# amin-abouee/apex-solver

Measured on AMD Instinct MI355X. Metric: ms per LM iter (Jacobian+Schur+solve), lower is better.
Workload: dtype f64; 1 GPU; final-13682 synthetic (13682 cameras / 4456117 landmarks / 28966251 observations); optimization_type=selfcal, camera_dof=9, schur_variant=sparse, s_tile_rows=856, s_tiles=8071, s_tiles_touched=4284, etree_levels=41, border_cameras=0, schur_form=4, variant_asked=Sparse, reason=, variant_choice=direct, parallelism=landmark-shard x1

## Files before the change

### apex-solver_amd/capi.py

```python
from __future__ import annotations

import ctypes as C
import os

import numpy as np

_HERE = os.path.dirname(os.path.abspath(__file__))
LIB_PATH = os.path.join(_HERE, "libapexgpu.so")
LIB_PATH = os.environ.get("APEXGPU_LIB", LIB_PATH)

NUM_STAGES = 10
STAGE_NAMES = ("cam_reduce", "landmark_reduce", "schur_scatter", "all_reduce", "factor", "tri_solve",
               "back_substitute", "step_stats", "retract", "cost")

SYMBOLS = (
    "apexgpu_create", "apexgpu_destroy", "apexgpu_last_error", "apexgpu_version", "apexgpu_set_structure",
    "apexgpu_set_cg_params", "apexgpu_set_params", "apexgpu_get_params", "apexgpu_cost", "apexgpu_assemble", "apexgpu_solve_augmented",
    "apexgpu_step_stats", "apexgpu_eval_step", "apexgpu_commit_step", "apexgpu_discard_step",
    "apexgpu_parameter_norm", "apexgpu_column_norms", "apexgpu_set_column_scaling", "apexgpu_lm_optimize", "apexgpu_get_residual", "apexgpu_get_jacobian_blocks",
    "apexgpu_get_schur", "apexgpu_camera_covariance", "apexgpu_covariance_stats", "apexgpu_landmark_covariance", "apexgpu_landmark_covariance_stats", "apexgpu_get_landmark_blocks", "apexgpu_get_hessian_csc", "apexgpu_debug_invert_blocks", "apexgpu_debug_pair_lists", "apexgpu_debug_pair_lists_queued", "apexgpu_debug_pair_lists_queued_dc", "apexgpu_debug_host_structure", "apexgpu_setup_times", "apexgpu_schur_matvec", "apexgpu_set_option", "apexgpu_enable_stage_timing", "apexgpu_reset_stage_times",
    "apexgpu_stage_times", "apexgpu_info", "apexgpu_variant_info", "apexgpu_variant_costs", "apexgpu_trim_host_cache", "apexgpu_host_cache_bytes", "apexgpu_counters", "apexgpu_debug_get_pair_records", "apexgpu_get_unique_id", "apexgpu_comm_init", "apexgpu_comm_init_shm", "apexgpu_set_shard", "apexgpu_shard_range",
    "apexgpu_debug_lockstep_solve", "apexgpu_export_step", "apexgpu_owned_landmarks", "apexgpu_debug_partition", "apexgpu_debug_check_schedule",
    "apexgpu_debug_schedule_ops", "apexgpu_debug_plan_lists", "apexgpu_debug_sinv_lists", "apexgpu_debug_sinv_lists_direct",
    "apexgpu_debug_tiles_create", "apexgpu_debug_tiles_pattern", "apexgpu_debug_tiles_set", "apexgpu_debug_tiles_factor",
    "apexgpu_debug_tiles_solve", "apexgpu_debug_tiles_matvec", "apexgpu_debug_tiles_pcg", "apexgpu_debug_tiles_get", "apexgpu_debug_tiles_destroy",
    "apexgpu_bal_open", "apexgpu_bal_close", "apexgpu_bal_last_error", "apexgpu_bal_sizes", "apexgpu_bal_raw",
    "apexgpu_bal_variables", "apexgpu_reference_columns",
    "apexgpu_pg_create", "apexgpu_pg_destroy", "apexgpu_pg_last_error", "apexgpu_pg_set_structure", "apexgpu_pg_set_params",
    "apexgpu_pg_get_params", "apexgpu_pg_cost", "apexgpu_pg_solve_augmented", "apexgpu_pg_step_stats", "apexgpu_pg_eval_step",
    "apexgpu_pg_commit_step", "apexgpu_pg_discard_step", "apexgpu_pg_parameter_norm", "apexgpu_pg_column_norms",
    "apexgpu_pg_set_column_scaling", "apexgpu_pg_lm_optimize",
    "apexgpu_pg_get_residual", "apexgpu_pg_get_jacobian_blocks", "apexgpu_pg_get_hessian", "apexgpu_pg_covariance", "apexgpu_pg_covariance_stats", "apexgpu_pg_set_option",
    "apexgpu_pg_enable_stage_timing", "apexgpu_pg_reset_stage_times", "apexgpu_pg_stage_times", "apexgpu_pg_info", "apexgpu_pg_counters",
    "apexgpu_pg_set_priors", "apexgpu_pg_get_prior_residual",
    "apexgpu_g2o_open", "apexgpu_g2o_close", "apexgpu_g2o_last_error", "apexgpu_g2o_sizes", "apexgpu_g2o_raw",
    "apexgpu_g2o_problem", "apexgpu_pose_graph_columns",
    "apexgpu_pg_create_se2", "apexgpu_pg_manifold", "apexgpu_g2o_raw_se2", "apexgpu_g2o_problem_se2",
    "apexgpu_pose_graph_columns_se2",
    "apexgpu_pg_create_so3",
    "apexgpu_pg_jv_gram", "apexgpu_pg_dogleg_step", "apexgpu_pg_gn_optimize", "apexgpu_pg_dogleg_optimize",
    "apexgpu_jv_gram", "apexgpu_dogleg_step", "apexgpu_dogleg_optimize",
    "apexgpu_pg_set_loss", "apexgpu_pg_get_loss", "apexgpu_loss_evaluate", "apexgpu_set_loss", "apexgpu_get_loss",
    "apexgpu_pg_set_information", "apexgpu_pg_get_information", "apexgpu_g2o_problem_information",
    "apexgpu_set_pose_priors", "apexgpu_set_intrinsic_priors", "apexgpu_get_prior_residual",
)
MANIFOLD_SE3, MANIFOLD_SE2, MANIFOLD_SO3 = 0, 1, 2
MANIFOLD_SIZES = {MANIFOLD_SE3: (7, 6), MANIFOLD_SE2: (3, 3), MANIFOLD_SO3: (4, 3)}
LOSS_KINDS = ("NONE", "L2", "L1", "HUBER", "CAUCHY", "FAIR", "GEMAN_MCCLURE", "WELSCH", "TUKEY", "ANDREWS", "RAMSAY",
              "TRIMMED_MEAN", "LP_NORM", "BARRON", "T_DISTRIBUTION")
(LOSS_NONE, LOSS_L2, LOSS_L1, LOSS_HUBER, LOSS_CAUCHY, LOSS_FAIR, LOSS_GEMAN_MCCLURE, LOSS_WELSCH, LOSS_TUKEY, LOSS_ANDREWS,
 LOSS_RAMSAY, LOSS_TRIMMED_MEAN, LOSS_LP_NORM, LOSS_BARRON, LOSS_T_DISTRIBUTION) = range(15)
PG_NUM_STAGES = 6
PG_STAGE_NAMES = ("assemble", "factor", "tri_solve", "step_stats", "retract", "cost")
_NON_INT = ("apexgpu_destroy", "apexgpu_debug_tiles_destroy", "apexgpu_last_error", "apexgpu_version", "apexgpu_host_cache_bytes", "apexgpu_bal_close", "apexgpu_bal_last_error",
            "apexgpu_pg_destroy", "apexgpu_pg_last_error", "apexgpu_g2o_close", "apexgpu_g2o_last_error")

ERROR_NAMES = {
    -1: "FactorizationFailed", -2: "SingularMatrix", -3: "SparseMatrixCreation", -4: "MatrixConversion",
    -5: "InvalidInput", -6: "InvalidState", -10: "DeviceError",
}


class LinAlgError(RuntimeError):

    def __init__(self, code: int, message: str):
        self.code = code
        self.kind = ERROR_NAMES.get(code, f"Error({code})")
        super().__init__(f"{self.kind}: {message}")


class LmConfigC(C.Structure):
    _fields_ = [
        ("max_iterations", C.c_int), ("cost_tolerance", C.c_double), ("parameter_tolerance", C.c_double),
        ("gradient_tolerance", C.c_double), ("damping", C.c_double), ("damping_min", C.c_double),
# ... 71 lines not shown
    L.apexgpu_eval_step.argtypes = [vp, C.POINTER(dbl)]
    L.apexgpu_commit_step.argtypes = [vp]
    L.apexgpu_discard_step.argtypes = [vp]
    L.apexgpu_parameter_norm.argtypes = [vp, C.POINTER(dbl)]
    L.apexgpu_column_norms.argtypes = [vp, vp]
    L.apexgpu_debug_lockstep_solve.argtypes = [vp, C.c_int, C.c_double]
    L.apexgpu_export_step.argtypes = [vp, vp, vp]
    L.apexgpu_owned_landmarks.argtypes = [vp, vp]
    L.apexgpu_debug_partition.argtypes = [C.c_int, vp, C.c_int, vp]
    L.apexgpu_debug_check_schedule.argtypes = [C.c_int, vp, C.c_int, C.c_int, vp, vp, C.c_char_p, C.c_int]
    L.apexgpu_debug_schedule_ops.argtypes = [C.c_int, vp, C.c_int, C.c_int, vp, C.c_int, vp, C.c_int]
    L.apexgpu_debug_plan_lists.argtypes = [C.c_int, vp, C.c_int, C.c_int, vp, C.c_int, vp, C.c_int]
    L.apexgpu_debug_sinv_lists.argtypes = [C.c_int, vp, vp, C.c_int, vp, vp]
    L.apexgpu_debug_sinv_lists_direct.argtypes = [C.c_int, vp, C.c_int, vp, vp, vp, C.c_int, vp, C.c_char_p, C.c_int]
    L.apexgpu_debug_tiles_create.argtypes = [C.c_int, C.c_int, vp, vp, C.POINTER(vp)]
    L.apexgpu_debug_tiles_pattern.argtypes = [vp, vp, vp]
    L.apexgpu_debug_tiles_set.argtypes = [vp, vp, C.c_int, dbl, C.c_int]
    L.apexgpu_debug_tiles_factor.argtypes = [vp, C.POINTER(C.c_int)]
    L.apexgpu_debug_tiles_solve.argtypes = [vp, C.c_int, vp, vp]
    L.apexgpu_debug_tiles_matvec.argtypes = [vp, vp, vp]
    L.apexgpu_debug_tiles_pcg.argtypes = [vp, vp, C.c_int, dbl, vp, C.POINTER(C.c_int), vp]
    L.apexgpu_debug_tiles_get.argtypes = [vp, C.c_int, vp, C.POINTER(C.c_int)]
    L.apexgpu_debug_tiles_destroy.argtypes = [vp]
    L.apexgpu_debug_tiles_destroy.restype = None
    L.apexgpu_set_column_scaling.argtypes = [vp, vp]
    L.apexgpu_lm_optimize.argtypes = [vp, C.POINTER(LmConfigC), C.POINTER(LmResultC), vp, C.c_int]
    L.apexgpu_get_residual.argtypes = [vp, vp]
    L.apexgpu_get_jacobian_blocks.argtypes = [vp, vp, vp]
    L.apexgpu_get_schur.argtypes = [vp, vp, vp]
    L.apexgpu_camera_covariance.argtypes = [vp, vp]
    L.apexgpu_covariance_stats.argtypes = [vp, C.POINTER(dbl * 6), vp, C.c_int]
    L.apexgpu_landmark_covariance.argtypes = [vp, vp]
    L.apexgpu_landmark_covariance_stats.argtypes = [vp, C.POINTER(dbl * 4)]
    L.apexgpu_get_landmark_blocks.argtypes = [vp, vp, vp]
    L.apexgpu_schur_matvec.argtypes = [vp, dbl, vp, vp, vp]
    L.apexgpu_set_option.argtypes = [vp, C.c_char_p, C.c_int]
    L.apexgpu_get_hessian_csc.argtypes = [vp, vp, vp, vp, vp]
    L.apexgpu_debug_invert_blocks.argtypes = [C.c_int, C.c_int64, vp, vp, vp]
    L.apexgpu_debug_host_structure.argtypes = [C.c_int64, C.c_int64, C.c_int64, C.c_int, vp, vp, C.c_int, C.c_int, vp, vp, vp, vp, vp]
    L.apexgpu_setup_times.argtypes = [vp, vp, vp]
    L.apexgpu_debug_pair_lists.argtypes = [C.c_int64, C.c_int64, C.c_int64, C.c_int, vp, vp, vp, vp, vp, vp, vp, vp]
    L.apexgpu_debug_pair_lists_queued.argtypes = [C.c_int64, C.c_int64, C.c_int64, vp, vp, vp, vp, vp, vp, vp, vp, vp]
    L.apexgpu_enable_stage_timing.argtypes = [vp, C.c_int]
    L.apexgpu_reset_stage_times.argtypes = [vp]
    L.apexgpu_stage_times.argtypes = [vp, C.POINTER(dbl * NUM_STAGES), C.POINTER(i64 * NUM_STAGES)]
    L.apexgpu_info.argtypes = [vp, C.POINTER(dbl * 16)]
    L.apexgpu_trim_host_cache.argtypes = [C.POINTER(C.c_int64)]
    L.apexgpu_host_cache_bytes.argtypes = []
    L.apexgpu_host_cache_bytes.restype = C.c_int64
    L.apexgpu_debug_get_pair_records.argtypes = [vp, vp, i64]
    L.apexgpu_variant_info.argtypes = [vp, C.c_int, C.POINTER(C.c_int), C.c_char_p, C.c_int]
    L.apexgpu_variant_costs.argtypes = [vp, C.POINTER(dbl * 4)]
    L.apexgpu_counters.argtypes = [vp, C.POINTER(i64 * 4)]
    L.apexgpu_get_unique_id.argtypes = [vp]
    L.apexgpu_comm_init.argtypes = [vp, C.c_int, C.c_int, vp]
    L.apexgpu_comm_init_shm.argtypes = [vp, C.c_int, C.c_int, C.c_char_p]
    L.apexgpu_set_shard.argtypes = [vp, C.c_int, C.c_int]
    L.apexgpu_shard_range.argtypes = [i64, i64, vp, C.c_int, C.c_int, C.POINTER(i64), C.POINTER(i64)]
    L.apexgpu_bal_open.argtypes = [C.c_char_p, C.POINTER(vp)]
    L.apexgpu_bal_close.argtypes = [vp]
    L.apexgpu_bal_close.restype = None
    L.apexgpu_bal_last_error.restype = C.c_char_p
    L.apexgpu_bal_sizes.argtypes = [vp, C.POINTER(i64), C.POINTER(i64), C.POINTER(i64)]
    L.apexgpu_bal_raw.argtypes = [vp, vp, vp, vp, vp, vp]
    L.apexgpu_bal_variables.argtypes = [vp, vp, vp]
    L.apexgpu_reference_columns.argtypes = [i64, i64, vp, vp, vp]
    L.apexgpu_pg_create.argtypes = [i64, i64, C.c_int, C.POINTER(vp)]
    L.apexgpu_pg_destroy.argtypes = [vp]
    L.apexgpu_pg_destroy.restype = None
    L.apexgpu_pg_last_error.argtypes = [vp]
    L.apexgpu_pg_last_error.restype = C.c_char_p
    L.apexgpu_pg_set_structure.argtypes = [vp, vp, vp, vp, vp, vp, dbl]
    L.apexgpu_pg_set_params.argtypes = [vp, vp]
    L.apexgpu_pg_set_priors.argtypes = [vp, C.c_int64, vp, vp, vp]
    L.apexgpu_pg_get_prior_residual.argtypes = [vp, vp]
    L.apexgpu_pg_set_loss.argtypes = [vp, C.c_int, dbl, dbl]
    L.apexgpu_set_loss.argtypes = [vp, C.c_int, dbl, dbl]
    L.apexgpu_set_pose_priors.argtypes = [vp, C.c_int64, vp, vp, vp, vp]
    L.apexgpu_set_intrinsic_priors.argtypes = [vp, C.c_int64, vp, vp, vp, vp]
    L.apexgpu_get_prior_residual.argtypes = [vp, vp, vp]
    L.apexgpu_get_loss.argtypes = [vp, C.POINTER(C.c_int), C.POINTER(dbl * 2)]
    L.apexgpu_pg_get_loss.argtypes = [vp, C.POINTER(C.c_int), C.POINTER(dbl * 2)]
    L.apexgpu_loss_evaluate.argtypes = [C.c_int, dbl, dbl, dbl, C.POINTER(dbl * 6)]
    L.apexgpu_pg_get_params.argtypes = [vp, vp]
    L.apexgpu_pg_cost.argtypes = [vp, C.POINTER(dbl)]
    L.apexgpu_pg_solve_augmented.argtypes = [vp, dbl, vp, vp]
    L.apexgpu_pg_step_stats.argtypes = [vp, C.POINTER(dbl * 3)]
    L.apexgpu_pg_eval_step.argtypes = [vp, C.POINTER(dbl)]
    L.apexgpu_pg_commit_step.argtypes = [vp]
    L.apexgpu_pg_discard_step.argtypes = [vp]
    L.apexgpu_pg_parameter_norm.argtypes = [vp, C.POINTER(dbl)]
    L.apexgpu_pg_column_norms.argtypes = [vp, vp]
    L.apexgpu_pg_set_column_scaling.argtypes = [vp, vp]
    L.apexgpu_pg_lm_optimize.argtypes = [vp, C.POINTER(LmConfigC), C.POINTER(LmResultC), vp, C.c_int]
    L.apexgpu_jv_gram.argtypes = [vp, vp, vp, C.POINTER(dbl * 3)]
    L.apexgpu_dogleg_step.argtypes = [vp, dbl, dbl, C.c_int, C.POINTER(dbl * 8)]
    L.apexgpu_dogleg_optimize.argtypes = [vp, C.POINTER(DlConfigC), C.POINTER(LmResultC), vp, C.c_int]
    L.apexgpu_pg_jv_gram.argtypes = [vp, vp, vp, C.POINTER(dbl * 3)]
    L.apexgpu_pg_dogleg_step.argtypes = [vp, dbl, dbl, C.c_int, C.POINTER(dbl * 8)]
    L.apexgpu_pg_gn_optimize.argtypes = [vp, C.POINTER(GnConfigC), C.POINTER(LmResultC), vp, C.c_int]
    L.apexgpu_pg_dogleg_optimize.argtypes = [vp, C.POINTER(DlConfigC), C.POINTER(LmResultC), vp, C.c_int]
    L.apexgpu_pg_get_residual.argtypes = [vp, vp]
    L.apexgpu_pg_get_jacobian_blocks.argtypes = [vp, vp]
    L.apexgpu_pg_get_hessian.argtypes = [vp, dbl, vp, vp]
    L.apexgpu_pg_covariance.argtypes = [vp, vp]
    L.apexgpu_pg_covariance_stats.argtypes = [vp, C.POINTER(dbl * 6), vp, C.c_int]
# ... 25 lines not shown
        if name not in _NON_INT:
            f.restype = C.c_int
    _lib = L
    return L


def tile_partition(present: np.ndarray, world: int):
    L = load()
    pr = np.ascontiguousarray(present, dtype=np.uint8)
    nt = pr.shape[0]
    owner = np.zeros(nt, dtype=np.int32)
    n_top = L.apexgpu_debug_partition(nt, pr.ctypes.data_as(C.c_void_p), int(world), owner.ctypes.data_as(C.c_void_p))
    if n_top < 0:
        raise LinAlgError(n_top, "apexgpu_debug_partition")
    return owner, n_top


def check_schedule(present: np.ndarray, world: int = 1, rank: int = 0, two_side: int = 1, overlap: int = 1, split_u1: int = 4,
                   flood_gate: int = 256, factor_flow: int = -1, factor_flow_rows: int = 24, old_idle_level_bug: bool = False,
                   drop_wait: int = -1) -> dict:
    L = load()
    pr = np.ascontiguousarray(present, dtype=np.uint8)
    nt = pr.shape[0]
    opts = np.array([two_side, overlap, split_u1, flood_gate, factor_flow, factor_flow_rows, int(old_idle_level_bug), drop_wait], dtype=np.int32)
    out = np.zeros(8, dtype=np.int64)
    msg = C.create_string_buffer(512)
    rc = L.apexgpu_debug_check_schedule(nt, pr.ctypes.data_as(C.c_void_p), int(world), int(rank), opts.ctypes.data_as(C.c_void_p),
                                        out.ctypes.data_as(C.c_void_p), msg, 512)
    if rc < 0:
        raise LinAlgError(rc, "apexgpu_debug_check_schedule: " + msg.value.decode())
    return dict(levels=rc, calls=int(out[0]), launches=int(out[1]), violations=int(out[2]) + int(out[3]), violations_top=int(out[3]),
                flow_units=int(out[4]), flow_groups=int(out[5]), waits=int(out[6]), dropped=bool(out[7]), first=msg.value.decode())


def schedule_ops(present: np.ndarray, phase: int = 0, world: int = 1, rank: int = 0, two_side: int = 1, overlap: int = 1, split_u1: int = 4,
                 flood_gate: int = 256, factor_flow: int = -1, factor_flow_rows: int = 24) -> np.ndarray:
    L = load()
    pr = np.ascontiguousarray(present, dtype=np.uint8)
    nt = pr.shape[0]
    opts = np.array([two_side, overlap, split_u1, flood_gate, factor_flow, factor_flow_rows, 0, -1], dtype=np.int32)
    args = (nt, pr.ctypes.data_as(C.c_void_p), int(world), int(rank), opts.ctypes.data_as(C.c_void_p), int(phase))
    n = L.apexgpu_debug_schedule_ops(*args, None, 0)
    if n < 0:
        raise LinAlgError(n, "apexgpu_debug_schedule_ops")
    rows = np.zeros((n, 6), dtype=np.int64)
    if n and L.apexgpu_debug_schedule_ops(*args, rows.ctypes.data_as(C.c_void_p), n) != n:
        raise LinAlgError(-6, "apexgpu_debug_schedule_ops")
    return rows


PLAN_TABLES = (("scalars", 23), ("slots", 3), ("columns", 4), ("owner_ranges", 5), ("levels", 9), ("fwd_cut", 2), ("upd_rounds", 2),
               ("bwd_step", 1), ("potrf", 5), ("panel", 7), ("upd", 7), ("fwd", 6), ("bwd", 6), ("flow_fwd", 10), ("flow_bwd", 10),
               ("units", 16), ("sym_row_ptr", 1), ("sym_entries", 3), ("sym_tiles", 3), ("group_cols", 2))


def plan_lists(present: np.ndarray, which: str, world: int = 1, rank: int = 0, two_side: int = 1, overlap: int = 1, split_u1: int = 4,
               flood_gate: int = 256, factor_flow: int = -1, factor_flow_rows: int = 24) -> np.ndarray:
    L = load()
    pr = np.ascontiguousarray(present, dtype=np.uint8)
    w = [n for n, _ in PLAN_TABLES].index(which)
    opts = np.array([two_side, overlap, split_u1, flood_gate, factor_flow, factor_flow_rows, 0, -1], dtype=np.int32)
    args = (pr.shape[0], pr.ctypes.data_as(C.c_void_p), int(world), int(rank), opts.ctypes.data_as(C.c_void_p), w)
    n = L.apexgpu_debug_plan_lists(*args, None, 0)
    if n < 0:
        raise LinAlgError(n, "apexgpu_debug_plan_lists")
    rows = np.zeros((n, PLAN_TABLES[w][1]), dtype=np.int64)
    if n and L.apexgpu_debug_plan_lists(*args, rows.ctypes.data_as(C.c_void_p), n) != n:
        raise LinAlgError(-6, "apexgpu_debug_plan_lists")
    return rows


def _sinv_rows(call, what, msg=None):
    counts = np.zeros(4, dtype=np.int64)
    n = call(None, 0, ptr(counts))
    if n < 0:
        raise LinAlgError(n, what + (": " + msg.value.decode() if msg is not None else ""))
    rows = np.zeros((n, 6), dtype=np.int64)
    if n and call(ptr(rows), n, ptr(counts)) != n:
        raise LinAlgError(-6, what)
    return rows, counts


def sinv_lists(present: np.ndarray, with_slots: bool = False):
    L = load()
    pr = np.ascontiguousarray(present, dtype=np.uint8)
    slot = np.zeros(pr.shape, dtype=np.int32)
    out = _sinv_rows(lambda rows, n, counts: L.apexgpu_debug_sinv_lists(pr.shape[0], ptr(pr), rows, n, counts, ptr(slot)), "apexgpu_debug_sinv_lists")
    return out + (slot,) if with_slots else out


def sinv_lists_direct(slot: np.ndarray, groups):
    L = load()
    sl = np.ascontiguousarray(slot, dtype=np.int32)
    gp = np.cumsum([0] + [len(g) for g in groups]).astype(np.int32)
    gc = np.array([c for g in groups for c in g] + [0], dtype=np.int32)
    msg = C.create_string_buffer(512)
    return _sinv_rows(lambda rows, n, counts: L.apexgpu_debug_sinv_lists_direct(sl.shape[0], ptr(sl), len(groups), ptr(gp), ptr(gc), rows, n, counts, msg, 512),
                      "apexgpu_debug_sinv_lists_direct", msg)


HOST_STRUCTURE_STATS = ("tile_rows", "hub_cameras", "border_tiles", "touched_tiles", "tiles", "etree_levels", "top_columns",
                        "tree_sharded", "s_order", "s_lists", "s_plan", "s_schur_lists", "s_uploads", "s_total", "pair_contributions",
                        "pair_blocks")


def host_structure(n_cam: int, n_pt: int, cam_idx: np.ndarray, pt_idx: np.ndarray, mode: int = 1, rank: int = 0, world: int = 1,
                   nested_dissection: int = 1, hubs_last: int = 1, dist_factor: int = 1, tree_sharding: int = 1, schur_form: int = 3):
    ci = np.ascontiguousarray(cam_idx, dtype=np.uint32); pi = np.ascontiguousarray(pt_idx, dtype=np.uint32)
    opts = np.array([nested_dissection, hubs_last, dist_factor, tree_sharding, schur_form], dtype=np.int32)
    stats = np.zeros(16); dc = 9 if mode in (1, 4, 5, 6) else 6
    nt = (n_cam * dc + 143) // 144
    cmap = np.zeros(n_cam, dtype=np.int32); owned = np.zeros(n_pt, dtype=np.uint8); towner = np.zeros(nt, dtype=np.int32)
    rc = load().apexgpu_debug_host_structure(n_cam, n_pt, len(ci), mode, ptr(ci), ptr(pi), rank, world, ptr(opts), ptr(stats),
                                             ptr(cmap), ptr(owned), ptr(towner))
    if rc != 0:
        raise LinAlgError(rc, "apexgpu_debug_host_structure failed")
    out = dict(zip(HOST_STRUCTURE_STATS, stats.tolist()))
    out.update(cmap=cmap, owned=owned.astype(bool), tile_owner=towner)
    return out
# ... 211 lines not shown
```

### apex-solver_amd/csrc/capi.cpp

```cpp
#include "../../include/apexgpu.h"

#include <string.h>

#include <algorithm>
#include <exception>
#include <new>
#include <string>
#include <vector>

#include "ba_structure.h"
#include "pg_solver.h"
#include "sinv_lists.h"
#include "solver.h"
#ifdef APEX_WITH_RCCL
#include <rccl/rccl.h>
#include <string.h>
#endif

struct apexgpu_solver {
    apex::Solver* s;
    std::string create_error;
};

static_assert(sizeof(apexgpu_lm_config) == sizeof(apex::LmConfig), "LmConfig layout");
static_assert(sizeof(apexgpu_lm_iter) == sizeof(apex::LmIterRecord), "LmIterRecord layout");
static_assert(sizeof(apexgpu_lm_result) == sizeof(apex::LmResult), "LmResult layout");
static_assert(sizeof(apexgpu_gn_config) == sizeof(apex::GnConfig), "GnConfig layout");
static_assert(sizeof(apexgpu_dl_config) == sizeof(apex::DlConfig), "DlConfig layout");
static_assert(sizeof(apexgpu_dl_iter) == sizeof(apex::DlIterRecord), "DlIterRecord layout");
static_assert(sizeof(apex::DoglegStepInfo) == 8 * sizeof(double), "DoglegStepInfo layout");
static_assert(APEXGPU_NUM_STAGES == apex::kNumStages, "stage count");
static_assert(APEXGPU_PG_NUM_STAGES == apex::kPgNumStages, "pose-graph stage count");

struct apexgpu_pg_solver {
    apex::PoseGraphSolver* s;
};

#define H_OR_FAIL            \
    if (!h || !h->s) return APEXGPU_ERR_INVALID_STATE

template <typename F>
static int guarded(F&& f) noexcept {
    try {
        return f();
    } catch (const std::bad_alloc&) {
        return APEXGPU_ERR_INVALID_INPUT;
    } catch (const std::exception&) {
        return APEXGPU_ERR_INVALID_INPUT;
    } catch (...) {
        return APEXGPU_ERR_INVALID_STATE;
    }
}

template <typename S>
static int covariance_stats(S* s, double out[6], double* group_ms, int group_cap) {
    if (!out) return APEXGPU_ERR_INVALID_INPUT;
    const apex::TilePlan& tp = s->plan();
    const apex::SelectedInverse& inv = tp.inverse();
    int64_t y = 0, zo = 0, zd = 0;
    inv.op_counts(&y, &zo, &zd);
    const std::vector<double>& ms = inv.group_ms();
    out[0] = (double)inv.bytes(); out[1] = (double)y; out[2] = (double)zo; out[3] = (double)zd; out[4] = tp.n_levels();
    int n = 0;
    if (group_ms)
        for (; n < group_cap && n < (int)ms.size(); ++n) group_ms[n] = ms[n];
    out[5] = n;
    return APEXGPU_OK;
}

template <typename S>
static bool shared_option(S* s, const std::string& n, int value) {
    if (n == "graphs") s->enable_graphs(value != 0);
    else if (n == "update_overlap") { s->enable_overlap(value != 0); if (value > 1) s->set_overlap_min(value); }
    else if (n == "tri_dataflow") s->enable_tri_flow(value != 0);
    else if (n == "split_u1") s->set_split_u1(value);
    else if (n == "flood_gate") s->set_gate_min(value);
    else if (n == "two_side") s->set_two_side(value);
    else if (n == "eager_step_eval") s->set_eager_step_eval(value != 0);
    else if (n == "one_wait") s->set_one_wait(value != 0);
    else if (n == "factor_flow") s->set_factor_flow(value, 0);
    else if (n == "factor_flow_rows") s->set_factor_flow(s->plan().factor_flow_cols(), value);
    else if (n == "debug_poison_sweep") s->debug_poison_next_solve(value);
    else if (n == "debug_poison_factor") s->debug_poison_next_factor();
    else if (n == "nested_dissection") s->set_nd(value != 0, value > 1 ? value : 0);
    else if (n == "covariance_timing") s->enable_covariance_timing(value != 0);
    else return false;
    return true;
}
template <typename S>
static int counters(S* s, int64_t out[4]) {
    if (!out) return APEXGPU_ERR_INVALID_INPUT;
    out[0] = s->sweep_timeouts(); out[1] = s->plan().tri_flow() ? 1 : 0; out[2] = s->factor_flow_timeouts(); out[3] = s->plan().factor_flow_groups();
    return APEXGPU_OK;
}
template <typename S>
static int stage_timing(S* s, int on) {
    if (on > 1) s->enable_stage_timing_only((uint32_t)on >> 1);
    else s->enable_stage_timing(on != 0);
    return APEXGPU_OK;
}

#include <execinfo.h>
#include <signal.h>
namespace {
void segv_backtrace(int sig) {
    void* frames[64];
    const int n = backtrace(frames, 64);
    backtrace_symbols_fd(frames, n, 2);
    raise(sig);
}
void segv_hook() {
    static const bool on = [] { const char* e = getenv("APEX_SEGV_BACKTRACE"); return e && e[0] == '1'; }();
    if (!on) return;
    static thread_local char alt[1 << 16];
    stack_t ss; ss.ss_sp = alt; ss.ss_size = sizeof(alt); ss.ss_flags = 0;
    (void)sigaltstack(&ss, nullptr);
    struct sigaction sa;
    memset(&sa, 0, sizeof(sa));
    sa.sa_handler = segv_backtrace; sa.sa_flags = SA_ONSTACK | SA_RESETHAND;
    (void)sigaction(SIGSEGV, &sa, nullptr);
}
}

extern "C" {

const char* apexgpu_version(void) { return "apexgpu 0.1 (gfx950)"; }

int apexgpu_create(int64_t n_cam, int64_t n_pt, int64_t n_obs, int mode, int device, apexgpu_solver** out) {
    if (!out) return APEXGPU_ERR_INVALID_INPUT;
// ... 240 lines not shown
    });
}

static int plan_table(const apex::PlanStructure& s, const apex::PlanLists& l, const double* tiles, const double* linv, int which, std::vector<int64_t>* out, int* width) {
    constexpr ptrdiff_t kTile = (ptrdiff_t)apex::kNB * apex::kNB;
    auto clean = [](const double* p) { return reinterpret_cast<const double*>(reinterpret_cast<uintptr_t>(p) & ~uintptr_t(7)); };
    auto in_linv = [&](const double* p) { return p >= linv && p < linv + s.nt * kTile; };
    auto arr = [&](const double* p) -> int64_t { p = clean(p); return !p ? -1 : in_linv(p) ? 1 : 0; };
    auto idx = [&](const double* p) -> int64_t { p = clean(p); return !p ? -1 : in_linv(p) ? (p - linv) / kTile : (p - tiles) / kTile; };
    auto bits = [](double v) { int64_t b; memcpy(&b, &v, sizeof b); return b; };
    auto row = [&](std::initializer_list<int64_t> v) { *width = (int)v.size(); out->insert(out->end(), v); };
    auto gemm = [&](const std::vector<apex::GemmTask>& v) {
        *width = 7;
        for (const apex::GemmTask& t : v) row({arr(t.C), idx(t.C), (int64_t)(reinterpret_cast<uintptr_t>(t.C) & 1), arr(t.A), idx(t.A), arr(t.B), idx(t.B)});
    };
    auto tri = [&](const std::vector<apex::TriTask>& v) {
        *width = 6;
        for (const apex::TriTask& t : v) row({arr(t.Mdiag), idx(t.Mdiag), arr(t.Moff), idx(t.Moff), t.k, t.other});
    };
    auto flow = [&](const std::vector<apex::FlowTask>& v) {
        *width = 10;
        for (const apex::FlowTask& t : v) row({arr(t.mat), idx(t.mat), t.src, t.dst, t.part, t.count, arr(t.mat2), idx(t.mat2), t.src2, t.slot2});
    };
    const int nt = s.nt;
    switch (which) {
        case 0: {
            const apex::PlanLists::Flow* f = l.flow;
            row({s.n_levels(), s.n_local_groups, s.n_top_cols, s.n_slots, s.n_touched, (int64_t)l.potrf.size(), (int64_t)l.panel.size(), (int64_t)l.upd.size(),
                 l.two_side_plan, l.first_ok, f[0].g0, f[0].g1, f[0].first, f[0].n, f[1].g0, f[1].g1, f[1].first, f[1].n, l.n_flow_local, l.n_flow_parts,
                 bits(s.predicted_ms), bits(f[0].sim_us), bits(f[1].sim_us)});
            break;
        }
        case 1: *width = 3; for (int I = 0; I < nt; ++I) for (int J = 0; J < nt; ++J) if (s.slot_of(I, J) >= 0) row({I, J, s.slot_of(I, J)}); break;
        case 2: *width = 4; for (int K = 0; K < nt; ++K) row({K, s.cls[K], s.owner[K], s.diag_slot[K]}); break;
        case 3:
            for (size_t o = 0; o < s.own_range.size(); ++o) row({(int64_t)o, s.own_range[o].first, s.own_range[o].second, s.own_fill[o].first, s.own_fill[o].second});
            row({-1, s.n_t_nt, s.n_touched - s.n_t_nt, s.n_f_nt, s.n_slots - s.n_f_nt});
            break;
        case 4: *width = 9; for (const apex::Level& v : l.lv) row({v.potrf, v.panel, v.fwd, v.upd, v.u1o, v.u2a, v.u2b1, v.u2b2, (int64_t)v.fwd_cut.size()}); break;
        case 5: *width = 2; for (size_t g = 0; g < l.lv.size(); ++g) for (int c : l.lv[g].fwd_cut) row({(int64_t)g, c}); break;
        case 6: *width = 2; for (const auto& r : l.upd_rounds) row({r.first, r.second}); break;
        case 7: *width = 1; for (int b : l.bwd_step) row({b}); break;
        case 8: *width = 5; for (const apex::PotrfTask& t : l.potrf) row({arr(t.A), idx(t.A), arr(t.Linv), idx(t.Linv), t.K}); break;
        case 9: gemm(l.panel); break;
        case 10: gemm(l.upd); break;
        case 11: tri(l.fwd); break;
        case 12: tri(l.bwd); break;
        case 13: flow(l.flow_fwd); break;
        case 14: flow(l.flow_bwd); break;
        case 15:
            *width = 16;
            for (const apex::FactorUnit& u : l.units)
                row({arr(u.C), idx(u.C), arr(u.A), idx(u.A), arr(u.B), idx(u.B), u.wait_flag[0], u.wait_flag[1], u.wait_flag[2], u.wait_val[0], u.wait_val[1], u.wait_val[2],
                     u.pub, u.kind, u.strip, u.pad});
            break;
        case 16: *width = 1; for (int v : l.sym_row_ptr) row({v}); break;
        case 17: *width = 3; for (const apex::SymEntry& e : l.sym_entries) row({e.slot, e.other, e.kind}); break;
        case 18: *width = 3; for (const apex::SymTile& t : l.sym_tiles) row({t.slot, t.I, t.J}); break;
        case 19: *width = 2; for (size_t g = 0; g < s.group_cols.size(); ++g) for (int K : s.group_cols[g]) row({(int64_t)g, K}); break;
        default: return APEXGPU_ERR_INVALID_INPUT;
    }
    return APEXGPU_OK;
}

int apexgpu_debug_plan_lists(int nt, const uint8_t* present, int world, int rank, const int opts[8], int which, int64_t* rows, int max_rows) {
    if (nt <= 0 || !present || !opts || world < 1 || rank < 0 || rank >= world || max_rows < 0 || (max_rows > 0 && !rows)) return APEXGPU_ERR_INVALID_INPUT;
    return guarded([&]() -> int {
    const HostPlan hp = host_plan(nt, present, world, rank, opts);
    if (!hp.err.empty()) return APEXGPU_ERR_INVALID_STATE;
    std::vector<int64_t> out;
    int width = 1;
    const int rc = plan_table(hp.s, hp.l, reinterpret_cast<const double*>(apex::kStandInTiles), reinterpret_cast<const double*>(apex::kStandInLinv), which, &out, &width);
    if (rc != APEXGPU_OK) return rc;
    const size_t n = out.size() / (size_t)width;
    if (max_rows > 0) memcpy(rows, out.data(), std::min(n, (size_t)max_rows) * (size_t)width * sizeof(int64_t));
    return (int)n;
    });
}

static int sinv_rows(const apex::SinvLists& l, int64_t* rows, int max_rows, int64_t counts[4]) {
    const size_t n = l.tasks.size() + l.prods.size();
    size_t i = 0;
    for (size_t g = 0; g < l.groups.size(); ++g)
        for (int k = 0; k < 3; ++k)
            for (int t = l.groups[g][k]; t < l.groups[g][k + 1] && i < (size_t)max_rows; ++t, ++i) {
                const apex::SinvTaskH& tk = l.tasks[t];
                int64_t* r = rows + 6 * i;
                r[0] = k; r[1] = (int64_t)g; r[2] = tk.C.array; r[3] = tk.C.tile; r[4] = tk.first; r[5] = tk.count;
            }
    for (size_t p = 0; p < l.prods.size() && l.tasks.size() + p < (size_t)max_rows; ++p) {
        const apex::SinvProdH& pr = l.prods[p];
        int64_t* r = rows + 6 * (l.tasks.size() + p);
        r[0] = 3; r[1] = pr.A.array; r[2] = pr.A.tile; r[3] = pr.B.array; r[4] = pr.B.tile; r[5] = pr.op;
    }
    if (counts) { counts[0] = l.n[0]; counts[1] = l.n[1]; counts[2] = l.n[2]; counts[3] = l.y_max; }
    return (int)n;
}

int apexgpu_debug_sinv_lists(int nt, const uint8_t* present, int64_t* rows, int max_rows, int64_t counts[4], int32_t* slot_out) {
    if (nt <= 0 || !present || max_rows < 0 || (max_rows > 0 && !rows)) return APEXGPU_ERR_INVALID_INPUT;
    return guarded([&]() -> int {
    const apex::PlanStructure s = apex::plan_structure(nt, std::vector<uint8_t>(present, present + (size_t)nt * nt), apex::PlanOptions());
    if (s.refused) return APEXGPU_ERR_INVALID_STATE;
    if (slot_out) memcpy(slot_out, s.slot.data(), (size_t)nt * nt * sizeof(int32_t));
    apex::SinvLists lists;
    if (!apex::build_sinv_lists(nt, s.slot.data(), s.group_cols, &lists).empty()) return APEXGPU_ERR_INVALID_STATE;
    return sinv_rows(lists, rows, max_rows, counts);
    });
}

int apexgpu_debug_sinv_lists_direct(int nt, const int32_t* slot, int n_groups, const int32_t* group_ptr, const int32_t* group_cols,
                                    int64_t* rows, int max_rows, int64_t counts[4], char* msg, int msg_len) {
    if (nt <= 0 || !slot || n_groups < 0 || !group_ptr || !group_cols || max_rows < 0 || (max_rows > 0 && !rows)) return APEXGPU_ERR_INVALID_INPUT;
    return guarded([&]() -> int {
    std::vector<std::vector<int>> groups(n_groups);
    for (int g = 0; g < n_groups; ++g) {
        if (group_ptr[g] < 0 || group_ptr[g + 1] < group_ptr[g]) return APEXGPU_ERR_INVALID_INPUT;
        for (int i = group_ptr[g]; i < group_ptr[g + 1]; ++i) {
            if (group_cols[i] < 0 || group_cols[i] >= nt || slot[(size_t)group_cols[i] * nt + group_cols[i]] < 0) return APEXGPU_ERR_INVALID_INPUT;
            groups[g].push_back(group_cols[i]);
        }
    }
    apex::SinvLists lists;
    const std::string e = apex::build_sinv_lists(nt, slot, groups, &lists);
    if (msg && msg_len > 0) snprintf(msg, (size_t)msg_len, "%s", e.c_str());
    if (!e.empty()) return APEXGPU_ERR_INVALID_STATE;
    return sinv_rows(lists, rows, max_rows, counts);
    });
}

int apexgpu_owned_landmarks(apexgpu_solver* h, uint8_t* mask) {
    H_OR_FAIL;
    if (!mask) return APEXGPU_ERR_INVALID_INPUT;
    return h->s->owned_landmarks(mask);
}
int apexgpu_export_step(apexgpu_solver* h, double* step_out, double* grad_out) { H_OR_FAIL; return guarded([&] { return h->s->export_step(step_out, grad_out); }); }

int apexgpu_set_option(apexgpu_solver* h, const char* name, int value) {
    H_OR_FAIL;
    const std::string n = name ? name : "";
    static const char* const structural[] = {"schur_form", "hubs_last", "dist_factor", "tree_sharding", "dist_selftest", "nested_dissection", "update_overlap",
                                             "split_u1", "flood_gate", "two_side", "factor_flow", "factor_flow_rows", "device_pair_list", "matrix_free_only",
                                             "auto_variant", "variant_cost_permille", "max_tile_updates"};
    if (h->s->has_structure())
        for (const char* k : structural)
            if (n == k) return APEXGPU_ERR_INVALID_STATE;
    if (n == "schur_form") {
        if (value != 3 && value != 4) return APEXGPU_ERR_INVALID_INPUT;
        h->s->set_schur_form(value);
    }
    else if (shared_option(h->s, n, value)) return APEXGPU_OK;
    else if (n == "matrix_free_only") h->s->set_matrix_free_only(value != 0);
    else if (n == "auto_variant") h->s->set_auto_variant(value != 0);
    else if (n == "variant_cost_permille") h->s->set_variant_cost_permille(value);
    else if (n == "device_pair_list") h->s->set_device_pair_recs(value != 0);
    else if (n == "max_tile_updates") h->s->set_max_tile_updates(value);
    else if (n == "debug_occupy_cus") return h->s->debug_occupy_cus(value, 40000);
    else if (n == "hubs_last") h->s->set_hubs_last(value != 0);
    else if (n == "dist_factor") h->s->set_dist_factor(value != 0);
    else if (n == "tree_sharding") h->s->set_tree_sharding(value != 0);
    else if (n == "dist_selftest") h->s->set_dist_selftest(value);
    else return APEXGPU_ERR_INVALID_INPUT;
    return APEXGPU_OK;
}
int apexgpu_enable_stage_timing(apexgpu_solver* h, int on) {
    H_OR_FAIL;
    return stage_timing(h->s, on);
}
int apexgpu_reset_stage_times(apexgpu_solver* h) { H_OR_FAIL; h->s->reset_stage_times(); return APEXGPU_OK; }
int apexgpu_stage_times(apexgpu_solver* h, double ms[APEXGPU_NUM_STAGES], int64_t calls[APEXGPU_NUM_STAGES]) {
    H_OR_FAIL;
    h->s->stage_times(ms, calls);
    return APEXGPU_OK;
}
int apexgpu_setup_times(apexgpu_solver* h, double seconds[6], double counts[4]) {
    H_OR_FAIL;
    if (!seconds) return APEXGPU_ERR_INVALID_INPUT;
    for (int k = 0; k < 6; ++k) seconds[k] = h->s->setup_seconds()[k];
    if (counts) { counts[0] = h->s->n_hubs(); counts[1] = h->s->pair_blocks(); counts[2] = h->s->pair_slots(); counts[3] = h->s->schur_form(); }
    return APEXGPU_OK;
}
int apexgpu_info(apexgpu_solver* h, double info[16]) {
    H_OR_FAIL;
    info[0] = h->s->n_tile_rows(); info[1] = (double)h->s->tile_count(); info[2] = h->s->schur_scatter_pairs();
    info[3] = (double)h->s->cam_dof_internal(); info[4] = h->s->last_reg(); info[5] = h->s->last_pcg_iters();
    info[6] = h->s->touched_tiles(); info[7] = h->s->local_obs();
    info[8] = h->s->n_levels();
    int64_t a = 0, b = 0, c = 0;
    h->s->plan().op_counts(&a, &b, &c);
    info[9] = (double)a; info[10] = (double)b; info[11] = (double)c;
    info[12] = h->s->dist_top_columns(); info[13] = h->s->dist_local_fraction();
    info[14] = h->s->tree_sharded() ? 1.0 : 0.0;
    info[15] = h->s->schur_form();
    return APEXGPU_OK;
}

int apexgpu_debug_get_pair_records(apexgpu_solver* h, uint32_t* recs4_out, int64_t cap_slots) {
    H_OR_FAIL;
    if (!recs4_out) return APEXGPU_ERR_INVALID_INPUT;
    return guarded([&] { return h->s->get_pair_records(recs4_out, cap_slots); });
}
int apexgpu_trim_host_cache(int64_t* released_bytes) {
    const size_t n = apex::HostBlockCache::get().trim();
    if (released_bytes) *released_bytes = (int64_t)n;
    return APEXGPU_OK;
}
int apexgpu_variant_costs(apexgpu_solver* h, double out[4]) {
    H_OR_FAIL;
    if (!out) return APEXGPU_ERR_INVALID_INPUT;
    h->s->variant_costs(out);
    return APEXGPU_OK;
}
int64_t apexgpu_host_cache_bytes(void) { return (int64_t)apex::HostBlockCache::get().kept_bytes(); }
int apexgpu_variant_info(apexgpu_solver* h, int asked_variant, int* used_variant, char* reason, int reason_len) {
    H_OR_FAIL;
    if (asked_variant != APEXGPU_VARIANT_SPARSE && asked_variant != APEXGPU_VARIANT_ITERATIVE && asked_variant != APEXGPU_VARIANT_IMPLICIT)
        return APEXGPU_ERR_INVALID_INPUT;
    if (used_variant) *used_variant = h->s->variant_used(asked_variant);
    if (reason && reason_len > 0) {
        const std::string& r = h->s->variant_reason();
        const size_t n = std::min<size_t>(r.size(), (size_t)reason_len - 1);
        memcpy(reason, r.data(), n);
        reason[n] = 0;
    }
    return APEXGPU_OK;
}

int apexgpu_counters(apexgpu_solver* h, int64_t out[4]) {
    H_OR_FAIL;
    return counters(h->s, out);
}

int apexgpu_get_unique_id(void* out128) {
#ifdef APEX_WITH_RCCL
    if (!out128) return APEXGPU_ERR_INVALID_INPUT;
    ncclUniqueId id;
    if (ncclGetUniqueId(&id) != ncclSuccess) return APEXGPU_ERR_DEVICE;
    memcpy(out128, &id, 128);
    return APEXGPU_OK;
#else
    (void)out128;
    return APEXGPU_ERR_INVALID_STATE;
#endif
}
int apexgpu_comm_init(apexgpu_solver* h, int world, int rank, const void* unique_id128) {
    H_OR_FAIL;
    if (!unique_id128) return APEXGPU_ERR_INVALID_INPUT;
    return guarded([&] { return h->s->comm_init(world, rank, unique_id128); });
}
int apexgpu_comm_init_shm(apexgpu_solver* h, int world, int rank, const char* name) {
    H_OR_FAIL;
    if (!name) return APEXGPU_ERR_INVALID_INPUT;
    return guarded([&] { return h->s->comm_init_shm(world, rank, name); });
}
int apexgpu_shard_range(int64_t n_pt, int64_t n_obs, const uint32_t* pt_idx, int rank, int world, int64_t* lo, int64_t* hi) {
    if (!pt_idx || !lo || !hi || world < 1 || rank < 0 || rank >= world || n_pt <= 0) return APEXGPU_ERR_INVALID_INPUT;
    return guarded([&]() -> int {
        std::vector<int64_t> ptr(n_pt + 1, 0);
        for (int64_t i = 0; i < n_obs; ++i) {
            if (pt_idx[i] >= (uint64_t)n_pt) return APEXGPU_ERR_INVALID_INPUT;
            ptr[pt_idx[i] + 1]++;
        }
        for (int64_t l = 0; l < n_pt; ++l) ptr[l + 1] += ptr[l];
        apex::shard_range(n_pt, ptr.data(), rank, world, lo, hi);
        return APEXGPU_OK;
    });
}
int apexgpu_set_shard(apexgpu_solver* h, int rank, int world) { H_OR_FAIL; return h->s->set_shard(rank, world); }

static int debug_pair_lists_impl(int64_t n_cam, int64_t n_pt, int64_t n_obs, int dc, const uint32_t* cam_idx, const uint32_t* pt_idx,
                                 int64_t counts[4], uint32_t* recs4_out, int32_t* chunks2_out, int64_t* blocks4_out,
                                 int32_t* tasks2_out, int32_t* o_index_out, bool queued, int64_t* qdesc3_out) {
    if (n_cam <= 0 || n_pt <= 0 || n_obs < 0 || (dc != 6 && dc != 9) || !cam_idx || !pt_idx || !counts) return APEXGPU_ERR_INVALID_INPUT;
    return guarded([&]() -> int {
        for (int64_t i = 0; i < n_obs; ++i)
            if (cam_idx[i] >= (uint64_t)n_cam || pt_idx[i] >= (uint64_t)n_pt) return APEXGPU_ERR_INVALID_INPUT;
        std::vector<int> pt_ptr(n_pt + 1, 0), order(n_obs);
        for (int64_t i = 0; i < n_obs; ++i) pt_ptr[pt_idx[i] + 1]++;
        for (int64_t l = 0; l < n_pt; ++l) pt_ptr[l + 1] += pt_ptr[l];
        { std::vector<int> fill(pt_ptr.begin(), pt_ptr.end() - 1); for (int64_t i = 0; i < n_obs; ++i) order[fill[pt_idx[i]]++] = (int)i; }
        for (int64_t l = 0; l < n_pt; ++l)
            std::stable_sort(order.begin() + pt_ptr[l], order.begin() + pt_ptr[l + 1], [&](int a, int b) { return cam_idx[a] < cam_idx[b]; });
        std::vector<uint32_t> o_cam(n_obs), o_pt(n_obs);
// ... 229 lines not shown
    return APEXGPU_OK;
}
int apexgpu_pg_set_information(apexgpu_pg_solver* h, const double* info) {
    PG_OR_FAIL;
    return guarded([&] { return h->s->set_information(info); });
}
int apexgpu_pg_get_information(apexgpu_pg_solver* h, int* present, double* info_out) {
    PG_OR_FAIL;
    if (!present) return APEXGPU_ERR_INVALID_INPUT;
    return h->s->get_information(present, info_out);
}
int apexgpu_loss_evaluate(int kind, double p0, double p1, double s, double out6[6]) {
    apex::PgLoss l;
    if (!out6 || !apex::pg_loss_make(kind, p0, p1, &l)) return APEXGPU_ERR_INVALID_INPUT;
    apex::pg_loss_evaluate(l, s, out6);
    const apex::PgCorrector c = apex::pg_corrector(out6, s);
    out6[3] = c.sqrt_rho1; out6[4] = c.residual_scaling; out6[5] = c.alpha_sq_norm;
    return APEXGPU_OK;
}
int apexgpu_pg_get_prior_residual(apexgpu_pg_solver* h, double* r7_out) {
    PG_OR_FAIL;
    return h->s->get_prior_residual(r7_out);
}
int apexgpu_pg_get_hessian(apexgpu_pg_solver* h, double lambda, double* H_out, double* g_out) {
    PG_OR_FAIL;
    return h->s->get_hessian(lambda, H_out, g_out);
}
int apexgpu_pg_covariance(apexgpu_pg_solver* h, double* cov_out) {
    PG_OR_FAIL;
    return guarded([&] { return h->s->covariance(cov_out); });
}
int apexgpu_pg_covariance_stats(apexgpu_pg_solver* h, double out[6], double* group_ms, int group_cap) { PG_OR_FAIL; return covariance_stats(h->s, out, group_ms, group_cap); }
int apexgpu_pg_set_option(apexgpu_pg_solver* h, const char* name, int value) {
    PG_OR_FAIL;
    const std::string n = name ? name : "";
    if (n == "row_owned_assembly")
        return (value == 0 || value == 1) && h->s->set_row_owned_option(value == 1) ? APEXGPU_OK : APEXGPU_ERR_INVALID_INPUT;
    return shared_option(h->s, n, value) ? APEXGPU_OK : APEXGPU_ERR_INVALID_INPUT;
}
int apexgpu_pg_enable_stage_timing(apexgpu_pg_solver* h, int on) {
    PG_OR_FAIL;
    return stage_timing(h->s, on);
}
int apexgpu_pg_reset_stage_times(apexgpu_pg_solver* h) { PG_OR_FAIL; h->s->reset_stage_times(); return APEXGPU_OK; }
int apexgpu_pg_stage_times(apexgpu_pg_solver* h, double ms[APEXGPU_PG_NUM_STAGES], int64_t calls[APEXGPU_PG_NUM_STAGES]) {
    PG_OR_FAIL;
    h->s->stage_times(ms, calls);
    return APEXGPU_OK;
}
int apexgpu_pg_counters(apexgpu_pg_solver* h, int64_t out[4]) {
    PG_OR_FAIL;
    return counters(h->s, out);
}
int apexgpu_pg_info(apexgpu_pg_solver* h, double info[8]) {
    PG_OR_FAIL;
    info[0] = h->s->n_tile_rows(); info[1] = (double)h->s->tile_count(); info[2] = (double)h->s->touched_tiles();
    info[3] = h->s->n_levels(); info[4] = (double)h->s->dof() * (double)h->s->n_vertices();
    int64_t a = 0, b = 0, c = 0;
    h->s->plan().op_counts(&a, &b, &c);
    info[5] = (double)a; info[6] = (double)b; info[7] = (double)c;
    return APEXGPU_OK;
}

}
```

### apex-solver_amd/csrc/chol_kernels.h

```cpp
#pragma once
#include <hip/hip_runtime.h>
#include <stdint.h>

#include "ba_kernels.h"
#include "tile_tasks.h"

namespace apex {

void launch_potrf_inv(const PotrfTask* tasks, int n, int* fail, hipStream_t s, int* arrived = nullptr);
void launch_gate(const int* arrived, int expected, int max_micros, hipStream_t s);
void launch_factor_flow(const FactorUnit* units, int n_units, int* ver, int* fail, int* err, hipStream_t s,
                        unsigned long long* trace = nullptr);
void launch_tile_gemm_nt(const GemmTask* tasks, int n, double alpha, double beta, hipStream_t s, bool tri_b = false);
void launch_clear_i32(int* p, int64_t n, hipStream_t s);
void launch_post_word(int* word, int* host_word_dev, hipStream_t s);
void launch_tri_flow(bool backward, const FlowTask* tasks, int n_tasks, const double* in, double* out, double* part, int* flags,
                     int nt, hipStream_t s, const double* fold_b, double* fold_out, int poison_block = -1, bool keep_flags = false);
void launch_occupy_cus(int n, int micros, int* started, hipStream_t s);
void launch_tri_step(bool trans, const TriTask* tasks, int n, double* vwork, double* vout, hipStream_t s);
void launch_tile_diag(const double* tiles, const int* diag_slot, int nt, double* diag, hipStream_t s);
void launch_tile_add_diag(double* tiles, const int* diag_slot, int n_valid, int n_total, double add_valid,
                          double set_pad, hipStream_t s);
void launch_vec_select(int n, const double* in, const int* cls, int mask, double* out, hipStream_t s);
void launch_vec_merge(int n, const double* src, const int* cls, int mask, double* dst, hipStream_t s);
void launch_tile_scale_sym(const SymTile* list, int n, double* tiles, const double* scale , hipStream_t s);

}
```

### apex-solver_amd/csrc/chol_kernels.hip

```cpp
#include <hip/hip_runtime.h>
#include <stdint.h>

#include "chol_kernels.h"
#include "device_reduce.hpp"
#include "tile_kernel_defs.h"
#include <algorithm>

namespace apex {

constexpr int BS = 16;
constexpr int NBK = NB / BS;
constexpr int BP = 18;
constexpr int BSZ = BS * BP;
constexpr int NLB = NBK * (NBK + 1) / 2;

__device__ __forceinline__ int bidx(int bi, int bj) { return bi * (bi + 1) / 2 + bj; }

__device__ __forceinline__ double readlane_f64(double v, int src) {
    const int lo = __builtin_amdgcn_readlane(__double2loint(v), src);
    const int hi = __builtin_amdgcn_readlane(__double2hiint(v), src);
    return __hiloint2double(hi, lo);
}

__device__ __forceinline__ double4_t blk_mma_nt(const double* X, const double* Y, double4_t acc, int lr, int lk, double sgn) {
// ... 38 lines not shown
__device__ __forceinline__ __amdgpu_buffer_rsrc_t coh_rsrc(const void* tile) {
    return __builtin_amdgcn_make_buffer_rsrc(const_cast<void*>(tile), 0, NB * NB * (int)sizeof(double), 0x00020000);
}
template <bool COH>
__device__ __forceinline__ double2 tile_ld2(const double* tile, __amdgpu_buffer_rsrc_t r, int off) {
    if constexpr (COH) {
        const i32x4_t q = __builtin_amdgcn_raw_buffer_load_b128(r, off * 8, 0, kCohAux);
        double2 v; v.x = __hiloint2double(q[1], q[0]); v.y = __hiloint2double(q[3], q[2]);
        return v;
    } else {
        return *reinterpret_cast<const double2*>(tile + off);
    }
}
template <bool COH>
__device__ __forceinline__ void tile_st2(double* tile, __amdgpu_buffer_rsrc_t r, int off, double2 v) {
    if constexpr (COH) {
        i32x4_t q;
        q[0] = __double2loint(v.x); q[1] = __double2hiint(v.x); q[2] = __double2loint(v.y); q[3] = __double2hiint(v.y);
        __builtin_amdgcn_raw_buffer_store_b128(q, r, off * 8, 0, kCohAux);
    } else {
        *reinterpret_cast<double2*>(tile + off) = v;
    }
}
__device__ __forceinline__ double coh_ld1(__amdgpu_buffer_rsrc_t r, int off) {
    const i32x2_t q = __builtin_amdgcn_raw_buffer_load_b64(r, off * 8, 0, kCohAux);
    return __hiloint2double(q[1], q[0]);
}
__device__ __forceinline__ void coh_st1(__amdgpu_buffer_rsrc_t r, int off, double v) {
    i32x2_t q; q[0] = __double2loint(v); q[1] = __double2hiint(v);
    __builtin_amdgcn_raw_buffer_store_b64(q, r, off * 8, 0, kCohAux);
}
template <bool COH>
__device__ __forceinline__ void blk_to_tile(const double* __restrict__ src, double* __restrict__ dst_tile, __amdgpu_buffer_rsrc_t r,
                                            int bi, int bj, int t, int nthreads) {
    for (int idx = t; idx < 128; idx += nthreads) {
        const int rr = idx >> 3, c2 = idx & 7;
        double2 v; v.x = src[rr * BP + 2 * c2]; v.y = src[rr * BP + 2 * c2 + 1];
        tile_st2<COH>(dst_tile, r, (16 * bi + rr) * NB + 16 * bj + 2 * c2, v);
    }
}

__device__ __forceinline__ double4_t blk_load_cd_sym(const double* C, int lr, int lk) {
    double4_t v;
#pragma unroll
    for (int r = 0; r < 4; ++r) {
        const int row = lk + 4 * r;
        v[r] = row >= lr ? C[row * BP + lr] : C[lr * BP + row];
    }
    return v;
}

template <int NW, bool COH>
__device__ __forceinline__ void potrf_tile_mf(double* __restrict__ A, double* __restrict__ Linv, int K, int* __restrict__ fail,
                                              double* sA, double* sD, int* bad, int* sync_cnt) {
    constexpr int NT = 64 * NW;
    const int tid = threadIdx.x, lane = tid & 63, w = tid >> 6;
    const int lr = lane & 15, lk = lane >> 4;
    constexpr int NH = NW - (NW + 3) / 4;
    const bool helper = (w & 3) != 0;
    const int hid = w - 1 - (w >> 2);
    const __amdgpu_buffer_rsrc_t rA = coh_rsrc(A), rL = coh_rsrc(Linv);
    if (tid == 0) { *bad = 0; *sync_cnt = 0; }
    {
        constexpr int NREG = (128 * 45 + NT - 1) / NT + NBK;
        double2 reg[NREG];
        int n = 0;
#pragma unroll
        for (int bi = 0; bi < NBK; ++bi) {
            const int per_row = 8 * (bi + 1), cnt = 16 * per_row;
#pragma unroll
            for (int it = 0; it < (16 * 8 * (bi + 1) + NT - 1) / NT; ++it, ++n) {
                const int idx = tid + NT * it;
                if (idx < cnt) {
                    const int rr = idx / per_row, c2 = idx - rr * per_row;
                    reg[n] = tile_ld2<COH>(A, rA, (16 * bi + rr) * NB + 2 * c2);
                }
            }
        }
        n = 0;
#pragma unroll
        for (int bi = 0; bi < NBK; ++bi) {
            const int per_row = 8 * (bi + 1), cnt = 16 * per_row;
#pragma unroll
            for (int it = 0; it < (16 * 8 * (bi + 1) + NT - 1) / NT; ++it, ++n) {
                const int idx = tid + NT * it;
                if (idx < cnt) {
                    const int rr = idx / per_row, c2 = idx - rr * per_row;
                    double* dst = sA + bidx(bi, c2 >> 3) * BSZ + rr * BP + 2 * (c2 & 7);
                    dst[0] = reg[n].x; dst[1] = reg[n].y;
                }
            }
        }
    }
    __syncthreads();
    POTRF_STAMP();

    double4_t Dm = (double4_t){0.0, 0.0, 0.0, 0.0};
    if (w == 0) Dm = blk_load_cd_sym(sA, lr, lk);
    for (int kb = 0; kb < NBK; ++kb) {
        double4_t T[(NBK - 1 + NH - 1) / NH];
        if (w == 0) {
            double4_t Xm, Ls = (double4_t){0.0, 0.0, 0.0, 0.0}, Xs = (double4_t){0.0, 0.0, 0.0, 0.0};
#pragma unroll
            for (int r = 0; r < 4; ++r) Xm[r] = (lk + 4 * r == lr) ? 1.0 : 0.0;
            double rmask[4];
#pragma unroll
            for (int q = 0; q < 4; ++q) rmask[q] = lk == q ? 1.0 : 0.0;
            auto rsq_newton = [](double d) {
                double r = __builtin_amdgcn_rsq(d);
                r = r * fma(-0.5 * d * r, r, 1.5);
// ... 70 lines not shown
                    double4_t acc = (double4_t){0.0, 0.0, 0.0, 0.0};
                    for (int k = j; k < r; ++k) {
                        const double* Y = (k == j) ? (sD + j * BSZ) : (sA + bidx(k, j) * BSZ);
                        acc = blk_mma_nn(sA + bidx(r, k) * BSZ, Y, acc, lr, lk);
                    }
                    T[nt] = acc;
                }
            }
        }
        __syncthreads();
        POTRF_STAMP();
        if (helper && kb >= 1) {
            const int r = kb - 1;
            int nt = 0;
            for (int j = hid; j < r; j += NH, ++nt) blk_store_cd(sA + bidx(r, j) * BSZ, T[nt], lr, lk, -1.0);
        }
        {
            const int m = NBK - 1 - kb;
            if (w == 0) {
                if (m > 0) {
                    double* N = sA + bidx(kb + 1, kb) * BSZ;
                    double4_t Lt = (double4_t){0.0, 0.0, 0.0, 0.0};
                    Lt = blk_mma_nt(sD + kb * BSZ, N, Lt, lr, lk, 1.0);
                    Dm = blk_load_cd_sym(sA + bidx(kb + 1, kb + 1) * BSZ, lr, lk);
#pragma unroll
                    for (int r = 0; r < 4; ++r) N[lr * BP + lk + 4 * r] = Lt[r];
#pragma unroll
                    for (int r = 0; r < 4; ++r) Dm = __builtin_amdgcn_mfma_f64_16x16x4f64(-Lt[r], Lt[r], Dm, 0, 0, 0);
                }
            } else if (helper) {
                const int t0 = m > 0 ? 1 : 0;
                for (int t = t0 + hid; t < m + kb; t += NH) {
                    if (t < m) {
                        double* P = sA + bidx(kb + 1 + t, kb) * BSZ;
                        double4_t acc = (double4_t){0.0, 0.0, 0.0, 0.0};
                        acc = blk_mma_nt(P, sD + kb * BSZ, acc, lr, lk, 1.0);
                        blk_store_cd(P, acc, lr, lk, 1.0);
                    } else {
                        const int k = t - m;
                        double* Bk = sA + bidx(kb, k) * BSZ;
                        blk_to_tile<COH>(Bk, A, rA, kb, k, lane, 64);
                        double4_t acc = (double4_t){0.0, 0.0, 0.0, 0.0};
                        acc = blk_mma_nn(sD + kb * BSZ, Bk, acc, lr, lk);
                        blk_store_cd(Bk, acc, lr, lk, 1.0);
                    }
                }
                if (hid == NH - 1) blk_to_tile<COH>(sA + bidx(kb, kb) * BSZ, A, rA, kb, kb, lane, 64);
            }
        }
        if (w == 0 || helper) {
            __builtin_amdgcn_fence(__ATOMIC_RELEASE, "workgroup");
            if (lane == 0) __hip_atomic_fetch_add(sync_cnt, 1, __ATOMIC_RELAXED, __HIP_MEMORY_SCOPE_WORKGROUP);
        }
        if (helper) {
            const int target = (kb + 1) * (NH + 1);
            while (__hip_atomic_load(sync_cnt, __ATOMIC_RELAXED, __HIP_MEMORY_SCOPE_WORKGROUP) < target) __builtin_amdgcn_s_sleep(0);
            __builtin_amdgcn_fence(__ATOMIC_ACQUIRE, "workgroup");
        }
        POTRF_STAMP();
    }
    __syncthreads();
    {
        const int r = NBK - 1;
        double4_t T[(NBK - 1 + NW - 1) / NW];
        int nt = 0;
        for (int j = w; j < r; j += NW, ++nt) {
            double4_t acc = (double4_t){0.0, 0.0, 0.0, 0.0};
            for (int k = j; k < r; ++k) {
                const double* Y = (k == j) ? (sD + j * BSZ) : (sA + bidx(k, j) * BSZ);
                acc = blk_mma_nn(sA + bidx(r, k) * BSZ, Y, acc, lr, lk);
            }
            T[nt] = acc;
        }
        __syncthreads();
        nt = 0;
        for (int j = w; j < r; j += NW, ++nt) blk_store_cd(sA + bidx(r, j) * BSZ, T[nt], lr, lk, -1.0);
        __syncthreads();
    }
#pragma unroll
    for (int bi = 0; bi < NBK; ++bi) {
        const int per_row = 8 * (bi + 1), cnt = 16 * per_row;
        for (int idx = tid; idx < cnt; idx += NT) {
            const int rr = idx / per_row, c2 = idx - rr * per_row;
            const int bj = c2 >> 3;
            const double* src = ((bj == bi) ? (sD + bi * BSZ) : (sA + bidx(bi, bj) * BSZ)) + rr * BP + 2 * (c2 & 7);
            double2 v; v.x = src[0]; v.y = src[1];
            tile_st2<COH>(Linv, rL, (16 * bi + rr) * NB + 2 * c2, v);
        }
    }
    if (tid == 0 && *bad) atomicCAS(fail, 0, K + 1);
    POTRF_STAMP();
}

template <int NW>
__global__ __launch_bounds__(64 * NW) void k_potrf_inv_mf(const PotrfTask* __restrict__ tasks, int* __restrict__ fail,
                                                          int* __restrict__ arrived) {
    if (arrived != nullptr && threadIdx.x == 0) __hip_atomic_fetch_add(arrived, 1, __ATOMIC_RELAXED, __HIP_MEMORY_SCOPE_AGENT);
    POTRF_STAMP();
    __shared__ double sA[NLB * BSZ];
    __shared__ double sD[NBK * BSZ];
    __shared__ int bad, sync_cnt;
    const PotrfTask pt = tasks[blockIdx.x];
    potrf_tile_mf<NW, false>(pt.A, pt.Linv, pt.K, fail, sA, sD, &bad, &sync_cnt);
}
#undef POTRF_STAMP

constexpr int KC = 16;
constexpr int STRIP = 48;
constexpr int NSTRIP = NB / STRIP;
constexpr int kGemmSmallMax = 56;

template <bool TRI>
__global__ __launch_bounds__(256, 3) void k_tile_gemm_nt(const GemmTask* __restrict__ tasks, int n_units, double alpha, double beta) {
    constexpr int P4 = KC + 2;
    constexpr int IMG = (NB + STRIP) * P4;
    __shared__ double sm[IMG];
    const int per_xcd = (n_units + 7) >> 3;
    const int unit = (blockIdx.x & 7) * per_xcd + (blockIdx.x >> 3);
    if ((int)(blockIdx.x >> 3) >= per_xcd || unit >= n_units) return;
    GemmTask tg = tasks[unit / NSTRIP];
    const bool first = (reinterpret_cast<uintptr_t>(tg.C) & 1) != 0;
    tg.C = reinterpret_cast<double*>(reinterpret_cast<uintptr_t>(tg.C) & ~uintptr_t(7));
    const int strip = unit % NSTRIP;
    const int tid = threadIdx.x, lane = tid & 63, w = __builtin_amdgcn_readfirstlane(tid >> 6);
    const int lr = lane & 15, lk = lane >> 4;
    GlobalCF64 Ag = (GlobalCF64)tg.A + (size_t)strip * STRIP * NB;
    GlobalCF64 Bg = (GlobalCF64)tg.B;
    constexpr int NACC = TRI ? 9 : 7;
    int cb[3];
    if (TRI) { cb[0] = 16 * (8 - w); cb[1] = 16 * (1 + w); cb[2] = w == 3 ? 0 : -16; }
    else { cb[0] = 32 * w; cb[1] = 32 * w + 16; cb[2] = 128; }
    const bool extra = TRI ? (w == 3) : (w < 3);
    double4_t acc[NACC];
#pragma unroll
    for (int j = 0; j < NACC; ++j) acc[j] = (double4_t){0.0, 0.0, 0.0, 0.0};
    constexpr int C2 = KC / 2, NR = (NB + STRIP) * C2 / 256, RPR = 256 / C2;
    static_assert((NB + STRIP) * C2 % 256 == 0 && 256 % C2 == 0 && NR == 6 && RPR == 32, "staging loop assumes whole rounds");
    const int r0 = tid / C2, c2 = tid % C2;
    const unsigned offB = r0 * NB + 2 * c2, offA = (r0 + 16) * NB + 2 * c2;
    GlobalCF64 p4 = r0 < 16 ? Bg + (size_t)(r0 + 128) * NB + 2 * c2 : Ag + (size_t)(r0 - 16) * NB + 2 * c2;
    const int dst0 = r0 * P4 + 2 * c2;
    f64x2_t rg[NR];
    auto gload = [&](int k0) {
#pragma unroll
        for (int i = 0; i < 4; ++i) rg[i] = *reinterpret_cast<GlobalCF64x2>(Bg + (offB + (unsigned)(RPR * i * NB + k0)));
        rg[4] = *reinterpret_cast<GlobalCF64x2>(p4 + k0);
        rg[5] = *reinterpret_cast<GlobalCF64x2>(Ag + (offA + (unsigned)k0));
    };
    auto stage = [&](double* img) {
#pragma unroll
        for (int i = 0; i < NR; ++i) { img[dst0 + RPR * i * P4] = rg[i].x; img[dst0 + RPR * i * P4 + 1] = rg[i].y; }
    };
    auto compute = [&](const double* img, int k0) {
        const double* sB = img;
        const double* sA = img + NB * P4;
#pragma unroll
        for (int kk = 0; kk < KC; kk += 4) {
            if (TRI) {
                if (k0 > cb[0]) continue;
                double av[3], bv[3];
#pragma unroll
                for (int i = 0; i < 3; ++i) av[i] = sA[(16 * i + lr) * P4 + kk + lk];
#pragma unroll
                for (int j = 0; j < 3; ++j) bv[j] = sB[((cb[j] < 0 ? 0 : cb[j]) + lr) * P4 + kk + lk];
#pragma unroll
                for (int j = 0; j < 3; ++j) {
                    if (k0 > cb[j]) continue;
#pragma unroll
                    for (int i = 0; i < 3; ++i)
                        acc[3 * i + j] = __builtin_amdgcn_mfma_f64_16x16x4f64(av[i], bv[j], acc[3 * i + j], 0, 0, 0);
                }
            } else {
                double av[3], bv[2];
#pragma unroll
                for (int i = 0; i < 3; ++i) av[i] = sA[(16 * i + lr) * P4 + kk + lk];
#pragma unroll
                for (int j = 0; j < 2; ++j) bv[j] = sB[(cb[j] + lr) * P4 + kk + lk];
#pragma unroll
                for (int i = 0; i < 3; ++i)
#pragma unroll
                    for (int j = 0; j < 2; ++j)
                        acc[2 * i + j] = __builtin_amdgcn_mfma_f64_16x16x4f64(av[i], bv[j], acc[2 * i + j], 0, 0, 0);
                if (extra) {
                    const double ax = sA[(16 * w + lr) * P4 + kk + lk], bx = sB[(128 + lr) * P4 + kk + lk];
                    acc[6] = __builtin_amdgcn_mfma_f64_16x16x4f64(ax, bx, acc[6], 0, 0, 0);
                }
            }
        }
    };
    gload(0);
    for (int k0 = 0; k0 < NB; k0 += KC) {
        __syncthreads();
        stage(sm);
        __syncthreads();
        if (k0 + KC < NB) gload(k0 + KC);
        compute(sm, k0);
    }
    GlobalF64 C = (GlobalF64)tg.C + (size_t)strip * STRIP * NB;
    auto brow = [&](int n) { return TRI ? 16 * (n / 3) : (n < 6 ? 16 * (n / 2) : 16 * w); };
    auto bcol = [&](int n) { return TRI ? cb[n % 3] : (n < 6 ? cb[n % 2] : 128); };
    if (beta == 0.0 || first) {
        const double zero = first ? 0.0 : -0.0;
#pragma unroll
        for (int n = 0; n < NACC; ++n) {
            if (TRI ? (n % 3 == 2 && !extra) : (n == 6 && !extra)) continue;
#pragma unroll
            for (int r = 0; r < 4; ++r) C[(size_t)(brow(n) + lk + 4 * r) * NB + bcol(n) + lr] = alpha * acc[n][r] + zero;
        }
        return;
    }
    if (TRI) {
#pragma unroll
        for (int n = 0; n < NACC; ++n) {
            if (n % 3 == 2 && !extra) continue;
#pragma unroll
            for (int r = 0; r < 4; ++r) {
                GlobalF64 p = C + (size_t)(brow(n) + lk + 4 * r) * NB + bcol(n) + lr;
                *p = alpha * acc[n][r] + beta * *p;
            }
        }
        return;
    }
    double cv[3][4];
#pragma unroll
    for (int n = 0; n < 2; ++n)
#pragma unroll
        for (int r = 0; r < 4; ++r) cv[n][r] = C[(size_t)(brow(n) + lk + 4 * r) * NB + bcol(n) + lr];
#pragma unroll
    for (int n = 0; n < NACC; ++n) {
        if (n + 2 < NACC && (n + 2 < 6 || extra)) {
#pragma unroll
            for (int r = 0; r < 4; ++r) cv[(n + 2) % 3][r] = C[(size_t)(brow(n + 2) + lk + 4 * r) * NB + bcol(n + 2) + lr];
        }
        if (n == 6 && !extra) continue;
#pragma unroll
        for (int r = 0; r < 4; ++r)
            C[(size_t)(brow(n) + lk + 4 * r) * NB + bcol(n) + lr] = alpha * acc[n][r] + beta * cv[n % 3][r];
    }
}

__global__ __launch_bounds__(192) void k_tile_gemm_nt_small(const GemmTask* __restrict__ tasks, int n_units, double alpha,
                                                              double beta) {
    __shared__ double sA[48 * PS];
    __shared__ double sB[48 * PS];
    const int unit = blockIdx.x;
    if (unit >= n_units) return;
    GemmTask tg = tasks[unit / 9];
    const bool first = (reinterpret_cast<uintptr_t>(tg.C) & 1) != 0;
    tg.C = reinterpret_cast<double*>(reinterpret_cast<uintptr_t>(tg.C) & ~uintptr_t(7));
    if (first) beta = 0.0;
    const int blk = unit % 9, bi = blk / 3, bj = blk % 3;
    GlobalCF64 Ag = (GlobalCF64)tg.A + (size_t)bi * 48 * NB;
    GlobalCF64 Bg = (GlobalCF64)tg.B + (size_t)bj * 48 * NB;
    GlobalF64 C = (GlobalF64)tg.C + (size_t)bi * 48 * NB + bj * 48;
    const int tid = threadIdx.x, lane = tid & 63, w = tid >> 6;
    const int lr = lane & 15, lk = lane >> 4;
    double4_t acc[3];
#pragma unroll
    for (int j = 0; j < 3; ++j) acc[j] = (double4_t){0.0, 0.0, 0.0, 0.0};
    constexpr int C2 = KS / 2, NR = 48 * C2 / 192;
    static_assert(48 * C2 % 192 == 0 && NB % KS == 0, "staging loops assume whole rounds");
    f64x2_t ra[NR], rb[NR];
    auto gload = [&](int k0) {
#pragma unroll
        for (int i = 0; i < NR; ++i) {
            const int idx = tid + 192 * i, row = idx / C2, c2 = idx % C2;
            ra[i] = *reinterpret_cast<GlobalCF64x2>(Ag + (size_t)row * NB + k0 + 2 * c2);
            rb[i] = *reinterpret_cast<GlobalCF64x2>(Bg + (size_t)row * NB + k0 + 2 * c2);
        }
    };
    double cv[3][4];
    if (beta != 0.0) {
#pragma unroll
        for (int j = 0; j < 3; ++j)
#pragma unroll
            for (int r = 0; r < 4; ++r) cv[j][r] = C[(size_t)(16 * w + lk + 4 * r) * NB + 16 * j + lr];
    }
    gload(0);
    for (int k0 = 0; k0 < NB; k0 += KS) {
        __syncthreads();
#pragma unroll
        for (int i = 0; i < NR; ++i) {
            const int idx = tid + 192 * i, row = idx / C2, c2 = idx % C2;
            sA[row * PS + 2 * c2] = ra[i].x; sA[row * PS + 2 * c2 + 1] = ra[i].y;
            sB[row * PS + 2 * c2] = rb[i].x; sB[row * PS + 2 * c2 + 1] = rb[i].y;
        }
        __syncthreads();
        if (k0 + KS < NB) gload(k0 + KS);
#pragma unroll
        for (int kk = 0; kk < KS; kk += 4) {
            const double a = sA[(16 * w + lr) * PS + kk + lk];
#pragma unroll
            for (int j = 0; j < 3; ++j) {
                const double b = sB[(16 * j + lr) * PS + kk + lk];
                acc[j] = __builtin_amdgcn_mfma_f64_16x16x4f64(a, b, acc[j], 0, 0, 0);
            }
        }
    }
#pragma unroll
    for (int j = 0; j < 3; ++j)
#pragma unroll
        for (int r = 0; r < 4; ++r) {
            const double v = alpha * acc[j][r];
            C[(size_t)(16 * w + lk + 4 * r) * NB + 16 * j + lr] = (beta != 0.0) ? v + beta * cv[j][r] : (first ? v + 0.0 : v);
        }
}

__global__ __launch_bounds__(576) void k_tile_gemm_nt_small_strip(const GemmTask* __restrict__ tasks, int n_units, double alpha,
                                                                    double beta) {
    __shared__ double sA[48 * PS];
    __shared__ double sB[NB * PS];
    const int unit = blockIdx.x;
    if (unit >= n_units) return;
    const GemmTask tg = tasks[unit / 3];
    const int bi = unit % 3;
    GlobalCF64 Ag = (GlobalCF64)tg.A + (size_t)bi * 48 * NB;
    GlobalCF64 Bg = (GlobalCF64)tg.B;
    GlobalF64 C = (GlobalF64)tg.C + (size_t)bi * 48 * NB;
    const int tid = threadIdx.x, lane = tid & 63, w = tid >> 6;
    const int lr = lane & 15, lk = lane >> 4;
    const int wr = w / 3, wc = w % 3;
    double4_t acc[3];
#pragma unroll
    for (int j = 0; j < 3; ++j) acc[j] = (double4_t){0.0, 0.0, 0.0, 0.0};
    constexpr int C2 = KS / 2, NRA = 48 * C2 / 576, NRB = NB * C2 / 576;
    static_assert(48 * C2 % 576 == 0 && NB * C2 % 576 == 0, "staging loops assume whole rounds");
    f64x2_t ra[NRA], rb[NRB];
    auto gload = [&](int k0) {
#pragma unroll
        for (int i = 0; i < NRA; ++i) {
            const int idx = tid + 576 * i, row = idx / C2, c2 = idx % C2;
            ra[i] = *reinterpret_cast<GlobalCF64x2>(Ag + (size_t)row * NB + k0 + 2 * c2);
        }
#pragma unroll
        for (int i = 0; i < NRB; ++i) {
            const int idx = tid + 576 * i, row = idx / C2, c2 = idx % C2;
            rb[i] = *reinterpret_cast<GlobalCF64x2>(Bg + (size_t)row * NB + k0 + 2 * c2);
        }
    };
    gload(0);
    for (int k0 = 0; k0 < NB; k0 += KS) {
        __syncthreads();
#pragma unroll
        for (int i = 0; i < NRA; ++i) {
            const int idx = tid + 576 * i, row = idx / C2, c2 = idx % C2;
            sA[row * PS + 2 * c2] = ra[i].x; sA[row * PS + 2 * c2 + 1] = ra[i].y;
        }
#pragma unroll
        for (int i = 0; i < NRB; ++i) {
            const int idx = tid + 576 * i, row = idx / C2, c2 = idx % C2;
            sB[row * PS + 2 * c2] = rb[i].x; sB[row * PS + 2 * c2 + 1] = rb[i].y;
        }
        __syncthreads();
        if (k0 + KS < NB) gload(k0 + KS);
#pragma unroll
        for (int kk = 0; kk < KS; kk += 4) {
            const double a = sA[(16 * wr + lr) * PS + kk + lk];
#pragma unroll
            for (int j = 0; j < 3; ++j) {
                const double b = sB[(48 * wc + 16 * j + lr) * PS + kk + lk];
                acc[j] = __builtin_amdgcn_mfma_f64_16x16x4f64(a, b, acc[j], 0, 0, 0);
            }
        }
    }
#pragma unroll
    for (int j = 0; j < 3; ++j)
#pragma unroll
        for (int r = 0; r < 4; ++r) {
            GlobalF64 dst = C + (size_t)(16 * wr + lk + 4 * r) * NB + 48 * wc + 16 * j + lr;
            const double v = alpha * acc[j][r];
            *dst = (beta != 0.0) ? v + beta * *dst : v;
        }
}

constexpr int HROWS = NB / 2;
constexpr int TP = NB + 1;

template <bool TRANS>
__device__ __forceinline__ void tile_gemv_lds(const double* __restrict__ M, const double* sv, double* sout, double* sT,
                                              double* spart, int tid) {
    double accT = 0.0;
    for (int h = 0; h < 2; ++h) {
        double2 reg[21];
#pragma unroll
        for (int i = 0; i < 21; ++i) {
            const int idx = tid + 256 * i;
            if (idx < HROWS * (NB / 2)) {
                const int row = idx / (NB / 2), c2 = idx - row * (NB / 2);
                reg[i] = *reinterpret_cast<const double2*>(M + (size_t)(HROWS * h + row) * NB + 2 * c2);
            }
        }
        __syncthreads();
// ... 264 lines not shown
        }
        spart[g][c] = v;
        __syncthreads();
        if (tid < NB) {
            const double* __restrict__ bsrc = t.src == -2 ? fold_b : b;
            const double rhs = bsrc ? bsrc[(size_t)t.dst * NB + tid] : 0.0;
            const double val = rhs - ((spart[0][tid] + spart[1][tid]) + (spart[2][tid] + spart[3][tid]));
            if (t.src == -2) fold_out[(size_t)t.dst * NB + tid] = val;
            else sx[tid] = val;
        }
        if (t.src == -2) return;
    }
    __syncthreads();
    double acc[kFwdRows];
    matvec(m, acc);
    if (cl == 15) {
        double* __restrict__ o = (t.src >= 0 ? part + (size_t)t.part * NB : y + (size_t)t.dst * NB) + row0;
#pragma unroll
        for (int rr = 0; rr < kFwdRows; ++rr) flow_st(o + rr, acc[rr]);
    }
    flow_publish(t.src >= 0 ? cnt + t.dst : done + t.dst, tid);
}

__device__ __forceinline__ void flow_wait_ge(const int* ver, int flag, int want, int tid, int* err) {
    if (flag >= 0) flow_wait(ver + flag, want, tid, err);
}
__device__ __forceinline__ void flow_wait_unit(const int* ver, const FactorUnit& u, int tid, int* err) {
    const int f0 = u.wait_flag[0], f1 = u.wait_flag[1], f2 = u.wait_flag[2], w0 = u.wait_val[0], w1 = u.wait_val[1], w2 = u.wait_val[2];
    if (tid < 64) {
        const int f = tid == 0 ? f0 : (tid == 1 ? f1 : (tid == 2 ? f2 : -1));
        const int want = tid == 0 ? w0 : (tid == 1 ? w1 : w2);
        int spins = 0;
        for (;;) {
            const bool ok = f < 0 || __hip_atomic_load(ver + f, __ATOMIC_RELAXED, __HIP_MEMORY_SCOPE_AGENT) >= want;
            if (__all(ok)) break;
            const bool dead = tid == 3 && __hip_atomic_load(err, __ATOMIC_RELAXED, __HIP_MEMORY_SCOPE_AGENT) != 0;
            if (__any(dead)) break;
            __builtin_amdgcn_s_sleep(1);
            if (++spins > kFlowSpinLimit) { if (tid == 0) atomicOr(err, 1); break; }
        }
    }
    __syncthreads();
}

constexpr int kFlowFactorThreadsC = 768;
constexpr int kFlowPK = NB + 2;
__device__ __forceinline__ void flow_update_unit(const FactorUnit& u, double* __restrict__ sA, double* __restrict__ sB,
                                                 int* __restrict__ ver, int* __restrict__ err, unsigned long long* __restrict__ trace) {
    const int tid = threadIdx.x, lane = tid & 63, w = tid >> 6;
    const int lr = lane & 15, lk = lane >> 4;
    const int wr = w / 3, wc = w % 3;
    const int bi = u.strip / 3, bj = u.strip % 3;
    const __amdgpu_buffer_rsrc_t rC = coh_rsrc(u.C), rA = coh_rsrc(u.A), rB = coh_rsrc(u.B);
    flow_wait_unit(ver, u, tid, err);
    if (trace && tid == 0) trace[1] = wall_clock64();
    const bool act = tid < 576;
    double cv[4] = {0.0, 0.0, 0.0, 0.0};
    if (act && !(u.kind & kFlowFirstWriter)) {
#pragma unroll
        for (int r = 0; r < 4; ++r) cv[r] = coh_ld1(rC, (48 * bi + 16 * wr + lk + 4 * r) * NB + 48 * bj + 16 * wc + lr);
    }
    constexpr int C2 = NB / 2, NR = 48 * C2 / 576;
    static_assert(48 * C2 % 576 == 0, "staging loops assume whole rounds");
    if (act) {
        double2 ra[NR], rb[NR];
#pragma unroll
        for (int i = 0; i < NR; ++i) {
            const int idx = tid + 576 * i, row = idx / C2, c2 = idx % C2;
            ra[i] = tile_ld2<true>(u.A, rA, (48 * bi + row) * NB + 2 * c2);
            rb[i] = tile_ld2<true>(u.B, rB, (48 * bj + row) * NB + 2 * c2);
        }
#pragma unroll
        for (int i = 0; i < NR; ++i) {
            const int idx = tid + 576 * i, row = idx / C2, c2 = idx % C2;
            sA[row * kFlowPK + 2 * c2] = ra[i].x; sA[row * kFlowPK + 2 * c2 + 1] = ra[i].y;
            sB[row * kFlowPK + 2 * c2] = rb[i].x; sB[row * kFlowPK + 2 * c2 + 1] = rb[i].y;
        }
    }
    __syncthreads();
    if (act) {
        double4_t acc = (double4_t){0.0, 0.0, 0.0, 0.0};
        const double* pa = sA + (16 * wr + lr) * kFlowPK + lk;
        const double* pb = sB + (16 * wc + lr) * kFlowPK + lk;
#pragma unroll
        for (int kk = 0; kk < NB; kk += 4) acc = __builtin_amdgcn_mfma_f64_16x16x4f64(pa[kk], pb[kk], acc, 0, 0, 0);
#pragma unroll
        for (int r = 0; r < 4; ++r)
            coh_st1(rC, (48 * bi + 16 * wr + lk + 4 * r) * NB + 48 * bj + 16 * wc + lr, -1.0 * acc[r] + 1.0 * cv[r]);
    }
    flow_publish(ver + u.pub, tid);
}

__device__ __forceinline__ void flow_solve_unit(const FactorUnit& u, double* __restrict__ sA, double* __restrict__ sB,
                                                int* __restrict__ ver, int* __restrict__ err, unsigned long long* __restrict__ trace) {
    const int tid = threadIdx.x, lane = tid & 63, w = tid >> 6;
    const int lr = lane & 15, lk = lane >> 4;
    const int row0 = 16 * u.strip;
    const __amdgpu_buffer_rsrc_t rC = coh_rsrc(u.C), rB = coh_rsrc(u.B);
    constexpr int C2 = KS / 2, NCH = NB / KS, NRB = NB * C2 / 576;
    static_assert(NB * C2 % 576 == 0 && 16 * C2 <= 576, "staging loops assume whole rounds");
    flow_wait_unit(ver, u, tid, err);
    if (trace && tid == 0) trace[1] = wall_clock64();
    const bool act = tid < 576;
    double2 ra[NCH], rb[NCH][NRB];
#pragma unroll
    for (int c = 0; c < NCH; ++c)
        if (tid < 16 * C2) ra[c] = tile_ld2<true>(u.C, rC, (row0 + tid / C2) * NB + KS * c + 2 * (tid % C2));
    if (act) {
#pragma unroll
        for (int c = 0; c < NCH; ++c)
#pragma unroll
            for (int i = 0; i < NRB; ++i) {
                const int idx = tid + 576 * i, row = idx / C2, c2 = idx % C2;
                rb[c][i] = tile_ld2<true>(u.B, rB, row * NB + KS * c + 2 * c2);
            }
    }
    double4_t acc = (double4_t){0.0, 0.0, 0.0, 0.0};
#pragma unroll
    for (int c = 0; c < NCH; ++c) {
        __syncthreads();
        if (tid < 16 * C2) { const int row = tid / C2, c2 = tid % C2; sA[row * PS + 2 * c2] = ra[c].x; sA[row * PS + 2 * c2 + 1] = ra[c].y; }
        if (act) {
#pragma unroll
            for (int i = 0; i < NRB; ++i) {
                const int idx = tid + 576 * i, row = idx / C2, c2 = idx % C2;
                sB[row * PS + 2 * c2] = rb[c][i].x; sB[row * PS + 2 * c2 + 1] = rb[c][i].y;
            }
        }
        __syncthreads();
        if (act) {
#pragma unroll
            for (int kk = 0; kk < KS; kk += 4)
                acc = __builtin_amdgcn_mfma_f64_16x16x4f64(sA[lr * PS + kk + lk], sB[(16 * w + lr) * PS + kk + lk], acc, 0, 0, 0);
        }
    }
    if (act) {
#pragma unroll
        for (int r = 0; r < 4; ++r) coh_st1(rC, (row0 + lk + 4 * r) * NB + 16 * w + lr, acc[r]);
    }
    flow_publish(ver + u.pub, tid);
}


__device__ __forceinline__ void flow_update_tile_unit(const FactorUnit& u, double* __restrict__ sA, double* __restrict__ sB,
                                                      int* __restrict__ ver, int* __restrict__ err, unsigned long long* __restrict__ trace) {
    const int tid = threadIdx.x, lane = tid & 63, w = tid >> 6;
    const int lr = lane & 15, lk = lane >> 4;
    const __amdgpu_buffer_rsrc_t rC = coh_rsrc(u.C), rA = coh_rsrc(u.A), rB = coh_rsrc(u.B);
    flow_wait_unit(ver, u, tid, err);
    if (trace && tid == 0) trace[1] = wall_clock64();
    constexpr int NBW = 7;
    const int nb = w < 9 ? 7 : 6, b0 = w < 9 ? 7 * w : 63 + 6 * (w - 9);
    constexpr int C2 = KS / 2, NCH = NB / KS;
    constexpr int NLD = (NB * C2 + kFlowFactorThreadsC - 1) / kFlowFactorThreadsC;
    double2 ra[NLD], rb[NLD];
    auto load_chunk = [&](int c) {
#pragma unroll
        for (int i = 0; i < NLD; ++i) {
            const int idx = tid + kFlowFactorThreadsC * i, row = min(idx / C2, NB - 1), c2 = idx % C2;
            ra[i] = tile_ld2<true>(u.A, rA, row * NB + KS * c + 2 * c2);
            rb[i] = tile_ld2<true>(u.B, rB, row * NB + KS * c + 2 * c2);
        }
    };
    load_chunk(0);
    double4_t acc[NBW];
#pragma unroll
    for (int q = 0; q < NBW; ++q) acc[q] = (double4_t){0.0, 0.0, 0.0, 0.0};
    double cv[NBW][4];
#pragma unroll
    for (int c = 0; c < NCH; ++c) {
        __syncthreads();
#pragma unroll
        for (int i = 0; i < NLD; ++i) {
            const int idx = tid + kFlowFactorThreadsC * i, row = idx / C2, c2 = idx % C2;
            if (idx < NB * C2) {
                sA[row * PS + 2 * c2] = ra[i].x; sA[row * PS + 2 * c2 + 1] = ra[i].y;
                sB[row * PS + 2 * c2] = rb[i].x; sB[row * PS + 2 * c2 + 1] = rb[i].y;
            }
        }
        if (c + 1 < NCH) {
            load_chunk(c + 1);
        } else {
            const bool first = (u.kind & kFlowFirstWriter) != 0;
#pragma unroll
            for (int q = 0; q < NBW; ++q) {
                const int b = min(b0 + q, 80), br = b / 9, bc = b - 9 * br;
#pragma unroll
                for (int r = 0; r < 4; ++r) cv[q][r] = first ? 0.0 : coh_ld1(rC, (16 * br + lk + 4 * r) * NB + 16 * bc + lr);
            }
        }
        __syncthreads();
#pragma unroll
        for (int q = 0; q < NBW; ++q) {
            if (q < nb) {
                const int b = b0 + q, br = b / 9, bc = b - 9 * br;
                const double* pa = sA + (16 * br + lr) * PS + lk;
                const double* pb = sB + (16 * bc + lr) * PS + lk;
#pragma unroll
                for (int kk = 0; kk < KS; kk += 4) acc[q] = __builtin_amdgcn_mfma_f64_16x16x4f64(pa[kk], pb[kk], acc[q], 0, 0, 0);
            }
        }
    }
#pragma unroll
    for (int q = 0; q < NBW; ++q) {
        if (q < nb) {
            const int b = b0 + q, br = b / 9, bc = b - 9 * br;
#pragma unroll
            for (int r = 0; r < 4; ++r) coh_st1(rC, (16 * br + lk + 4 * r) * NB + 16 * bc + lr, -1.0 * acc[q][r] + 1.0 * cv[q][r]);
        }
    }
    __builtin_amdgcn_s_waitcnt(0);
    __syncthreads();
    if (tid == 0) __hip_atomic_fetch_add(ver + u.pub, kFlowUnitsPerTile, __ATOMIC_RELAXED, __HIP_MEMORY_SCOPE_AGENT);
}

constexpr int kFlowFactorThreads = 768;
__global__ __launch_bounds__(kFlowFactorThreads) void k_factor_flow(const FactorUnit* __restrict__ units, int* __restrict__ ver,
                                                                     int* __restrict__ fail, int* __restrict__ err,
                                                                     unsigned long long* __restrict__ trace) {
    __shared__ double smem[(NLB + NBK) * BSZ];
    __shared__ int bad, sync_cnt;
    static_assert((16 + NB) * PS <= (NLB + NBK) * BSZ && 2 * 48 * kFlowPK <= (NLB + NBK) * BSZ && 2 * NB * PS <= (NLB + NBK) * BSZ, "the products' staging areas fit in the potrf's");
    static_assert(kFlowFactorThreadsC == kFlowFactorThreads, "one constant");
    const FactorUnit u = units[blockIdx.x];
    const int tid = threadIdx.x;
    if (trace) {
        trace += 3 * (size_t)blockIdx.x;
        if (tid == 0) trace[0] = wall_clock64();
    }
    const int kind = u.kind & 15;
    if (kind == 0) {
        flow_wait_unit(ver, u, tid, err);
        if (trace && tid == 0) trace[1] = wall_clock64();
        potrf_tile_mf<kFlowFactorThreads / 64, true>(u.C, const_cast<double*>(u.A), u.strip, fail, smem, smem + NLB * BSZ, &bad, &sync_cnt);
        __builtin_amdgcn_s_waitcnt(0);
        __syncthreads();
        if (tid == 0) __hip_atomic_fetch_add(ver + u.pub, kFlowUnitsPerTile, __ATOMIC_RELAXED, __HIP_MEMORY_SCOPE_AGENT);
    } else if (kind == 1) {
        flow_solve_unit(u, smem, smem + 16 * PS, ver, err, trace);
    } else if (kind == 3) {
        flow_update_tile_unit(u, smem, smem + NB * PS, ver, err, trace);
    } else {
        flow_update_unit(u, smem, smem + 48 * kFlowPK, ver, err, trace);
    }
    if (trace && tid == 0) trace[2] = wall_clock64();
}

__global__ __launch_bounds__(256) void k_tile_diag(const double* __restrict__ tiles, const int* __restrict__ diag_slot,
                                                     int nt, double* __restrict__ diag) {
    const int i = blockIdx.x * 256 + threadIdx.x;
    if (i >= nt * NB) return;
    const int I = i / NB, r = i - I * NB;
    diag[i] = tiles[(size_t)diag_slot[I] * (NB * NB) + (size_t)r * NB + r];
}

__global__ __launch_bounds__(256) void k_tile_add_diag(double* __restrict__ tiles, const int* __restrict__ diag_slot,
                                                         int n_valid, int n_total, double add_valid, double set_pad) {
    const int i = blockIdx.x * 256 + threadIdx.x;
    if (i >= n_total) return;
    const int I = i / NB, r = i - I * NB;
    double* d = tiles + (size_t)diag_slot[I] * (NB * NB) + (size_t)r * NB + r;
    if (i < n_valid) { if (add_valid != 0.0) *d += add_valid; }
    else *d = set_pad;
}

__global__ __launch_bounds__(256) void k_tile_scale_sym(const SymTile* __restrict__ list, double* __restrict__ tiles,
                                                          const double* __restrict__ scale) {
    const SymTile t = list[blockIdx.x];
    double* T = tiles + (size_t)t.slot * (NB * NB);
    const double* sr = scale + (size_t)t.I * NB;
    const double* sc = scale + (size_t)t.J * NB;
    for (int e = threadIdx.x; e < NB * NB; e += 256) {
        const int r = e / NB, c = e - r * NB;
        T[e] *= sr[r] * sc[c];
    }
}

__global__ __launch_bounds__(256) void k_vec_select(int n, const double* __restrict__ in, const int* __restrict__ cls, int mask,
                                                      double* __restrict__ out) {
    const int i = blockIdx.x * 256 + threadIdx.x;
    if (i < n) out[i] = ((mask >> cls[i / NB]) & 1) ? in[i] : 0.0;
}
__global__ __launch_bounds__(256) void k_vec_merge(int n, const double* __restrict__ src, const int* __restrict__ cls, int mask,
                                                     double* __restrict__ dst) {
    const int i = blockIdx.x * 256 + threadIdx.x;
    if (i < n && ((mask >> cls[i / NB]) & 1)) dst[i] = src[i];
}

__global__ __launch_bounds__(64) void k_gate(const int* __restrict__ arrived, int expected, long long max_ticks) {
    if (threadIdx.x != 0) return;
    const long long t0 = wall_clock64();
    while (__hip_atomic_load(arrived, __ATOMIC_RELAXED, __HIP_MEMORY_SCOPE_AGENT) < expected && wall_clock64() - t0 < max_ticks)
        __builtin_amdgcn_s_sleep(16);
}
void launch_gate(const int* arrived, int expected, int max_micros, hipStream_t s) {
    hipLaunchKernelGGL(k_gate, dim3(1), dim3(64), 0, s, arrived, expected, (long long)max_micros * 100);
}
void launch_factor_flow(const FactorUnit* units, int n_units, int* ver, int* fail, int* err, hipStream_t s, unsigned long long* trace) {
    if (n_units <= 0) return;
    hipLaunchKernelGGL(k_factor_flow, dim3(n_units), dim3(kFlowFactorThreads), 0, s, units, ver, fail, err, trace);
}
void launch_potrf_inv(const PotrfTask* tasks, int n, int* fail, hipStream_t s, int* arrived) {
    if (n <= 0) return;
    hipLaunchKernelGGL(k_potrf_inv_mf<12>, dim3(n), dim3(768), 0, s, tasks, fail, arrived);
}
void launch_tile_gemm_nt(const GemmTask* tasks, int n, double alpha, double beta, hipStream_t s, bool tri_b) {
    if (n <= 0) return;
    if (n <= kGemmSmallMax) {
        if (beta != 0.0) hipLaunchKernelGGL(k_tile_gemm_nt_small, dim3(9 * n), dim3(192), 0, s, tasks, 9 * n, alpha, beta);
        else hipLaunchKernelGGL(k_tile_gemm_nt_small_strip, dim3(3 * n), dim3(576), 0, s, tasks, 3 * n, alpha, beta);
        return;
    }
    const int units = n * NSTRIP, per_xcd = (units + 7) / 8;
    if (tri_b) hipLaunchKernelGGL(k_tile_gemm_nt<true>, dim3(8 * per_xcd), dim3(256), 0, s, tasks, units, alpha, beta);
    else hipLaunchKernelGGL(k_tile_gemm_nt<false>, dim3(8 * per_xcd), dim3(256), 0, s, tasks, units, alpha, beta);
}
void launch_tri_step(bool trans, const TriTask* tasks, int n, double* vwork, double* vout, hipStream_t s) {
    if (n <= 0) return;
    const int grid = 8 * ((n + 7) / 8);
    if (trans) hipLaunchKernelGGL(k_tri_step<true>, dim3(grid), dim3(256), 0, s, tasks, n, vwork, vout);
    else hipLaunchKernelGGL(k_tri_step<false>, dim3(grid), dim3(256), 0, s, tasks, n, vwork, vout);
}
__global__ __launch_bounds__(256) void k_occupy_cu(long long ticks_100mhz, int* started) {
    __shared__ char hog[156 * 1024];
    if (threadIdx.x == 0) {
        hog[blockIdx.x & 1023] = 1;
        __hip_atomic_fetch_add(started, 1, __ATOMIC_RELAXED, __HIP_MEMORY_SCOPE_SYSTEM);
        const long long t0 = (long long)__builtin_amdgcn_s_memrealtime();
        while ((long long)__builtin_amdgcn_s_memrealtime() - t0 < ticks_100mhz) __builtin_amdgcn_s_sleep(32);
        if (hog[(blockIdx.x + 7) & 1023] == 77) started[1] = 1;
    }
    __syncthreads();
}
void launch_occupy_cus(int n, int micros, int* started, hipStream_t s) {
    if (n > 0) hipLaunchKernelGGL(k_occupy_cu, dim3(n), dim3(256), 0, s, (long long)micros * 100, started);
}

__global__ __launch_bounds__(256) void k_clear_i32(int* __restrict__ p, int64_t n) {
    for (int64_t i = (int64_t)blockIdx.x * 256 + threadIdx.x; i < n; i += (int64_t)gridDim.x * 256) p[i] = 0;
}
void launch_clear_i32(int* p, int64_t n, hipStream_t s) {
    if (n <= 0) return;
    hipLaunchKernelGGL(k_clear_i32, dim3((unsigned)std::min<int64_t>(64, (n + 255) / 256)), dim3(256), 0, s, p, n);
}
__global__ void k_post_word(int* __restrict__ word, int* __restrict__ host_word) {
    const int v = word[0];
    if (v != 0) { host_word[0] = v; word[0] = 0; }
}
void launch_post_word(int* word, int* host_word_dev, hipStream_t s) { hipLaunchKernelGGL(k_post_word, dim3(1), dim3(1), 0, s, word, host_word_dev); }

void launch_tri_flow(bool backward, const FlowTask* tasks, int n_tasks, const double* in, double* out, double* part, int* flags,
                     int nt, hipStream_t s, const double* fold_b, double* fold_out, int poison_block, bool keep_flags) {
    if (n_tasks <= 0) return;
    if (!keep_flags) launch_clear_i32(flags, (int64_t)2 * nt, s);
    if (poison_block >= 0 && poison_block < nt)
        (void)hipMemsetD32Async(reinterpret_cast<hipDeviceptr_t>(flags + poison_block), (int)0x80000000, 1, s);
    int* err = flags + 2 * nt;
    if (backward) hipLaunchKernelGGL(k_tri_bwd_flow, dim3(n_tasks), dim3(kBwdThreads), 0, s, tasks, in, out, part, flags, flags + nt, err);
    else hipLaunchKernelGGL(k_tri_fwd_flow, dim3(n_tasks), dim3(kFwdThreads), 0, s, tasks, in, out, part, flags, flags + nt, err, fold_b, fold_out);
}
void launch_tile_diag(const double* tiles, const int* diag_slot, int nt, double* diag, hipStream_t s) {
    hipLaunchKernelGGL(k_tile_diag, dim3((nt * NB + 255) / 256), dim3(256), 0, s, tiles, diag_slot, nt, diag);
}
void launch_tile_add_diag(double* tiles, const int* diag_slot, int n_valid, int n_total, double add_valid,
                          double set_pad, hipStream_t s) {
    hipLaunchKernelGGL(k_tile_add_diag, dim3((n_total + 255) / 256), dim3(256), 0, s, tiles, diag_slot, n_valid, n_total, add_valid, set_pad);
}
void launch_vec_select(int n, const double* in, const int* cls, int mask, double* out, hipStream_t s) {
// ... 14 lines not shown
```

### apex-solver_amd/csrc/factor_schedule.cpp

```cpp
#include "factor_schedule.h"

#include <algorithm>

namespace apex {

std::vector<SchedOp> factor_schedule(const ScheduleInput& in, int g0, int g1) {
    const std::vector<Level>& lv_ = in.lv;
    std::vector<SchedOp> ops;
    auto launch = [&](StreamId s, int list, int64_t first, int64_t n, int arrive = -1) {
        if (n > 0) ops.push_back({kOpLaunch, (uintptr_t)s, 0, list, first, (int)n, arrive});
    };
    auto wait = [&](StreamId s, int lv, LevelEvent k) { ops.push_back({kOpWait, (uintptr_t)s, (uintptr_t)lv * kLevelEvents + k, -1, 0, 0, -1}); };
    auto record = [&](int lv, LevelEvent k, StreamId s) { ops.push_back({kOpRecord, (uintptr_t)s, (uintptr_t)lv * kLevelEvents + k, -1, 0, 0, -1}); };
    auto potrf = [&](int lv) { launch(kMain, 0, lv_[lv].potrf, lv_[lv + 1].potrf - lv_[lv].potrf, in.gate_min > 0 ? lv : -1); };
    auto panel = [&](int lv) { launch(kMain, 1, lv_[lv].panel, lv_[lv + 1].panel - lv_[lv].panel); };
    auto updates = [&](int r0, int r1, StreamId s) {
        for (int r = r0; r < r1; ++r) launch(s, 2, in.upd_rounds[r].first, in.upd_rounds[r].second);
    };
    auto gate = [&](int lv, StreamId s) { ops.push_back({kOpGate, (uintptr_t)s, 0, -1, lv + 1, lv_[lv + 2].potrf - lv_[lv + 1].potrf, -1}); };
    const bool two = in.overlap && in.n_levels > 2;
    const int ph = (g0 == in.n_local_groups && g1 == in.n_levels && in.n_local_groups < in.n_levels) ? 1 : 0;
    const ScheduleInput::Flow& flow = in.flow[ph];
    const int g_end = g1;
    if (in.flow_on && flow.n > 0 && flow.g0 >= g0 && flow.g1 == g1) g1 = flow.g0;
    if (in.gate_min > 0) ops.push_back({kOpClearGates, kMain, 0, -1, 0, in.n_levels + 1, -1});
    int last_a = -1, last_b = -1;
    std::vector<int> lastb((size_t)std::max(g1 - g0, 1), -1);
    bool u2_pending = false, o_pending = false;
    int b2_pending = -1, a_waited = -1;
    auto a_wait_upto = [&](int lvb) {
        if (lvb > a_waited) { wait(kSide, lvb, kEvB2); a_waited = lvb; }
    };
    for (int lv = g0; lv < g1; ++lv) {
        potrf(lv);
        if (lv > g0 && o_pending) wait(kMain, lv - 1, kEvO);
        const int r0 = lv_[lv].upd, rd = lv_[lv].u1o, rs = lv_[lv].u2a, r1 = lv_[lv + 1].upd;
        int64_t n_u2 = 0, n_o = 0;
        for (int r = rs; r < r1; ++r) n_u2 += in.upd_rounds[r].second;
        for (int r = rd; r < rs; ++r) n_o += in.upd_rounds[r].second;
        const bool has_u2 = two && n_u2 >= in.overlap_min;
        const bool has_o = two && in.split_u1 && n_o >= in.split_u1_min;
        panel(lv);
        if (has_u2 || has_o) record(lv, kEvT, kMain);
        if (has_u2) wait(kSide, lv, kEvT);
        if (has_o) wait(kSo, lv, kEvT);
        if (two && lv > g0 && u2_pending) {
            wait(kMain, lv - 1, kEvU2);
            if (has_o) wait(kSo, lv - 1, kEvU2);
        } else if (two && lv > g0 && !in.skip_idle_wait) {
            if (last_a >= 0) {
                wait(kMain, last_a, kEvB);
                if (has_o) wait(kSo, last_a, kEvB);
                last_a = -1;
            }
            if (last_b >= 0) {
                wait(kMain, last_b, kEvB2);
                if (has_o) wait(kSo, last_b, kEvB2);
                last_b = -1;
            }
        }
        updates(r0, rd, kMain);
        updates(rd, rs, has_o ? kSo : kMain);
        o_pending = has_o;
        if (has_o) record(lv, kEvO, kSo);
        const bool b2_side = has_u2 && in.two_side_plan && r1 > lv_[lv].u2b2;
        const bool gated = has_u2 && in.gate_min > 0 && n_u2 >= in.gate_min && lv + 1 < g1;
        if (gated) gate(lv, kSide);
        if (!has_u2 && r1 > rs) {
            if (last_a >= 0) { wait(kMain, last_a, kEvB); last_a = -1; }
            if (last_b >= 0) { wait(kMain, last_b, kEvB2); last_b = -1; }
        }
        const int ra = lv_[lv].u2b1, rb = lv_[lv].u2b2;
        const StreamId sa = has_u2 ? kSide : kMain, sb = b2_side ? kSide2 : sa;
        if (has_u2 && lv - 2 >= g0) a_wait_upto(lastb[lv - 2 - g0]);
        updates(rs, ra, sa);
        u2_pending = has_u2;
        if (has_u2) record(lv, kEvU2, kSide);
        if (b2_side) {
            wait(kSide2, lv, kEvT);
            if (gated) gate(lv, kSide2);
        }
        if (has_u2 && lv - 1 >= g0) a_wait_upto(lastb[lv - 1 - g0]);
        updates(ra, rb, sa);
        updates(rb, r1, sb);
        if (has_u2) { record(lv, kEvB, kSide); last_a = lv; }
        if (b2_side) { record(lv, kEvB2, kSide2); last_b = lv; }
        lastb[lv - g0] = b2_pending = b2_side ? lv : b2_pending;
    }
    if (g1 > g0 && o_pending) wait(kMain, g1 - 1, kEvO);
    if (last_a >= 0) wait(kMain, last_a, kEvB);
    if (last_b >= 0) wait(kMain, last_b, kEvB2);
    if (g1 < g_end) {
        ops.push_back({kOpClearVersions, kMain, 0, -1, flow.first, flow.n, -1});
        launch(kMain, 3, flow.first, flow.n);
    }
    return ops;
}

int check_schedule(const std::vector<SchedOp>& ops, const std::vector<PotrfTask>& potrf, const std::vector<GemmTask>& panel,
                   const std::vector<GemmTask>& upd, const std::vector<FactorUnit>& units, std::string* first_violation) {
    std::vector<uintptr_t> streams;
    auto sid = [&](uintptr_t s) { for (size_t i = 0; i < streams.size(); ++i) if (streams[i] == s) return (int)i; streams.push_back(s); return (int)streams.size() - 1; };
    auto orders = [](const SchedOp& o) { return o.op == kOpLaunch || o.op == kOpRecord || o.op == kOpWait; };
    for (const SchedOp& o : ops) if (orders(o)) (void)sid(o.stream);
    const int S = (int)streams.size();
    typedef std::vector<int> Clock;
    std::vector<Clock> now((size_t)S, Clock((size_t)S, 0));
    std::vector<std::pair<uintptr_t, Clock>> events;
    struct Access { int launch; bool write; };
    struct Launch { int stream, pos; Clock before; const SchedOp* op; };
    std::vector<Launch> launches;
    std::vector<std::pair<const double*, Access>> acc;
    int bad = 0;
    auto complain = [&](const std::string& m) { if (bad++ == 0 && first_violation) *first_violation = m; };
// ... 63 lines not shown
```

### apex-solver_amd/csrc/factor_schedule.h

```cpp
#pragma once
#include <stdint.h>

#include <string>
#include <utility>
#include <vector>

#include "tile_tasks.h"

namespace apex {

enum StreamId { kMain, kSide, kSide2, kSo };
enum LevelEvent { kEvT, kEvU2, kEvO, kEvB, kEvB2, kLevelEvents };

enum SchedKind {
    kOpLaunch = 0,
    kOpRecord = 1,
    kOpWait = 2,
    kOpGate = 3,
    kOpClearGates = 4,
    kOpClearVersions = 5,
};

struct SchedOp {
    int op;
    uintptr_t stream;
    uintptr_t event;
    int list;
    int64_t first;
    int count;
    int arrive;
};

struct Level { int potrf = 0, panel = 0, fwd = 0, upd = 0, u1o = 0, u2a = 0, u2b1 = 0, u2b2 = 0; std::vector<int> fwd_cut; };

struct ScheduleInput {
    const std::vector<Level>& lv;
    const std::vector<std::pair<int64_t, int64_t>>& upd_rounds;
    int n_levels, n_local_groups;
    bool overlap; int overlap_min;
    bool split_u1; int split_u1_min;
    bool two_side_plan;
    int gate_min;
    bool skip_idle_wait;
    bool flow_on;
    struct Flow { int g0, g1, first, n; } flow[2];
};

std::vector<SchedOp> factor_schedule(const ScheduleInput& in, int g0, int g1);

int check_schedule(const std::vector<SchedOp>& ops, const std::vector<PotrfTask>& potrf, const std::vector<GemmTask>& panel,
                   const std::vector<GemmTask>& upd, const std::vector<FactorUnit>& units, std::string* first_violation);

}
```

### apex-solver_amd/csrc/plan_lists.cpp

```cpp
#include "plan_lists.h"

#include <math.h>
#include <stdio.h>
#include <stdlib.h>

#include <algorithm>
#include <iterator>
#include <numeric>

#include "host_parallel.h"

namespace apex {

namespace {
constexpr int kTriInline = 8;

double* tile_at(double* base, int64_t i) { return base + (size_t)i * kNB * kNB; }

void nested_dissection(const std::vector<std::vector<int>>& adj, std::vector<int> nodes, std::vector<int>& out,
                              int leaf) {
    std::sort(nodes.begin(), nodes.end());
    if ((int)nodes.size() <= leaf) { out.insert(out.end(), nodes.begin(), nodes.end()); return; }
    const int n = (int)adj.size();
    std::vector<int> mark(n, -1), dist(n, -1);
// ... 610 lines not shown
                }, 1);
                for (size_t i = 0; i < c1 - c0 && !past; ++i) {
                    if (!errs[i].empty()) return errs[i];
                    const double gain = cands[c0 + i].second - (sims[i] + 15.0);
                    if (gain > best_total) { best_total = gain; best_gf = cands[c0 + i].first; }
                    else if (gain < best_total - 300.0) past = true;
                }
            }
        }
        if (g1 - best_gf < 2) continue;
        std::vector<FactorUnit> best_units;
        double sim = 0.0;
        const std::string e = flow_units(s, best_gf, g1, tiles, linv, &best_units, &sim);
        if (!e.empty()) return e;
        fl.g0 = best_gf; fl.n = (int)best_units.size(); fl.sim_us = sim;
        out->units.insert(out->units.end(), best_units.begin(), best_units.end());
    }
    return "";
}

void flag_first_writers(const PlanStructure& s, const double* tiles, PlanLists* out) {
    const PlanLists::Flow* flow = out->flow;
    out->first_ok = false;
    if (s.distributed() || s.n_slots <= s.n_touched || flow[1].n != 0) return;
    auto slot_of_ptr = [&](const double* c) { return (int64_t)((c - tiles) / (ptrdiff_t)(kNB * kNB)); };
    std::vector<char> seen_a((size_t)s.n_slots, 0);
    for (int64_t sl = 0; sl < s.n_touched; ++sl) seen_a[(size_t)sl] = 1;
    std::vector<char> seen_b(seen_a);
    int64_t upd_before_flow = (int64_t)out->upd.size();
    if (flow[0].n > 0) {
        const int r = out->lv[(size_t)flow[0].g0].upd;
        if (r < (int)out->upd_rounds.size()) upd_before_flow = out->upd_rounds[(size_t)r].first;
    }
    for (size_t q = 0; q < out->upd.size(); ++q) {
        const int64_t sl = slot_of_ptr(out->upd[q].C);
        if ((int64_t)q < upd_before_flow) seen_b[(size_t)sl] = 1;
        if (!seen_a[(size_t)sl]) { seen_a[(size_t)sl] = 1; out->upd[q].C = reinterpret_cast<double*>(reinterpret_cast<uintptr_t>(out->upd[q].C) | 1); }
    }
    std::vector<const double*> first_a((size_t)s.n_slots, nullptr), first_b((size_t)s.n_slots, nullptr);
    for (FactorUnit& u : out->units) {
        if (u.kind != 2 && u.kind != 3) continue;
        const int64_t sl = slot_of_ptr(u.C);
        if (!seen_b[(size_t)sl]) { seen_b[(size_t)sl] = 1; first_a[(size_t)sl] = u.A; first_b[(size_t)sl] = u.B; }
        if (first_a[(size_t)sl] == u.A && first_b[(size_t)sl] == u.B && first_a[(size_t)sl] != nullptr) u.kind |= kFlowFirstWriter;
    }
    bool all = true;
    for (int64_t sl = s.n_touched; sl < s.n_slots; ++sl) all = all && seen_a[(size_t)sl] && (flow[0].n == 0 || seen_b[(size_t)sl]);
    if (all) out->first_ok = true;
    else {
        for (GemmTask& t : out->upd) t.C = reinterpret_cast<double*>(reinterpret_cast<uintptr_t>(t.C) & ~uintptr_t(7));
        for (FactorUnit& u : out->units) u.kind &= 15;
    }
}
}

std::string build_plan_lists(const PlanStructure& s, const std::vector<uint8_t>& present, const PlanOptions& o, double* tiles, double* linv, PlanLists* out) {
    *out = PlanLists();
    if (s.refused) return s.message;
    level_lists(s, tiles, linv, out);
    sweep_lists(s, tiles, linv, out);
    sym_lists(s, present, out);
    out->two_side_plan = o.two_side == 2 || (o.two_side == 1 && (int64_t)out->upd.size() >= 256 * (int64_t)s.n_levels());
    const std::string e = flow_regions(s, o.flow_cols, o.flow_rows, tiles, linv, out);
    if (e.empty()) flag_first_writers(s, tiles, out);
    return e;
}

}
```

### apex-solver_amd/csrc/plan_lists.h

```cpp
#pragma once
#include <stdint.h>

#include <string>
#include <utility>
#include <vector>

#include "factor_schedule.h"
#include "tile_tasks.h"

namespace apex {

constexpr uintptr_t kStandInTiles = uintptr_t(1) << 44, kStandInLinv = uintptr_t(1) << 45;

struct PlanOptions {
    int rank = 0, world = 1;
    bool own_all = false;
    int two_side = 1;
    int flow_cols = -1, flow_rows = 24;
    int64_t max_updates = 80000000LL;
    double cost_limit_ms = 0.0;
};

using PlanCols = std::vector<std::vector<int>>;

struct PlanStructure {
    int nt = 0;
    PlanCols col_rows;
    std::vector<int> cls;
    std::vector<int> owner;
    int n_top_cols = 0;
    double local_frac = 1.0;
    std::vector<int> slot, diag_slot;
    std::vector<std::pair<int64_t, int64_t>> own_range, own_fill;
    int64_t n_t_nt = 0, n_f_nt = 0, n_slots = 0, n_touched = 0;
    int64_t n_potrf = 0, n_trsm = 0, n_upd = 0;
    int n_true_levels = 0, n_local_groups = 0;
    PlanCols group_cols, row_cols;
    std::vector<int> group_of;
    double predicted_ms = 0.0;
    int refused = 0;
    std::string message;

    int n_levels() const { return (int)group_cols.size(); }
    bool distributed() const { return n_local_groups < n_levels(); }
    int slot_of(int I, int J) const { return slot[(size_t)I * nt + J]; }
};

struct PlanLists {
    std::vector<PotrfTask> potrf;
    std::vector<GemmTask> panel, upd;
    std::vector<std::pair<int64_t, int64_t>> upd_rounds;
    std::vector<Level> lv;
    std::vector<int> bwd_step;
    std::vector<TriTask> fwd, bwd;
    std::vector<FlowTask> flow_fwd, flow_bwd;
    int n_flow_local = 0;
    int n_flow_parts = 0;
    std::vector<int> sym_row_ptr; std::vector<SymEntry> sym_entries; std::vector<SymTile> sym_tiles;
    std::vector<FactorUnit> units;
    struct Flow { int g0 = 0, g1 = 0, first = 0, n = 0; double sim_us = 0.0; } flow[2];
    bool two_side_plan = false;
    bool first_ok = false;
};

struct ScheduleSwitches {
    bool overlap = true;
    int overlap_min = 2;
    bool split_u1 = true;
    int split_u1_min = 4;
    int gate_min = 256;
    bool skip_idle_wait = false;
    bool flow_on = true;
};
inline ScheduleInput schedule_input(const PlanStructure& s, const PlanLists& l, const ScheduleSwitches& w) {
    const PlanLists::Flow* f = l.flow;
    return ScheduleInput{l.lv, l.upd_rounds, s.n_levels(), s.n_local_groups, w.overlap, w.overlap_min, w.split_u1, w.split_u1_min, l.two_side_plan,
                         w.gate_min, w.skip_idle_wait, w.flow_on, {{f[0].g0, f[0].g1, f[0].first, f[0].n}, {f[1].g0, f[1].g1, f[1].first, f[1].n}}};
}

std::vector<int> tile_order(int nt, const std::vector<uint8_t>& adj, bool nested_dissection, int leaf, int n_fixed_last = 1);

double predict_solve_ms(int64_t n_potrf, int64_t n_trsm, int64_t n_upd, int64_t n_tiles, int n_levels);

PlanStructure plan_structure(int nt, const std::vector<uint8_t>& present, const PlanOptions& opts);

std::vector<int> plan_owners(int nt, const std::vector<uint8_t>& present, int world);

std::string build_plan_lists(const PlanStructure& s, const std::vector<uint8_t>& present, const PlanOptions& opts, double* tiles,
                             double* linv, PlanLists* out);

}
```

### apex-solver_amd/csrc/tile_backend.h

```cpp
#pragma once
#include <hip/hip_runtime.h>
#include <stdint.h>

#include <initializer_list>
#include <string>

#include "column_map.h"
#include "device_buffer.h"
#include "dogleg_kernels.h"
#include "dogleg_scalars.hpp"
#include "jacobi_scaling.h"
#include "lm_loop.h"
#include "stage_timer.h"
#include "step_state.h"
#include "tile_plan.h"
#include "tr_loop.h"

namespace apex {

#define HIP_TRY(expr, ...)                                    \
    do {                                                      \
        int _rc = check_hip((expr), #expr, ##__VA_ARGS__);    \
        if (_rc != kOk) return _rc;                           \
    } while (0)

class TileBackend : public TrBackend {
   public:
    void enable_graphs(bool on) { tp_.enable_graphs(on); }
    void enable_overlap(bool on) { tp_.enable_overlap(on); }
    void enable_tri_flow(bool on) { tp_.enable_tri_flow(on); }
    int sweep_timeouts() const { return tp_.sweep_timeouts(); }
    void debug_poison_next_solve(int which) { tp_.debug_poison_next_solve(which); }
    void debug_poison_next_factor() { tp_.debug_poison_next_factor(); }
    void set_split_u1(int min_tasks) { tp_.set_split_u1(min_tasks); }
    void set_overlap_min(int n) { tp_.set_overlap_min(n); }
    void set_gate_min(int n) { tp_.set_gate_min(n); }
    void set_two_side(int mode) { tp_.set_two_side(mode); }
    void set_factor_flow(int max_cols, int max_rows) { tp_.set_factor_flow(max_cols, max_rows); }
    int factor_flow_timeouts() const { return n_factor_flow_timeouts_; }
    void set_one_wait(bool on) { one_wait_ = on; }
    void set_eager_step_eval(bool on) { eager_eval_ = on; }
    void set_nd(bool on, int leaf) { use_nd_ = on; if (leaf > 0) nd_leaf_ = leaf; }
    void enable_covariance_timing(bool on) { tp_.inverse().enable_timing(on); }
    void enable_stage_timing(bool on) { timer_.enable(on); }
    void enable_stage_timing_only(uint32_t stage_mask) { timer_.enable_only(stage_mask); }
    void reset_stage_times() { timer_.reset(); }
    int stage_times(double* ms, int64_t* launches) { return timer_.times(ms, launches); }
    int n_levels() const { return tp_.n_levels(); }
    const TilePlan& plan() const { return tp_; }
    const char* last_error() const override { return err_.c_str(); }
    int step_stats(double out3[3]) final;
    int eval_step(double* trial_cost) final;
    int commit_step() final;
    int discard_step() final;
    int dogleg_step(double mu, double radius, int reuse, DoglegStepInfo* out) final;

   protected:
    TileBackend(int device, int n_stages, int nd_leaf, int stats_stage, int n_partial)
        : device_(device), nd_leaf_(nd_leaf), timer_(n_stages), n_partial_(n_partial), stats_stage_(stats_stage) {}
    int fail(int code, const std::string& msg) { err_ = msg; return code; }
    int check_hip(hipError_t e, const char* what, std::string* err = nullptr);
    void begin_solve(double lambda) { st_.begin_solve(); last_lambda_ = lambda; }
    int enqueue_eager_eval();
    void post_eager_answers() { st_.post_answers(answers_from_sums(eager_host_)); }
    int answers_of_step(bool trial, StepAnswers* out);
    int direct_solve(bool speculative, double lambda, double* step_out, double* grad_out);
    int factor_fresh(double lambda, double reg, int* failed);
    int factor_again(double lambda, double reg, int* failed);
    enum class ExportAs { kPlain, kStep, kGradient };
    struct ExportSegment { const double* dev; const ColumnMap* map; const JacobiScaling* scale; };
    int export_columns(std::initializer_list<ExportSegment> segs, ExportAs as, double* out);
    int export_tiles_dense(const ColumnMap& map, int64_t ld, int64_t slot_bound, double* out);

    virtual int rebuild_system(double lambda, double reg) = 0;
    virtual int factor_now(int* failed, bool defer_flags) = 0;
    virtual int enqueue_sweeps() = 0;
    virtual int finish_step(double* step_out, double* grad_out) = 0;
    virtual int recover_factor(double lambda, int failed, bool gave_up) = 0;
    virtual const int* own_flag() const { return nullptr; }
    virtual int own_flag_raised() { return kOk; }
    virtual void keep_factor() { tp_.set_factor_valid(true); }
    virtual int enqueue_step_stats() = 0;
    virtual int enqueue_trial_point(double* sumsq_out) = 0;
    virtual int enqueue_retract(int from, double sign, int to) = 0;
    virtual bool keeps_current_on_discard() const { return false; }
    virtual double* step_sums(int* n) = 0;
    virtual StepAnswers answers_from_sums(const double* h) const = 0;
    virtual void params_moved() {}
    virtual int dogleg_refusal() = 0;
    virtual int dogleg_segments(DlSegment out[2]) = 0;
    virtual void enqueue_jv_gram(const double* const a[2], const double* const b[2], double* out3) = 0;
    virtual int solve_for_dogleg(double mu) = 0;
    virtual void dogleg_trial_begins() {}

    int enqueue_dogleg_tail(bool fresh);
    int jv_gram_columns(const double* a, const double* b, double out3[3]);
    void drop_dogleg_cache() { have_dl_cache_ = false; }
    void release_dogleg_buffers() { for (int k = 0; k < 2; ++k) { dl_h_[k].reset(); dl_a_[k].reset(); } dls_.reset(); }

    int device_;
    StepState st_;
    double last_lambda_ = 0.0;
    bool one_wait_ = true, eager_eval_ = true;
    bool scaled_ = false;
    int n_factor_flow_timeouts_ = 0;
    bool use_nd_ = true;
    int nd_leaf_;
    std::string err_;
    hipStream_t stream_ = nullptr;
    struct StreamLast { hipStream_t& s; ~StreamLast() { if (s) (void)hipStreamDestroy(s); } } stream_last_{stream_};
    TilePlan tp_;
    StageTimer timer_;
    PinnedBuffer<double> eager_host_;
    DeviceBuffer<double> partial_;
    const int n_partial_;
    bool dl_mode_ = false;

   private:
    const int stats_stage_;
    DeviceBuffer<double> dl_h_[2], dl_a_[2];
    DeviceBuffer<DoglegScalars> dls_;
    PinnedBuffer<DoglegScalars> dl_host_;
    DeviceBuffer<double> jv_out_;
    double dl_radius_ = 0.0;
    bool have_dl_cache_ = false;
// ... 4 lines not shown
```

### apex-solver_amd/csrc/tile_backend.hip

```cpp
#include "tile_backend.h"

#include <stddef.h>

#include <vector>

namespace apex {

int TileBackend::check_hip(hipError_t e, const char* what, std::string* err) {
    if (e == hipSuccess) return kOk;
    *(err ? err : &err_) = std::string("HIP error in ") + what + ": " + hipGetErrorString(e);
    return kDeviceError;
}

int TileBackend::factor_again(double lambda, double reg, int* failed) {
    ++n_factor_flow_timeouts_;
    int rc = rebuild_system(lambda, reg);
    if (rc == kOk) rc = factor_now(failed, false);
    if (rc == kOk && tp_.factor_flow_gave_up()) return fail(kDeviceError, "dataflow factorisation timed out twice");
    return rc;
}

int TileBackend::factor_fresh(double lambda, double reg, int* failed) {
    const int rc = factor_now(failed, false);
    return (rc != kOk || !tp_.factor_flow_gave_up()) ? rc : factor_again(lambda, reg, failed);
// ... 19 lines not shown
                rc = recover_factor(lambda, failed, gave_up);
                attempt = -1;
                continue;
            }
        }
        if (!tp_.sweep_timed_out()) { keep_factor(); return kOk; }
        st_.invalidate_step();
        if (attempt > 0 || !tp_.tri_flow()) return fail(kDeviceError, "triangular sweep timed out");
        tp_.enable_tri_flow(false);
    }
    return rc;
}

int TileBackend::export_columns(std::initializer_list<ExportSegment> segs, ExportAs as, double* out) {
    std::vector<std::vector<double>> h;
    for (const ExportSegment& sg : segs) {
        h.emplace_back((size_t)sg.map->size());
        HIP_TRY(hipMemcpyAsync(h.back().data(), sg.dev, h.back().size() * sizeof(double), hipMemcpyDeviceToHost, stream_));
    }
    HIP_TRY(hipStreamSynchronize(stream_));
    size_t k = 0;
    for (const ExportSegment& sg : segs) {
        const double* v = h[k++].data();
        const double* s = (scaled_ && as != ExportAs::kPlain) ? sg.scale->host.data() : nullptr;
        if (!s) sg.map->scatter(v, out, 0.0);
        else if (as == ExportAs::kStep) sg.map->scatter(v, out, 0.0, [s](double x, int64_t i) { return x / s[i]; });
        else sg.map->scatter(v, out, 0.0, [s](double x, int64_t i) { return x * s[i]; });
    }
    return kOk;
}

int TileBackend::export_tiles_dense(const ColumnMap& map, int64_t ld, int64_t slot_bound, double* out) {
    const size_t tile_elems = (size_t)kNB * kNB;
    const int64_t n = map.size();
    std::vector<double> t(tile_elems);
    for (int I = 0; I < tp_.nt(); ++I)
        for (int J = 0; J <= I; ++J) {
            const int s = tp_.slot(I, J);
            if (s < 0 || s >= slot_bound) continue;
            HIP_TRY(hipMemcpyAsync(t.data(), tp_.tiles() + (size_t)s * tile_elems, tile_elems * sizeof(double), hipMemcpyDeviceToHost, stream_));
            HIP_TRY(hipStreamSynchronize(stream_));
            for (int r = 0; r < kNB; ++r)
                for (int c = 0; c < kNB; ++c) {
                    const int64_t gi = (int64_t)I * kNB + r, gj = (int64_t)J * kNB + c;
                    if (gi >= n || gj >= n || gj > gi) continue;
                    const double val = t[(size_t)r * kNB + c];
                    out[map.col[gi] * ld + map.col[gj]] = val;
                    out[map.col[gj] * ld + map.col[gi]] = val;
                }
        }
    return kOk;
}

int TileBackend::enqueue_eager_eval() {
    if (!eager_host_) HIP_TRY(eager_host_.alloc(8));
    int n = 0;
    double* sums = step_sums(&n);
    int rc = enqueue_step_stats();
    if (rc == kOk) rc = enqueue_trial_point(sums + n);
    if (rc != kOk) return rc;
    HIP_TRY(hipMemcpyAsync(eager_host_, sums, (n + 1) * sizeof(double), hipMemcpyDeviceToHost, stream_));
    return kOk;
}

int TileBackend::answers_of_step(bool trial, StepAnswers* out) {
    const StepAnswers* posted = nullptr;
    if (const Status rc = trial ? st_.ask_trial(&posted) : st_.ask_stats(&posted)) return fail(rc, st_.refusal);
    if (posted) { *out = *posted; return kOk; }
    HIP_TRY(hipSetDevice(device_));
    int n = 0;
    double* sums = step_sums(&n);
    if (trial) st_.trial_written();
    const int rc = trial ? enqueue_trial_point(sums + n) : enqueue_step_stats();
    if (rc != kOk) return rc;
    HIP_TRY(hipGetLastError());
    double h[8] = {};
    HIP_TRY(hipMemcpyAsync(h + (trial ? n : 0), sums + (trial ? n : 0), (trial ? 1 : n) * sizeof(double), hipMemcpyDeviceToHost, stream_));
    HIP_TRY(hipStreamSynchronize(stream_));
    *out = answers_from_sums(h);
    return kOk;
}
int TileBackend::step_stats(double out3[3]) {
    StepAnswers a;
    const int rc = answers_of_step(false, &a);
    if (rc == kOk) { out3[0] = a.gradient_norm; out3[1] = a.step_norm; out3[2] = a.predicted_reduction; }
    return rc;
}
int TileBackend::eval_step(double* trial_cost) {
    StepAnswers a;
    const int rc = answers_of_step(true, &a);
    if (rc == kOk) *trial_cost = cost_from_sumsq(a.trial_sumsq);
    return rc;
}
int TileBackend::commit_step() {
    if (const Status rc = st_.commit()) return fail(rc, st_.refusal);
    params_moved();
    return kOk;
}
int TileBackend::discard_step() {
    if (const Status rc = st_.begin_discard()) return fail(rc, st_.refusal);
    HIP_TRY(hipSetDevice(device_));
    if (!keeps_current_on_discard()) {
        const int rc = enqueue_retract(st_.cur ^ 1, -1.0, st_.cur);
        if (rc != kOk) return rc;
    }
    HIP_TRY(hipStreamSynchronize(stream_));
// ... 93 lines not shown
```

### apex-solver_amd/csrc/tile_plan.h

```cpp
#pragma once
#include <hip/hip_runtime.h>
#include <stdint.h>

#include <array>
#include <functional>
#include <string>
#include <utility>
#include <vector>

#include "chol_kernels.h"
#include "device_buffer.h"
#include "factor_schedule.h"
#include "plan_lists.h"
#include "tile_pcg.h"
#include "tile_sinv.h"

namespace apex {

struct TilePlanMemory {
    DeviceBuffer<double> tiles_, linv_;
    DeviceBuffer<int> slot_, diag_slot_, flag_;
    DeviceBuffer<int> cls_;
    DeviceBuffer<double> exch_;
    DeviceBuffer<int> gate_cnt_;
    DeviceBuffer<PotrfTask> potrf_tasks_;
    DeviceBuffer<GemmTask> trsm_tasks_, upd_tasks_;
    DeviceBuffer<TriTask> tri_fwd_, tri_bwd_;
    DeviceBuffer<FlowTask> flow_fwd_, flow_bwd_;
    DeviceBuffer<double> flow_part_;
    DeviceBuffer<int> flow_flags_;
    PinnedBuffer<int> flow_err_host_;
    DeviceBuffer<FactorUnit> flow_units_;
    DeviceBuffer<int> flow_ver_;
    DeviceBuffer<unsigned long long> flow_trace_;
    DeviceBuffer<SymTile> sym_tiles_;
};

class TilePlan : private TilePlanMemory {
   public:
    TilePlan() = default;
    ~TilePlan();
    TilePlan(const TilePlan&) = delete;
    TilePlan& operator=(const TilePlan&) = delete;

    std::string build(int nt, const std::vector<uint8_t>& present, hipStream_t stream);

    struct Comm {
        std::function<bool(double* buf, size_t n, hipStream_t stream)> sum;
        std::function<bool(int* buf, size_t n, hipStream_t stream)> max_int;
    };
    void set_partition(int rank, int world) { opts_.rank = rank; opts_.world = world; }
    void set_own_all(bool on) { opts_.own_all = on; }
    void set_comm(Comm c) { comm_ = std::move(c); }
    bool distributed() const { return structure_.distributed(); }
    int n_top_columns() const { return structure_.n_top_cols; }
    double local_work_fraction() const { return structure_.local_frac; }
    int64_t n_reduce_slots() const { return distributed() ? structure_.n_t_nt : structure_.n_touched; }
    int part_world() const { return opts_.world; }
    std::pair<int64_t, int64_t> owner_slot_range(int o) const { return structure_.own_range[o]; }
    void top_slot_ranges(std::pair<int64_t, int64_t> out[2]) const;
    void factor_phase(int phase);
    int* flag_dev() const { return flag_; }
    void solve_phase(int phase, const double* rhs, double* x, double* work);
    double* exch_buffer() const { return exch_; }

    int nt() const { return structure_.nt; }
    int64_t n_pad() const { return (int64_t)structure_.nt * kNB; }
    int64_t n_slots() const { return structure_.n_slots; }
    int64_t n_touched_slots() const { return structure_.n_touched; }
    int n_levels() const { return structure_.n_levels(); }
    const std::vector<std::vector<int>>& group_columns() const { return structure_.group_cols; }
    void op_counts(int64_t* potrf, int64_t* trsm, int64_t* upd) const { *potrf = (int64_t)lists_.potrf.size(); *trsm = (int64_t)lists_.panel.size(); *upd = (int64_t)lists_.upd.size(); }
    double* tiles() const { return tiles_; }
    const double* linv() const { return linv_; }
    const int* slot_host() const { return structure_.slot.data(); }
    int slot(int I, int J) const { return structure_.slot_of(I, J); }
    TileMap tilemap() const { return TileMap{tiles_, slot_, structure_.nt}; }
    const int* diag_slot_dev() const { return diag_slot_; }
    void enable_graphs(bool on) { use_graphs_ = on; }
    void enable_overlap(bool on) { sw_.overlap = on; }
    void set_overlap_min(int n) { sw_.overlap_min = n; }
    void set_two_side(int mode) { opts_.two_side = mode; }
    void set_gate_min(int n) { sw_.gate_min = n; }
    void set_factor_flow(int max_cols, int max_rows) { opts_.flow_cols = max_cols; if (max_rows > 0) opts_.flow_rows = max_rows; }
    int factor_flow_groups() const { return !sw_.flow_on ? 0 : (lists_.flow[0].g1 - lists_.flow[0].g0) + (lists_.flow[1].g1 - lists_.flow[1].g0); }
    int factor_flow_cols() const { return opts_.flow_cols; }
    double factor_flow_sim_us() const { return lists_.flow[0].sim_us + lists_.flow[1].sim_us; }
    int factor_flow_units() const { return lists_.flow[0].n + lists_.flow[1].n; }
    hipError_t enable_flow_trace();
    hipError_t read_flow_trace(std::vector<FactorUnit>* units, std::vector<unsigned long long>* stamps);
    bool refused_too_large() const { return refused_ == 1; }
    bool refused_no_memory() const { return refused_ == 2; }
    bool refused_by_cost() const { return refused_ == 3; }
    double predicted_ms() const { return structure_.predicted_ms; }
    void set_cost_limit_ms(double ms) { opts_.cost_limit_ms = ms; }
    void set_max_updates(int64_t n) { opts_.max_updates = n > 0 ? n : PlanOptions().max_updates; }
    bool factor_flow_gave_up() { const bool g = flow_gave_up_; flow_gave_up_ = false; return g; }
    void set_split_u1(int min_tasks) { sw_.split_u1 = min_tasks > 0; if (min_tasks > 0) sw_.split_u1_min = min_tasks; }
    hipError_t read_flags(int* failed_at);
    void enable_tri_flow(bool on);
    bool tri_flow() const { return tri_flow_; }
    bool sweep_timed_out();
    bool sweep_timed_out_peek() const { return flow_err_host_ && flow_err_host_[0] != 0; }
    int sweep_timeouts() const { return n_sweep_timeouts_; }
    void debug_poison_next_solve(int which) { poison_ = which; }
    void debug_poison_next_factor() { poison_factor_ = true; }
    hipError_t debug_occupy_cus(int n_cus, int micros);

    hipError_t zero_tiles(bool own_touched_only = false, bool skip_fill = false);
    bool first_writers_flagged() const { return lists_.first_ok; }
    void add_diag(int n_valid, double add_valid, double pad_value);
    void diag(double* out) const;
    void scale_sym(const double* scale);
    hipError_t factor(int* failed_at, bool defer_flags = false);
    hipError_t solve(const double* rhs, double* x, double* work);
    void sym_matvec(const double* x, double* y) { pcg_.matvec(x, y); }
    hipError_t pcg(const double* rhs, double* x, double* work, int max_iter, double tol, int* iters) { tiles_written(); return pcg_.solve(rhs, x, work, max_iter, tol, iters); }
    const double* pcg_scalars() const { return pcg_.scalars(); }

    void set_factor_valid(bool on) { factor_valid_ = on; ++factor_epoch_; }
    bool factor_valid() const { return factor_valid_; }
    SelectedInverse& inverse();
    const SelectedInverse& inverse() const { return inverse_; }

   private:
    std::string refuse_by_memory();
    std::string upload();
    ScheduleInput input() const;
    void issue(const std::vector<SchedOp>& ops);
    void enqueue_factor(int g0, int g1) { issue(factor_schedule(input(), g0, g1)); }
    void enqueue_solve(const double* rhs, double* x, double* work);
    void launch_fwd_group(int lv, double* bvec, double* yvec, hipStream_t s);
    void enqueue_dist_solve(int phase, const double* rhs, double* x, double* work);
    bool run_graph(int which, const double* rhs, double* x, double* work);
    void release();
// ... 39 lines not shown
```

### apex-solver_amd/csrc/tile_plan.hip

```cpp
#include "tile_plan.h"
#include "host_parallel.h"

#include <chrono>
#include <thread>

#include <stdlib.h>

#include <algorithm>

namespace apex {

void TilePlan::release() {
    for (int i = 0; i < kGraphs; ++i) {
        if (graph_exec_[i]) { (void)hipGraphExecDestroy(graph_exec_[i]); graph_exec_[i] = nullptr; }
        graph_failed_[i] = false;
    }
    inverse_.release();
    pcg_.release();
    tiles_written();
    static_cast<TilePlanMemory&>(*this) = TilePlanMemory();
    lists_ = PlanLists(); sw_.flow_on = true; flow_gave_up_ = false;
    flow_err_host_dev_ = nullptr;
    if (occ_stream_) { (void)hipStreamSynchronize(occ_stream_); (void)hipStreamDestroy(occ_stream_); occ_stream_ = nullptr; }
    for (const auto& evs : ev_) for (hipEvent_t e : evs) if (e) (void)hipEventDestroy(e);
// ... 73 lines not shown
    TP_TRY(hipDeviceSynchronize());
    return "";
}
#undef TP_TRY

hipError_t TilePlan::zero_tiles(bool own_touched_only, bool skip_fill) {
    tiles_written();
    const size_t te = (size_t)kNB * kNB * sizeof(double);
    hipError_t e = hipSuccess;
    auto clear = [&](int64_t first, int64_t count) {
        if (e == hipSuccess && count > 0) e = hipMemsetAsync(tiles_ + (size_t)first * kNB * kNB, 0, (size_t)count * te, stream_);
    };
    if (distributed() && !opts_.own_all && opts_.rank < (int)structure_.own_range.size()) {
        if (own_touched_only) { clear(structure_.own_range[opts_.rank].first, structure_.own_range[opts_.rank].second); clear(structure_.n_t_nt, structure_.n_touched - structure_.n_t_nt); }
        else clear(0, structure_.n_touched);
        clear(structure_.own_fill[opts_.rank].first, structure_.own_fill[opts_.rank].second);
        clear(structure_.n_f_nt, structure_.n_slots - structure_.n_f_nt);
    } else {
        clear(0, (skip_fill && lists_.first_ok) ? structure_.n_touched : structure_.n_slots);
    }
    if (e != hipSuccess) return e;
    launch_clear_i32(flag_, 4, stream_);
    return hipGetLastError();
}

void TilePlan::add_diag(int n_valid, double add_valid, double pad_value) {
    tiles_written();
    launch_tile_add_diag(tiles_, diag_slot_, n_valid, (int)n_pad(), add_valid, pad_value, stream_);
}

void TilePlan::scale_sym(const double* scale) { tiles_written(); launch_tile_scale_sym(sym_tiles_, n_sym_tiles(), tiles_, scale, stream_); }

void TilePlan::diag(double* out) const { launch_tile_diag(tiles_, diag_slot_, structure_.nt, out, stream_); }

void TilePlan::launch_fwd_group(int lv, double* bvec, double* yvec, hipStream_t s) {
    const std::vector<int>& cut = lists_.lv[lv].fwd_cut;
    if (cut.size() < 2) {
        launch_tri_step(false, tri_fwd_ + lists_.lv[lv].fwd, lists_.lv[lv + 1].fwd - lists_.lv[lv].fwd, bvec, yvec, s);
        return;
    }
    for (size_t i = 0; i < cut.size(); ++i) {
        const int b = cut[i], e = i + 1 < cut.size() ? cut[i + 1] : lists_.lv[lv + 1].fwd;
        launch_tri_step(false, tri_fwd_ + b, e - b, bvec, yvec, s);
    }
}

ScheduleInput TilePlan::input() const { return schedule_input(structure_, lists_, sw_); }

void TilePlan::issue(const std::vector<SchedOp>& ops) {
    for (const SchedOp& o : ops) {
        const hipStream_t s = stream_of(o.stream);
        switch (o.op) {
            case kOpLaunch:
                if (o.list == 0) launch_potrf_inv(potrf_tasks_ + o.first, o.count, flag_, s, o.arrive >= 0 ? gate_cnt_ + o.arrive : nullptr);
                else if (o.list == 1) launch_tile_gemm_nt(trsm_tasks_ + o.first, o.count, 1.0, 0.0, s, true);
                else if (o.list == 2) launch_tile_gemm_nt(upd_tasks_ + o.first, o.count, -1.0, 1.0, s);
                else launch_factor_flow(flow_units_ + o.first, o.count, flow_ver_, flag_, flag_ + 1, s, flow_trace_ ? flow_trace_ + 3 * (size_t)o.first : nullptr);
                break;
            case kOpRecord: (void)hipEventRecord(ev_[o.event / kLevelEvents][o.event % kLevelEvents], s); break;
            case kOpWait: (void)hipStreamWaitEvent(s, ev_[o.event / kLevelEvents][o.event % kLevelEvents], 0); break;
            case kOpGate: launch_gate(gate_cnt_ + o.first, o.count, 150, s); break;
            case kOpClearGates: launch_clear_i32(gate_cnt_, o.count, s); break;
            case kOpClearVersions:
                launch_clear_i32(flow_ver_, structure_.n_slots, s);
                if (poison_factor_)
                    (void)hipMemsetAsync(flow_ver_ + lists_.units[(size_t)o.first].pub, 0x80, sizeof(int), s);
                break;
        }
    }
}

void TilePlan::enqueue_solve(const double* rhs, double* x, double* work) {
    double* bvec = work;
    double* yvec = work + n_pad();
    const bool flow = tri_flow_ && n_flow_fwd() > 0;
    if (flow) {
        launch_tri_flow(false, flow_fwd_, n_flow_fwd(), rhs, yvec, flow_part_, flow_flags_, structure_.nt, stream_, nullptr, nullptr,
                        poison_ == 1 ? structure_.nt - 1 : -1);
    } else {
        (void)hipMemcpyAsync(bvec, rhs, n_pad() * sizeof(double), hipMemcpyDeviceToDevice, stream_);
        for (int lv = 0; lv < structure_.n_levels(); ++lv)
            launch_fwd_group(lv, bvec, yvec, stream_);
    }
    if (flow) {
        launch_tri_flow(true, flow_bwd_, n_flow_bwd(), yvec, x, flow_part_, flow_flags_, structure_.nt, stream_, nullptr, nullptr,
                        poison_ == 2 ? structure_.nt - 1 : -1);
        return;
    }
    for (int s = 0; s < structure_.n_levels(); ++s)
        launch_tri_step(true, tri_bwd_ + lists_.bwd_step[s], lists_.bwd_step[s + 1] - lists_.bwd_step[s], yvec, x, stream_);
}

void TilePlan::enqueue_dist_solve(int phase, const double* rhs, double* x, double* work) {
    double* bvec = work;
    double* yvec = work + n_pad();
    const int n = (int)n_pad();
    const int L1 = structure_.n_local_groups;
    const bool flow = tri_flow_ && lists_.n_flow_local > 0;
    if (phase == 0 && flow) {
        (void)hipMemsetAsync(exch_, 0, n_pad() * sizeof(double), stream_);
        launch_tri_flow(false, flow_fwd_, lists_.n_flow_local, rhs, yvec, flow_part_, flow_flags_, structure_.nt, stream_,
                        opts_.rank == 0 ? rhs : nullptr, exch_);
    } else if (phase == 1 && flow) {
        launch_tri_flow(false, flow_fwd_ + lists_.n_flow_local, n_flow_fwd() - lists_.n_flow_local, exch_, yvec, flow_part_, flow_flags_, structure_.nt,
                        stream_, nullptr, nullptr);
        launch_tri_flow(true, flow_bwd_, n_flow_bwd(), yvec, x, flow_part_, flow_flags_, structure_.nt, stream_, nullptr, nullptr);
        launch_vec_select(n, x, cls_, opts_.rank == 0 ? 6 : 2, exch_, stream_);
    } else if (phase == 0) {
        launch_vec_select(n, rhs, cls_, opts_.rank == 0 ? 7 : 3, bvec, stream_);
// ... 179 lines not shown
```

### apex-solver_amd/csrc/tile_tasks.h

```cpp
#pragma once

namespace apex {

constexpr int kNB = 144;

struct GemmTask {
    double* C;
    const double* A;
    const double* B;
};

struct PotrfTask {
    double* A;
    double* Linv;
    int K;
};

constexpr int kFlowFirstWriter = 16;
constexpr int kFlowUnitsPerTile = 9;
struct FactorUnit {
    double* C;
    const double* A;
    const double* B;
    int wait_flag[3];
    int wait_val[3];
    int pub;
    int kind;
    int strip;
    int pad;
};

struct TriTask {
    const double* Mdiag;
    const double* Moff;
    int k;
    int other;
};

struct FlowTask {
    const double* mat;
    int src;
    int dst;
    int part;
    int count;
    const double* mat2 = nullptr;
    int src2 = -1;
    int slot2 = -1;
};

struct SymEntry {
    int slot;
    int other;
    int kind;
};

struct SymTile { int slot, I, J; };

constexpr int kSinvTransA = 1, kSinvTransB = 2, kSinvNeg = 4;
struct SinvProd {
    const double* A;
    const double* B;
    int op;
    int pad;
};
struct SinvTask {
    double* C;
    int first;
    int count;
};

}
// ... 1 lines not shown
```

### apex-solver_amd/pose_graph.py

```python
from __future__ import annotations

import ctypes as C
from dataclasses import dataclass, field

import numpy as np

from . import capi
from .loss import Loss, create_loss_function
from .synthetic import PoseGraphData

G2O_ERROR_NAMES = {-30: "Io", -31: "Parse", -32: "MissingFields", -33: "InvalidNumber", -34: "DuplicateVertex",
                   -35: "InvalidQuaternion"}


class G2oError(RuntimeError):

    def __init__(self, code: int, message: str):
        self.code = code
        self.kind = G2O_ERROR_NAMES.get(code, f"Error({code})")
        super().__init__(f"{self.kind}: {message}")


@dataclass
class G2oGraph:
# ... 419 lines not shown
    def commit_step(self): h = self._need(); h.check(h.L.apexgpu_pg_commit_step(h.h))
    def discard_step(self): h = self._need(); h.check(h.L.apexgpu_pg_discard_step(h.h))

    def parameter_norm(self) -> float:
        h = self._need()
        c = C.c_double()
        h.check(h.L.apexgpu_pg_parameter_norm(h.h, C.byref(c)))
        return c.value

    def get_residual(self) -> np.ndarray:
        h = self._need()
        r = np.zeros((h.n_edges, h.dof))
        h.check(h.L.apexgpu_pg_get_residual(h.h, capi.ptr(r)))
        return r

    def get_jacobian_blocks(self) -> np.ndarray:
        h = self._need()
        j = np.zeros((h.n_edges, h.dof, 2 * h.dof))
        h.check(h.L.apexgpu_pg_get_jacobian_blocks(h.h, capi.ptr(j)))
        return j

    def get_hessian(self, lam: float = 0.0):
        h = self._need()
        n = h.dof * h.n_vertices
        H = np.zeros((n, n)); g = np.zeros(n)
        h.check(h.L.apexgpu_pg_get_hessian(h.h, float(lam), capi.ptr(H), capi.ptr(g)))
        return H, g

    def pose_covariance_blocks(self) -> np.ndarray:
        h = self._need()
        out = np.zeros((h.n_vertices, h.dof, h.dof))
        h.check(h.L.apexgpu_pg_covariance(h.h, capi.ptr(out)))
        return out

    def compute_covariances(self) -> dict:
        blocks = self.pose_covariance_blocks()
        return {f"x{int(i)}": blocks[k].copy() for k, i in enumerate(self.problem.data.ids)}

    def covariance_stats(self, group_cap: int = 0) -> dict:
        from .solver import _covariance_stats
        h = self._need()
        return _covariance_stats(h, h.L.apexgpu_pg_covariance_stats, group_cap)

    def info(self) -> dict:
        h = self._need()
        a = (C.c_double * 8)()
        h.check(h.L.apexgpu_pg_info(h.h, C.byref(a)))
        return {"tile_rows": int(a[0]), "tiles": int(a[1]), "touched_tiles": int(a[2]), "etree_levels": int(a[3]),
                "total_dof": int(a[4]), "n_potrf": int(a[5]), "n_trsm": int(a[6]), "n_update": int(a[7])}

    def set_option(self, name: str, value: int):
        h = self._need(); h.check(h.L.apexgpu_pg_set_option(h.h, name.encode(), int(value)))

    def counters(self) -> dict:
        h = self._need(); out = (C.c_int64 * 4)()
        h.check(h.L.apexgpu_pg_counters(h.h, C.byref(out)))
        return dict(sweep_timeouts=int(out[0]), tri_dataflow=bool(out[1]), factor_flow_timeouts=int(out[2]), factor_flow_groups=int(out[3]))

    def enable_stage_timing(self, on=True): h = self._need(); h.check(h.L.apexgpu_pg_enable_stage_timing(h.h, int(on)))
    def reset_stage_times(self): h = self._need(); h.check(h.L.apexgpu_pg_reset_stage_times(h.h))

    def stage_times(self) -> dict:
        h = self._need()
        ms = (C.c_double * capi.PG_NUM_STAGES)(); n = (C.c_int64 * capi.PG_NUM_STAGES)()
        h.check(h.L.apexgpu_pg_stage_times(h.h, C.byref(ms), C.byref(n)))
        return {name: (ms[i], n[i]) for i, name in enumerate(capi.PG_STAGE_NAMES)}

    def lm_optimize(self, cfg):
        h = self._need()
        c = cfg.to_c()
        c.variant = 0
        res = capi.LmResultC()
        cap = cfg.max_iterations + 2
        hist = (capi.LmIterC * cap)()
        h.check(h.L.apexgpu_pg_lm_optimize(h.h, C.byref(c), C.byref(res), C.cast(hist, C.c_void_p), cap))
        n = res.iterations
        H = np.array([[getattr(hist[i], f) for f, _ in capi.LmIterC._fields_] for i in range(min(n, cap))])
        return res, H.reshape(-1, 8), c

    def gn_optimize(self, cfg: GaussNewtonConfig):
        h = self._need()
        c = cfg.to_c()
        res = capi.LmResultC()
        cap = cfg.max_iterations + 2
        hist = (capi.LmIterC * cap)()
        h.check(h.L.apexgpu_pg_gn_optimize(h.h, C.byref(c), C.byref(res), C.cast(hist, C.c_void_p), cap))
        H = np.array([[getattr(hist[i], f) for f, _ in capi.LmIterC._fields_] for i in range(min(res.iterations, cap))])
        return res, H.reshape(-1, 8), c

    def dogleg_optimize(self, cfg: DogLegConfig):
        h = self._need()
        c = cfg.to_c()
        res = capi.LmResultC()
        cap = cfg.max_iterations + 2
        hist = (capi.DlIterC * cap)()
        h.check(h.L.apexgpu_pg_dogleg_optimize(h.h, C.byref(c), C.byref(res), C.cast(hist, C.c_void_p), cap))
        H = np.array([[getattr(hist[i], f) for f, _ in capi.DlIterC._fields_] for i in range(min(res.iterations, cap))])
        return res, H.reshape(-1, 12), c

    def dogleg_step(self, mu: float, radius: float, reuse: bool = False) -> dict:
        h = self._need()
        o = (C.c_double * 8)()
        h.check(h.L.apexgpu_pg_dogleg_step(h.h, float(mu), float(radius), 1 if reuse else 0, C.byref(o)))
        return dict(gradient_norm=o[0], step_norm=o[1], predicted_reduction=o[2], step_type=int(o[3]), alpha=o[4], beta=o[5],
                    scaled_step_norm=o[6], reused=bool(o[7]))

# ... 15 lines not shown
```

### apex-solver_amd/solver.py

```python
from __future__ import annotations

import ctypes as C
import enum
from dataclasses import dataclass, field, replace

import numpy as np

from . import capi
from .layout import ColumnLayout, reference_column_layout
from .loss import Loss, create_loss_function
from .pose_graph import DogLegConfig
from .synthetic import BAProblemData


class LinearSolverType(enum.Enum):

    SparseCholesky = "SparseCholesky"
    SparseQR = "SparseQR"
    SparseSchurComplement = "SparseSchurComplement"
    DenseCholesky = "DenseCholesky"
    DenseQR = "DenseQR"
    GpuSchurComplement = "GpuSchurComplement"
    GpuSparseCholesky = "GpuSparseCholesky"

# ... 421 lines not shown
        return out

    def landmark_covariance_blocks(self) -> np.ndarray:
        h = self._need()
        out = np.zeros((h.n_pt, 3, 3))
        h.check(h.L.apexgpu_landmark_covariance(h.h, capi.ptr(out)))
        return out

    def compute_covariances(self, landmarks: bool = False) -> dict:
        out = camera_covariance_dict(self.camera_covariance_blocks())
        if landmarks:
            out.update(landmark_covariance_dict(self.landmark_covariance_blocks()))
        return out

    def covariance_stats(self, group_cap: int = 0) -> dict:
        h = self._need()
        return _covariance_stats(h, h.L.apexgpu_covariance_stats, group_cap)

    def landmark_covariance_stats(self) -> dict:
        h = self._need()
        out = (C.c_double * 4)()
        h.check(h.L.apexgpu_landmark_covariance_stats(h.h, C.byref(out)))
        return dict(extra_bytes=int(out[0]), pairs=int(out[1]), recomputed_z=bool(out[2]), landmark_ms=float(out[3]))

    def get_landmark_blocks(self):
        h = self._need()
        hi = np.zeros((h.n_pt, 3, 3)); gl = np.zeros((h.n_pt, 3))
        h.check(h.L.apexgpu_get_landmark_blocks(h.h, capi.ptr(hi), capi.ptr(gl)))
        return hi, gl

    def info(self) -> dict:
        h = self._need(); out = (C.c_double * 16)()
        h.check(h.L.apexgpu_info(h.h, C.byref(out)))
        return dict(tile_rows=int(out[0]), tiles=int(out[1]), pair_blocks=float(out[2]), cam_dof=int(out[3]),
                    last_reg=float(out[4]), pcg_iterations=int(out[5]), touched_tiles=int(out[6]), local_obs=int(out[7]), etree_levels=int(out[8]),
                    n_potrf=int(out[9]), n_trsm=int(out[10]), n_update=int(out[11]),
                    dist_top_columns=int(out[12]), dist_local_fraction=float(out[13]), tree_sharded=bool(out[14]), schur_form=int(out[15]))

    def variant_info(self, asked: "SchurVariant | None" = None) -> dict:
        h = self._need()
        asked = self.variant if asked is None else asked
        used = C.c_int(0); buf = C.create_string_buffer(512)
        h.check(h.L.apexgpu_variant_info(h.h, asked.value, C.byref(used), buf, 512))
        c = (C.c_double * 4)()
        h.check(h.L.apexgpu_variant_costs(h.h, C.byref(c)))
        return dict(variant_asked=asked.name, variant_used=SchurVariant(used.value).name, reason=buf.value.decode(),
                    predicted_direct_ms=float(c[0]), predicted_matrix_free_ms=float(c[1]),
                    variant_choice=("direct", "matrix-free by predicted cost", "matrix-free: plan refused", "matrix-free by option")[int(c[2])])

    def counters(self) -> dict:
        h = self._need(); out = (C.c_int64 * 4)()
        h.check(h.L.apexgpu_counters(h.h, C.byref(out)))
        return dict(sweep_timeouts=int(out[0]), tri_dataflow=bool(out[1]), factor_flow_timeouts=int(out[2]), factor_flow_groups=int(out[3]))

    def setup_times(self) -> dict:
        h = self._need(); sec = (C.c_double * 6)(); cnt = (C.c_double * 4)()
        h.check(h.L.apexgpu_setup_times(h.h, C.byref(sec), C.byref(cnt)))
        return dict(order=sec[0], lists=sec[1], tile_plan=sec[2], schur_lists=sec[3], uploads=sec[4], total=sec[5],
                    hub_cameras=int(cnt[0]), pair_blocks=int(cnt[1]), pair_slots=int(cnt[2]), schur_form=int(cnt[3]))

    def set_option(self, name: str, value: int):
        h = self._need(); h.check(h.L.apexgpu_set_option(h.h, name.encode(), int(value)))

    def pair_records(self) -> np.ndarray:
        h = self._need()
        n = self.setup_times()["pair_slots"]
        out = np.zeros((n, 4), dtype=np.uint32)
        h.check(h.L.apexgpu_debug_get_pair_records(h.h, capi.ptr(out), n))
        return out

    def owned_landmarks(self) -> np.ndarray:
        h = self._need()
        m = np.zeros(h.n_pt, dtype=np.uint8)
        h.check(h.L.apexgpu_owned_landmarks(h.h, capi.ptr(m)))
        return m.astype(bool)

    def export_step(self):
        h = self._need()
        step = np.zeros(self._problem.total_dof); grad = np.zeros(self._problem.total_dof)
        h.check(h.L.apexgpu_export_step(h.h, capi.ptr(step), capi.ptr(grad)))
        return step, grad

    @staticmethod
    def lockstep_solve(solvers, lam: float):
        hs = (C.c_void_p * len(solvers))(*[s._need().h for s in solvers])
        h0 = solvers[0]._need()
        rc = h0.L.apexgpu_debug_lockstep_solve(hs, len(solvers), float(lam))
        if rc != 0:
            for s in solvers:
                msg = s._need().L.apexgpu_last_error(s._need().h)
                if msg:
                    raise capi.LinAlgError(rc, msg.decode())
            raise capi.LinAlgError(rc, "lockstep solve")

    def enable_stage_timing(self, on=True): h = self._need(); h.check(h.L.apexgpu_enable_stage_timing(h.h, int(on)))
    def reset_stage_times(self): h = self._need(); h.check(h.L.apexgpu_reset_stage_times(h.h))

    def stage_times(self) -> dict:
        h = self._need()
        ms = (C.c_double * capi.NUM_STAGES)(); n = (C.c_int64 * capi.NUM_STAGES)()
        h.check(h.L.apexgpu_stage_times(h.h, C.byref(ms), C.byref(n)))
        return {name: (ms[i], n[i]) for i, name in enumerate(capi.STAGE_NAMES)}

    def lm_optimize(self, cfg: LevenbergMarquardtConfig):
        h = self._need()
        c = cfg.to_c()
# ... 185 lines not shown
```

### include/apexgpu.h

```cpp
#ifndef APEXGPU_H
#define APEXGPU_H

#include <stdint.h>

#ifdef __cplusplus
extern "C" {
#endif

typedef struct apexgpu_solver apexgpu_solver;

#define APEXGPU_OK 0
#define APEXGPU_ERR_FACTORIZATION_FAILED (-1)
#define APEXGPU_ERR_SINGULAR_MATRIX (-2)
#define APEXGPU_ERR_SPARSE_MATRIX_CREATION (-3)
#define APEXGPU_ERR_MATRIX_CONVERSION (-4)
#define APEXGPU_ERR_INVALID_INPUT (-5)
#define APEXGPU_ERR_INVALID_STATE (-6)
#define APEXGPU_ERR_DEVICE (-10)

#define APEXGPU_MODE_BUNDLE_ADJUSTMENT 0
#define APEXGPU_MODE_SELF_CALIBRATION 1
#define APEXGPU_MODE_ONLY_POSE 2
#define APEXGPU_MODE_ONLY_LANDMARKS 3
#define APEXGPU_MODE_ONLY_INTRINSICS 4
// ... 46 lines not shown
typedef struct {
    int max_iterations;
    double cost_tolerance;
    double parameter_tolerance;
    double gradient_tolerance;
    double damping;
    double damping_min;
    double damping_max;
    double damping_nu;
    double trust_region_radius;
    double min_trust_region_radius;
    double min_cost_threshold;
    double timeout_s;
    int variant;
    int use_jacobi_scaling;
} apexgpu_lm_config;

typedef struct {
    double cost, damping, rho, accepted, gradient_norm, step_norm, predicted_reduction, trial_cost;
} apexgpu_lm_iter;

typedef struct {
    int status;
    int iterations;
    double initial_cost, final_cost, final_gradient_norm, final_step_norm, elapsed_s;
    int cost_evaluations, jacobian_evaluations, successful_steps, unsuccessful_steps;
} apexgpu_lm_result;

int apexgpu_lm_optimize(apexgpu_solver* h, apexgpu_lm_config* cfg, apexgpu_lm_result* result,
                        apexgpu_lm_iter* history, int history_capacity);

int apexgpu_get_residual(apexgpu_solver* h, double* r_out );
int apexgpu_get_jacobian_blocks(apexgpu_solver* h, double* jc_out, double* jl_out);
int apexgpu_get_schur(apexgpu_solver* h, double* S_out, double* gred_out);
int apexgpu_camera_covariance(apexgpu_solver* h, double* cov_out );
int apexgpu_covariance_stats(apexgpu_solver* h, double out[6], double* group_ms, int group_cap);
int apexgpu_landmark_covariance(apexgpu_solver* h, double* cov_out );
int apexgpu_landmark_covariance_stats(apexgpu_solver* h, double out[4]);
int apexgpu_get_landmark_blocks(apexgpu_solver* h, double* hinv_out , double* gl_out );
int apexgpu_debug_invert_blocks(int device, int64_t n, const double* blocks9, double* inv9_out, int32_t* ok_out);
int apexgpu_get_hessian_csc(apexgpu_solver* h, int64_t* nnz_out, int64_t* colptr_out, int64_t* rowidx_out, double* values_out);
int apexgpu_schur_matvec(apexgpu_solver* h, double lambda, const double* x_in, double* y_explicit, double* y_implicit);

int apexgpu_set_option(apexgpu_solver* h, const char* name, int value);

#define APEXGPU_NUM_STAGES 10
int apexgpu_enable_stage_timing(apexgpu_solver* h, int on);
int apexgpu_reset_stage_times(apexgpu_solver* h);
int apexgpu_stage_times(apexgpu_solver* h, double ms[APEXGPU_NUM_STAGES], int64_t calls[APEXGPU_NUM_STAGES]);
int apexgpu_info(apexgpu_solver* h, double info[16]);
int apexgpu_variant_info(apexgpu_solver* h, int asked_variant, int* used_variant, char* reason, int reason_len);
int apexgpu_variant_costs(apexgpu_solver* h, double out[4]);
int apexgpu_counters(apexgpu_solver* h, int64_t out[4]);
int apexgpu_debug_get_pair_records(apexgpu_solver* h, uint32_t* recs4_out, int64_t cap_slots);
int apexgpu_setup_times(apexgpu_solver* h, double seconds[6], double counts[4]);

int apexgpu_get_unique_id(void* out128);
int apexgpu_comm_init(apexgpu_solver* h, int world, int rank, const void* unique_id128);
int apexgpu_comm_init_shm(apexgpu_solver* h, int world, int rank, const char* name);
int apexgpu_set_shard(apexgpu_solver* h, int rank, int world);
int apexgpu_debug_lockstep_solve(apexgpu_solver** hs, int n, double lambda);
int apexgpu_owned_landmarks(apexgpu_solver* h, uint8_t* mask);
int apexgpu_debug_partition(int nt, const uint8_t* present, int world, int* owner_out);
int apexgpu_debug_check_schedule(int nt, const uint8_t* present, int world, int rank, const int opts[8], int64_t out[8], char* msg, int msg_len);
int apexgpu_debug_schedule_ops(int nt, const uint8_t* present, int world, int rank, const int opts[8], int phase, int64_t* rows, int max_rows);
int apexgpu_debug_plan_lists(int nt, const uint8_t* present, int world, int rank, const int opts[8], int which, int64_t* rows, int max_rows);
int apexgpu_debug_sinv_lists(int nt, const uint8_t* present, int64_t* rows, int max_rows, int64_t counts[4], int32_t* slot_out);
int apexgpu_debug_sinv_lists_direct(int nt, const int32_t* slot, int n_groups, const int32_t* group_ptr, const int32_t* group_cols,
                                    int64_t* rows, int max_rows, int64_t counts[4], char* msg, int msg_len);
typedef struct apexgpu_tiles apexgpu_tiles;
int apexgpu_debug_tiles_create(int device, int nt, const uint8_t* present, const int opts[8], apexgpu_tiles** out);
int apexgpu_debug_tiles_pattern(apexgpu_tiles* h, int32_t* slot_out, int64_t info[8]);
int apexgpu_debug_tiles_set(apexgpu_tiles* h, const double* touched, int n_valid, double add_diag, int fill_mode);
int apexgpu_debug_tiles_factor(apexgpu_tiles* h, int* failed_at);
int apexgpu_debug_tiles_solve(apexgpu_tiles* h, int n_rhs, const double* rhs, double* x);
int apexgpu_debug_tiles_matvec(apexgpu_tiles* h, const double* x, double* y);
int apexgpu_debug_tiles_pcg(apexgpu_tiles* h, const double* rhs, int max_iter, double tol, double* x, int* iters, double scal_out[5]);
int apexgpu_debug_tiles_get(apexgpu_tiles* h, int which, double* out, int* recomputed);
void apexgpu_debug_tiles_destroy(apexgpu_tiles* h);
int apexgpu_debug_host_structure(int64_t n_cam, int64_t n_pt, int64_t n_obs, int mode, const uint32_t* cam_idx,
                                 const uint32_t* pt_idx, int rank, int world, const int opts[5], double stats_out[16],
                                 int32_t* cmap_out, uint8_t* owned_out, int32_t* tile_owner_out);
int apexgpu_debug_pair_lists(int64_t n_cam, int64_t n_pt, int64_t n_obs, int dc, const uint32_t* cam_idx, const uint32_t* pt_idx,
                             int64_t counts[4], uint32_t* recs4_out, int32_t* chunks2_out, int64_t* blocks4_out,
                             int32_t* tasks2_out, int32_t* o_index_out);
int apexgpu_debug_pair_lists_queued(int64_t n_cam, int64_t n_pt, int64_t n_obs, const uint32_t* cam_idx, const uint32_t* pt_idx,
                                    int64_t counts[4], uint32_t* recs4_out, int32_t* chunks2_out, int64_t* blocks4_out,
                                    int32_t* tasks2_out, int32_t* o_index_out, int64_t* qdesc3_out);
int apexgpu_debug_pair_lists_queued_dc(int64_t n_cam, int64_t n_pt, int64_t n_obs, int dc, const uint32_t* cam_idx, const uint32_t* pt_idx,
                                       int64_t counts[4], uint32_t* recs4_out, int32_t* chunks2_out, int64_t* blocks4_out,
                                       int32_t* tasks2_out, int32_t* o_index_out, int64_t* qdesc3_out);
int apexgpu_export_step(apexgpu_solver* h, double* step_out, double* grad_out);
int apexgpu_shard_range(int64_t n_pt, int64_t n_obs, const uint32_t* pt_idx, int rank, int world, int64_t* lo,
                        int64_t* hi);

typedef struct apexgpu_bal apexgpu_bal;
#define APEXGPU_BAL_ERR_IO (-20)
#define APEXGPU_BAL_ERR_PARSE (-21)
#define APEXGPU_BAL_ERR_MISSING_FIELDS (-22)
#define APEXGPU_BAL_ERR_INVALID_NUMBER (-23)
int apexgpu_bal_open(const char* path, apexgpu_bal** out);
void apexgpu_bal_close(apexgpu_bal* b);
const char* apexgpu_bal_last_error(void);
int apexgpu_bal_sizes(const apexgpu_bal* b, int64_t* n_cam, int64_t* n_pt, int64_t* n_obs);
int apexgpu_bal_raw(const apexgpu_bal* b, uint32_t* cam_idx, uint32_t* pt_idx, double* obs_uv, double* cameras9,
                    double* points3);
// ... 65 lines not shown
} apexgpu_gn_config;

typedef struct {
    int max_iterations;
    double cost_tolerance;
    double parameter_tolerance;
    double gradient_tolerance;
    double trust_region_radius;
    double trust_region_min;
    double trust_region_max;
    double trust_region_decrease_factor;
    double good_step_quality;
    double poor_step_quality;
    double mu;
    double min_mu;
    double max_mu;
    double mu_increase_factor;
    double min_cost_threshold;
    double timeout_s;
    int variant;
    int use_jacobi_scaling;
    int enable_step_reuse;
} apexgpu_dl_config;

typedef struct {
    double cost, radius, mu, rho, accepted, gradient_norm, step_norm, predicted_reduction, trial_cost, step_type, beta, reused;
} apexgpu_dl_iter;

int apexgpu_pg_jv_gram(apexgpu_pg_solver* h, const double* a, const double* b, double out3[3]);
int apexgpu_pg_dogleg_step(apexgpu_pg_solver* h, double mu, double radius, int reuse, double out8[8]);
int apexgpu_pg_gn_optimize(apexgpu_pg_solver* h, apexgpu_gn_config* cfg, apexgpu_lm_result* result, apexgpu_lm_iter* history,
                           int history_capacity);
int apexgpu_pg_dogleg_optimize(apexgpu_pg_solver* h, apexgpu_dl_config* cfg, apexgpu_lm_result* result, apexgpu_dl_iter* history,
                               int history_capacity);

int apexgpu_jv_gram(apexgpu_solver* h, const double* a, const double* b, double out3[3]);
int apexgpu_dogleg_step(apexgpu_solver* h, double mu, double radius, int reuse, double out8[8]);
int apexgpu_dogleg_optimize(apexgpu_solver* h, apexgpu_dl_config* cfg, apexgpu_lm_result* result, apexgpu_dl_iter* history,
                            int history_capacity);

int apexgpu_pg_get_residual(apexgpu_pg_solver* h, double* r_out);
int apexgpu_pg_get_jacobian_blocks(apexgpu_pg_solver* h, double* j_out);
int apexgpu_pg_get_hessian(apexgpu_pg_solver* h, double lambda, double* H_out, double* g_out);
int apexgpu_pg_covariance(apexgpu_pg_solver* h, double* cov_out );
int apexgpu_pg_covariance_stats(apexgpu_pg_solver* h, double out[6], double* group_ms, int group_cap);

int apexgpu_pg_set_option(apexgpu_pg_solver* h, const char* name, int value);
#define APEXGPU_PG_NUM_STAGES 6
int apexgpu_pg_enable_stage_timing(apexgpu_pg_solver* h, int on);
int apexgpu_pg_reset_stage_times(apexgpu_pg_solver* h);
int apexgpu_pg_stage_times(apexgpu_pg_solver* h, double ms[APEXGPU_PG_NUM_STAGES], int64_t calls[APEXGPU_PG_NUM_STAGES]);
int apexgpu_pg_info(apexgpu_pg_solver* h, double info[8]);
int apexgpu_pg_counters(apexgpu_pg_solver* h, int64_t out[4]);

typedef struct apexgpu_g2o apexgpu_g2o;
#define APEXGPU_G2O_ERR_IO (-30)
#define APEXGPU_G2O_ERR_PARSE (-31)
#define APEXGPU_G2O_ERR_MISSING_FIELDS (-32)
#define APEXGPU_G2O_ERR_INVALID_NUMBER (-33)
#define APEXGPU_G2O_ERR_DUPLICATE_VERTEX (-34)
#define APEXGPU_G2O_ERR_INVALID_QUATERNION (-35)
int apexgpu_g2o_open(const char* path, apexgpu_g2o** out);
void apexgpu_g2o_close(apexgpu_g2o* g);
const char* apexgpu_g2o_last_error(void);
int apexgpu_g2o_sizes(const apexgpu_g2o* g, int64_t* n_vertices_se3, int64_t* n_edges_se3, int64_t* n_vertices_se2,
                      int64_t* n_edges_se2);
int apexgpu_g2o_raw(const apexgpu_g2o* g, int64_t* ids, double* poses7, int64_t* e_from, int64_t* e_to, double* meas7,
                    double* info36);
int apexgpu_g2o_problem(const apexgpu_g2o* g, int64_t* sorted_ids, double* poses7, uint32_t* e_from, uint32_t* e_to,
                        double* meas7, int64_t* pose_col, uint8_t* fix6);
int apexgpu_pose_graph_columns(int64_t n_vertices, const int64_t* ids, int64_t* pose_col);
int apexgpu_g2o_raw_se2(const apexgpu_g2o* g, int64_t* ids, double* poses3, int64_t* e_from, int64_t* e_to, double* meas3,
                        double* info9);
int apexgpu_g2o_problem_se2(const apexgpu_g2o* g, int64_t* sorted_ids, double* poses3, uint32_t* e_from, uint32_t* e_to,
                            double* meas3, int64_t* pose_col, uint8_t* fix3);
int apexgpu_pose_graph_columns_se2(int64_t n_vertices, const int64_t* ids, int64_t* pose_col);
int apexgpu_g2o_problem_information(const apexgpu_g2o* g, int manifold, double* info_out);

#ifdef __cplusplus
}
#endif
#endif
```

Baseline: 12.19 ms.

## Raise wave priority on critical-chain factor units and kernels

Marks factorization units on the critical dependency chain (kFlowCritical) and raises hardware wave priority via s_setprio for potrf, trsm and update kernels and for flow units on that chain. Helper waves in potrf drop priority while spinning. The aim is to shorten the elimination-tree critical path when many independent updates compete for compute units. It is on by default (chain_prio=true, threshold 256). It also adds a debug factor_diag export and a plan table for chain units. The risk is starving non-critical work or adding scheduling overhead.

```diff
diff --git a/apex-solver_amd/capi.py b/apex-solver_amd/capi.py
--- a/apex-solver_amd/capi.py
+++ b/apex-solver_amd/capi.py
@@ -19,7 +19,7 @@
     "apexgpu_step_stats", "apexgpu_eval_step", "apexgpu_commit_step", "apexgpu_discard_step",
     "apexgpu_parameter_norm", "apexgpu_column_norms", "apexgpu_set_column_scaling", "apexgpu_lm_optimize", "apexgpu_get_residual", "apexgpu_get_jacobian_blocks",
     "apexgpu_get_schur", "apexgpu_camera_covariance", "apexgpu_covariance_stats", "apexgpu_landmark_covariance", "apexgpu_landmark_covariance_stats", "apexgpu_get_landmark_blocks", "apexgpu_get_hessian_csc", "apexgpu_debug_invert_blocks", "apexgpu_debug_pair_lists", "apexgpu_debug_pair_lists_queued", "apexgpu_debug_pair_lists_queued_dc", "apexgpu_debug_host_structure", "apexgpu_setup_times", "apexgpu_schur_matvec", "apexgpu_set_option", "apexgpu_enable_stage_timing", "apexgpu_reset_stage_times",
-    "apexgpu_stage_times", "apexgpu_info", "apexgpu_variant_info", "apexgpu_variant_costs", "apexgpu_trim_host_cache", "apexgpu_host_cache_bytes", "apexgpu_counters", "apexgpu_debug_get_pair_records", "apexgpu_get_unique_id", "apexgpu_comm_init", "apexgpu_comm_init_shm", "apexgpu_set_shard", "apexgpu_shard_range",
+    "apexgpu_stage_times", "apexgpu_info", "apexgpu_variant_info", "apexgpu_variant_costs", "apexgpu_trim_host_cache", "apexgpu_host_cache_bytes", "apexgpu_counters", "apexgpu_debug_factor_diag", "apexgpu_pg_debug_factor_diag", "apexgpu_debug_get_pair_records", "apexgpu_get_unique_id", "apexgpu_comm_init", "apexgpu_comm_init_shm", "apexgpu_set_shard", "apexgpu_shard_range",
     "apexgpu_debug_lockstep_solve", "apexgpu_export_step", "apexgpu_owned_landmarks", "apexgpu_debug_partition", "apexgpu_debug_check_schedule",
     "apexgpu_debug_schedule_ops", "apexgpu_debug_plan_lists", "apexgpu_debug_sinv_lists", "apexgpu_debug_sinv_lists_direct",
     "apexgpu_debug_tiles_create", "apexgpu_debug_tiles_pattern", "apexgpu_debug_tiles_set", "apexgpu_debug_tiles_factor",
@@ -197,6 +197,8 @@
     L.apexgpu_variant_info.argtypes = [vp, C.c_int, C.POINTER(C.c_int), C.c_char_p, C.c_int]
     L.apexgpu_variant_costs.argtypes = [vp, C.POINTER(dbl * 4)]
     L.apexgpu_counters.argtypes = [vp, C.POINTER(i64 * 4)]
+    L.apexgpu_debug_factor_diag.argtypes = [vp, vp, C.POINTER(i64)]
+    L.apexgpu_pg_debug_factor_diag.argtypes = [vp, vp, C.POINTER(i64)]
     L.apexgpu_get_unique_id.argtypes = [vp]
     L.apexgpu_comm_init.argtypes = [vp, C.c_int, C.c_int, vp]
     L.apexgpu_comm_init_shm.argtypes = [vp, C.c_int, C.c_int, C.c_char_p]
@@ -328,19 +330,21 @@
 PLAN_TABLES = (("scalars", 23), ("slots", 3), ("columns", 4), ("owner_ranges", 5), ("levels", 9), ("fwd_cut", 2), ("upd_rounds", 2),
                ("bwd_step", 1), ("potrf", 5), ("panel", 7), ("upd", 7), ("fwd", 6), ("bwd", 6), ("flow_fwd", 10), ("flow_bwd", 10),
                ("units", 16), ("sym_row_ptr", 1), ("sym_entries", 3), ("sym_tiles", 3), ("group_cols", 2))
+PLAN_TABLES_MORE = (("chain_units", 5),)
 
 
 def plan_lists(present: np.ndarray, which: str, world: int = 1, rank: int = 0, two_side: int = 1, overlap: int = 1, split_u1: int = 4,
                flood_gate: int = 256, factor_flow: int = -1, factor_flow_rows: int = 24) -> np.ndarray:
     L = load()
     pr = np.ascontiguousarray(present, dtype=np.uint8)
-    w = [n for n, _ in PLAN_TABLES].index(which)
+    tables = PLAN_TABLES + PLAN_TABLES_MORE
+    w = [n for n, _ in tables].index(which)
     opts = np.array([two_side, overlap, split_u1, flood_gate, factor_flow, factor_flow_rows, 0, -1], dtype=np.int32)
     args = (pr.shape[0], pr.ctypes.data_as(C.c_void_p), int(world), int(rank), opts.ctypes.data_as(C.c_void_p), w)
     n = L.apexgpu_debug_plan_lists(*args, None, 0)
     if n < 0:
         raise LinAlgError(n, "apexgpu_debug_plan_lists")
-    rows = np.zeros((n, PLAN_TABLES[w][1]), dtype=np.int64)
+    rows = np.zeros((n, tables[w][1]), dtype=np.int64)
     if n and L.apexgpu_debug_plan_lists(*args, rows.ctypes.data_as(C.c_void_p), n) != n:
         raise LinAlgError(-6, "apexgpu_debug_plan_lists")
     return rows
diff --git a/apex-solver_amd/csrc/capi.cpp b/apex-solver_amd/csrc/capi.cpp
--- a/apex-solver_amd/csrc/capi.cpp
+++ b/apex-solver_amd/csrc/capi.cpp
@@ -75,6 +75,7 @@
     else if (n == "tri_dataflow") s->enable_tri_flow(value != 0);
     else if (n == "split_u1") s->set_split_u1(value);
     else if (n == "flood_gate") s->set_gate_min(value);
+    else if (n == "chain_prio") s->set_chain_prio(value);
     else if (n == "two_side") s->set_two_side(value);
     else if (n == "eager_step_eval") s->set_eager_step_eval(value != 0);
     else if (n == "one_wait") s->set_one_wait(value != 0);
@@ -421,12 +422,13 @@
             *width = 16;
             for (const apex::FactorUnit& u : l.units)
                 row({arr(u.C), idx(u.C), arr(u.A), idx(u.A), arr(u.B), idx(u.B), u.wait_flag[0], u.wait_flag[1], u.wait_flag[2], u.wait_val[0], u.wait_val[1], u.wait_val[2],
-                     u.pub, u.kind, u.strip, u.pad});
+                     u.pub, u.kind & ~apex::kFlowCritical, u.strip, u.pad});
             break;
         case 16: *width = 1; for (int v : l.sym_row_ptr) row({v}); break;
         case 17: *width = 3; for (const apex::SymEntry& e : l.sym_entries) row({e.slot, e.other, e.kind}); break;
         case 18: *width = 3; for (const apex::SymTile& t : l.sym_tiles) row({t.slot, t.I, t.J}); break;
         case 19: *width = 2; for (size_t g = 0; g < s.group_cols.size(); ++g) for (int K : s.group_cols[g]) row({(int64_t)g, K}); break;
+        case 20: *width = 5; for (const apex::FactorUnit& u : l.units) row({u.kind & 15, arr(u.C), idx(u.C), u.strip, (u.kind & apex::kFlowCritical) != 0}); break;
         default: return APEXGPU_ERR_INVALID_INPUT;
     }
     return APEXGPU_OK;
@@ -509,7 +511,7 @@
     H_OR_FAIL;
     const std::string n = name ? name : "";
     static const char* const structural[] = {"schur_form", "hubs_last", "dist_factor", "tree_sharding", "dist_selftest", "nested_dissection", "update_overlap",
-                                             "split_u1", "flood_gate", "two_side", "factor_flow", "factor_flow_rows", "device_pair_list", "matrix_free_only",
+                                             "split_u1", "flood_gate", "chain_prio", "two_side", "factor_flow", "factor_flow_rows", "device_pair_list", "matrix_free_only",
                                              "auto_variant", "variant_cost_permille", "max_tile_updates"};
     if (h->s->has_structure())
         for (const char* k : structural)
@@ -598,6 +600,11 @@
 int apexgpu_counters(apexgpu_solver* h, int64_t out[4]) {
     H_OR_FAIL;
     return counters(h->s, out);
+}
+int apexgpu_debug_factor_diag(apexgpu_solver* h, double* out, int64_t* n) {
+    H_OR_FAIL;
+    if (!n) return APEXGPU_ERR_INVALID_INPUT;
+    return guarded([&] { return h->s->factor_diag(out, n); });
 }
 
 int apexgpu_get_unique_id(void* out128) {
@@ -933,6 +940,11 @@
     PG_OR_FAIL;
     return counters(h->s, out);
 }
+int apexgpu_pg_debug_factor_diag(apexgpu_pg_solver* h, double* out, int64_t* n) {
+    PG_OR_FAIL;
+    if (!n) return APEXGPU_ERR_INVALID_INPUT;
+    return guarded([&] { return h->s->factor_diag(out, n); });
+}
 int apexgpu_pg_info(apexgpu_pg_solver* h, double info[8]) {
     PG_OR_FAIL;
     info[0] = h->s->n_tile_rows(); info[1] = (double)h->s->tile_count(); info[2] = (double)h->s->touched_tiles();
diff --git a/apex-solver_amd/csrc/chol_kernels.h b/apex-solver_amd/csrc/chol_kernels.h
--- a/apex-solver_amd/csrc/chol_kernels.h
+++ b/apex-solver_amd/csrc/chol_kernels.h
@@ -7,11 +7,11 @@
 
 namespace apex {
 
-void launch_potrf_inv(const PotrfTask* tasks, int n, int* fail, hipStream_t s, int* arrived = nullptr);
+void launch_potrf_inv(const PotrfTask* tasks, int n, int* fail, hipStream_t s, int* arrived = nullptr, bool chain_prio = false);
 void launch_gate(const int* arrived, int expected, int max_micros, hipStream_t s);
 void launch_factor_flow(const FactorUnit* units, int n_units, int* ver, int* fail, int* err, hipStream_t s,
                         unsigned long long* trace = nullptr);
-void launch_tile_gemm_nt(const GemmTask* tasks, int n, double alpha, double beta, hipStream_t s, bool tri_b = false);
+void launch_tile_gemm_nt(const GemmTask* tasks, int n, double alpha, double beta, hipStream_t s, bool tri_b = false, bool chain_prio = false);
 void launch_clear_i32(int* p, int64_t n, hipStream_t s);
 void launch_post_word(int* word, int* host_word_dev, hipStream_t s);
 void launch_tri_flow(bool backward, const FlowTask* tasks, int n_tasks, const double* in, double* out, double* part, int* flags,
diff --git a/apex-solver_amd/csrc/chol_kernels.hip b/apex-solver_amd/csrc/chol_kernels.hip
--- a/apex-solver_amd/csrc/chol_kernels.hip
+++ b/apex-solver_amd/csrc/chol_kernels.hip
@@ -114,10 +114,13 @@
 
 template <int NW, bool COH>
 __device__ __forceinline__ void potrf_tile_mf(double* __restrict__ A, double* __restrict__ Linv, int K, int* __restrict__ fail,
-                                              double* sA, double* sD, int* bad, int* sync_cnt) {
+                                              double* sA, double* sD, int* bad, int* sync_cnt, bool prio) {
     constexpr int NT = 64 * NW;
     const int tid = threadIdx.x, lane = tid & 63, w = tid >> 6;
     const int lr = lane & 15, lk = lane >> 4;
+    const int wu = __builtin_amdgcn_readfirstlane(w);
+    const bool helper_u = (wu & 3) != 0;
+    if (prio) { if (wu == 0) __builtin_amdgcn_s_setprio(3); else __builtin_amdgcn_s_setprio(2); }
     constexpr int NH = NW - (NW + 3) / 4;
     const bool helper = (w & 3) != 0;
     const int hid = w - 1 - (w >> 2);
@@ -294,11 +297,13 @@
             __builtin_amdgcn_fence(__ATOMIC_RELEASE, "workgroup");
             if (lane == 0) __hip_atomic_fetch_add(sync_cnt, 1, __ATOMIC_RELAXED, __HIP_MEMORY_SCOPE_WORKGROUP);
         }
+        if (prio && helper_u) __builtin_amdgcn_s_setprio(0);
         if (helper) {
             const int target = (kb + 1) * (NH + 1);
             while (__hip_atomic_load(sync_cnt, __ATOMIC_RELAXED, __HIP_MEMORY_SCOPE_WORKGROUP) < target) __builtin_amdgcn_s_sleep(0);
             __builtin_amdgcn_fence(__ATOMIC_ACQUIRE, "workgroup");
         }
+        if (prio && helper_u) __builtin_amdgcn_s_setprio(2);
         POTRF_STAMP();
     }
     __syncthreads();
@@ -331,19 +336,20 @@
         }
     }
     if (tid == 0 && *bad) atomicCAS(fail, 0, K + 1);
+    if (prio) __builtin_amdgcn_s_setprio(0);
     POTRF_STAMP();
 }
 
 template <int NW>
 __global__ __launch_bounds__(64 * NW) void k_potrf_inv_mf(const PotrfTask* __restrict__ tasks, int* __restrict__ fail,
-                                                          int* __restrict__ arrived) {
+                                                          int* __restrict__ arrived, int prio) {
     if (arrived != nullptr && threadIdx.x == 0) __hip_atomic_fetch_add(arrived, 1, __ATOMIC_RELAXED, __HIP_MEMORY_SCOPE_AGENT);
     POTRF_STAMP();
     __shared__ double sA[NLB * BSZ];
     __shared__ double sD[NBK * BSZ];
     __shared__ int bad, sync_cnt;
     const PotrfTask pt = tasks[blockIdx.x];
-    potrf_tile_mf<NW, false>(pt.A, pt.Linv, pt.K, fail, sA, sD, &bad, &sync_cnt);
+    potrf_tile_mf<NW, false>(pt.A, pt.Linv, pt.K, fail, sA, sD, &bad, &sync_cnt, prio != 0);
 }
 #undef POTRF_STAMP
 
@@ -353,7 +359,7 @@
 constexpr int kGemmSmallMax = 56;
 
 template <bool TRI>
-__global__ __launch_bounds__(256, 3) void k_tile_gemm_nt(const GemmTask* __restrict__ tasks, int n_units, double alpha, double beta) {
+__global__ __launch_bounds__(256, 3) void k_tile_gemm_nt(const GemmTask* __restrict__ tasks, int n_units, double alpha, double beta, int prio) {
     constexpr int P4 = KC + 2;
     constexpr int IMG = (NB + STRIP) * P4;
     __shared__ double sm[IMG];
@@ -430,6 +436,7 @@
             }
         }
     };
+    if (prio) __builtin_amdgcn_s_setprio(1);
     gload(0);
     for (int k0 = 0; k0 < NB; k0 += KC) {
         __syncthreads();
@@ -482,7 +489,7 @@
 }
 
 __global__ __launch_bounds__(192) void k_tile_gemm_nt_small(const GemmTask* __restrict__ tasks, int n_units, double alpha,
-                                                              double beta) {
+                                                              double beta, int prio) {
     __shared__ double sA[48 * PS];
     __shared__ double sB[48 * PS];
     const int unit = blockIdx.x;
@@ -518,6 +525,7 @@
 #pragma unroll
             for (int r = 0; r < 4; ++r) cv[j][r] = C[(size_t)(16 * w + lk + 4 * r) * NB + 16 * j + lr];
     }
+    if (prio) __builtin_amdgcn_s_setprio(1);
     gload(0);
     for (int k0 = 0; k0 < NB; k0 += KS) {
         __syncthreads();
@@ -549,7 +557,7 @@
 }
 
 __global__ __launch_bounds__(576) void k_tile_gemm_nt_small_strip(const GemmTask* __restrict__ tasks, int n_units, double alpha,
-                                                                    double beta) {
+                                                                    double beta, int prio) {
     __shared__ double sA[48 * PS];
     __shared__ double sB[NB * PS];
     const int unit = blockIdx.x;
@@ -580,6 +588,7 @@
             rb[i] = *reinterpret_cast<GlobalCF64x2>(Bg + (size_t)row * NB + k0 + 2 * c2);
         }
     };
+    if (prio) __builtin_amdgcn_s_setprio(1);
     gload(0);
     for (int k0 = 0; k0 < NB; k0 += KS) {
         __syncthreads();
@@ -950,7 +959,9 @@
     const int wr = w / 3, wc = w % 3;
     const int bi = u.strip / 3, bj = u.strip % 3;
     const __amdgpu_buffer_rsrc_t rC = coh_rsrc(u.C), rA = coh_rsrc(u.A), rB = coh_rsrc(u.B);
+    const bool crit = __builtin_amdgcn_readfirstlane(u.kind & kFlowCritical) != 0;
     flow_wait_unit(ver, u, tid, err);
+    if (crit) __builtin_amdgcn_s_setprio(1);
     if (trace && tid == 0) trace[1] = wall_clock64();
     const bool act = tid < 576;
     double cv[4] = {0.0, 0.0, 0.0, 0.0};
@@ -986,6 +997,7 @@
         for (int r = 0; r < 4; ++r)
             coh_st1(rC, (48 * bi + 16 * wr + lk + 4 * r) * NB + 48 * bj + 16 * wc + lr, -1.0 * acc[r] + 1.0 * cv[r]);
     }
+    if (crit) __builtin_amdgcn_s_setprio(0);
     flow_publish(ver + u.pub, tid);
 }
 
@@ -997,7 +1009,9 @@
     const __amdgpu_buffer_rsrc_t rC = coh_rsrc(u.C), rB = coh_rsrc(u.B);
     constexpr int C2 = KS / 2, NCH = NB / KS, NRB = NB * C2 / 576;
     static_assert(NB * C2 % 576 == 0 && 16 * C2 <= 576, "staging loops assume whole rounds");
+    const bool crit = __builtin_amdgcn_readfirstlane(u.kind & kFlowCritical) != 0;
     flow_wait_unit(ver, u, tid, err);
+    if (crit) __builtin_amdgcn_s_setprio(1);
     if (trace && tid == 0) trace[1] = wall_clock64();
     const bool act = tid < 576;
     double2 ra[NCH], rb[NCH][NRB];
@@ -1036,6 +1050,7 @@
 #pragma unroll
         for (int r = 0; r < 4; ++r) coh_st1(rC, (row0 + lk + 4 * r) * NB + 16 * w + lr, acc[r]);
     }
+    if (crit) __builtin_amdgcn_s_setprio(0);
     flow_publish(ver + u.pub, tid);
 }
 
@@ -1130,7 +1145,8 @@
     if (kind == 0) {
         flow_wait_unit(ver, u, tid, err);
         if (trace && tid == 0) trace[1] = wall_clock64();
-        potrf_tile_mf<kFlowFactorThreads / 64, true>(u.C, const_cast<double*>(u.A), u.strip, fail, smem, smem + NLB * BSZ, &bad, &sync_cnt);
+        potrf_tile_mf<kFlowFactorThreads / 64, true>(u.C, const_cast<double*>(u.A), u.strip, fail, smem, smem + NLB * BSZ, &bad, &sync_cnt,
+                                                     __builtin_amdgcn_readfirstlane(u.kind & kFlowCritical) != 0);
         __builtin_amdgcn_s_waitcnt(0);
         __syncthreads();
         if (tid == 0) __hip_atomic_fetch_add(ver + u.pub, kFlowUnitsPerTile, __ATOMIC_RELAXED, __HIP_MEMORY_SCOPE_AGENT);
@@ -1198,20 +1214,21 @@
     if (n_units <= 0) return;
     hipLaunchKernelGGL(k_factor_flow, dim3(n_units), dim3(kFlowFactorThreads), 0, s, units, ver, fail, err, trace);
 }
-void launch_potrf_inv(const PotrfTask* tasks, int n, int* fail, hipStream_t s, int* arrived) {
+void launch_potrf_inv(const PotrfTask* tasks, int n, int* fail, hipStream_t s, int* arrived, bool chain_prio) {
     if (n <= 0) return;
-    hipLaunchKernelGGL(k_potrf_inv_mf<12>, dim3(n), dim3(768), 0, s, tasks, fail, arrived);
-}
-void launch_tile_gemm_nt(const GemmTask* tasks, int n, double alpha, double beta, hipStream_t s, bool tri_b) {
+    hipLaunchKernelGGL(k_potrf_inv_mf<12>, dim3(n), dim3(768), 0, s, tasks, fail, arrived, chain_prio ? 1 : 0);
+}
+void launch_tile_gemm_nt(const GemmTask* tasks, int n, double alpha, double beta, hipStream_t s, bool tri_b, bool chain_prio) {
     if (n <= 0) return;
+    const int prio = chain_prio ? 1 : 0;
     if (n <= kGemmSmallMax) {
-        if (beta != 0.0) hipLaunchKernelGGL(k_tile_gemm_nt_small, dim3(9 * n), dim3(192), 0, s, tasks, 9 * n, alpha, beta);
-        else hipLaunchKernelGGL(k_tile_gemm_nt_small_strip, dim3(3 * n), dim3(576), 0, s, tasks, 3 * n, alpha, beta);
+        if (beta != 0.0) hipLaunchKernelGGL(k_tile_gemm_nt_small, dim3(9 * n), dim3(192), 0, s, tasks, 9 * n, alpha, beta, prio);
+        else hipLaunchKernelGGL(k_tile_gemm_nt_small_strip, dim3(3 * n), dim3(576), 0, s, tasks, 3 * n, alpha, beta, prio);
         return;
     }
     const int units = n * NSTRIP, per_xcd = (units + 7) / 8;
-    if (tri_b) hipLaunchKernelGGL(k_tile_gemm_nt<true>, dim3(8 * per_xcd), dim3(256), 0, s, tasks, units, alpha, beta);
-    else hipLaunchKernelGGL(k_tile_gemm_nt<false>, dim3(8 * per_xcd), dim3(256), 0, s, tasks, units, alpha, beta);
+    if (tri_b) hipLaunchKernelGGL(k_tile_gemm_nt<true>, dim3(8 * per_xcd), dim3(256), 0, s, tasks, units, alpha, beta, prio);
+    else hipLaunchKernelGGL(k_tile_gemm_nt<false>, dim3(8 * per_xcd), dim3(256), 0, s, tasks, units, alpha, beta, prio);
 }
 void launch_tri_step(bool trans, const TriTask* tasks, int n, double* vwork, double* vout, hipStream_t s) {
     if (n <= 0) return;
diff --git a/apex-solver_amd/csrc/factor_schedule.cpp b/apex-solver_amd/csrc/factor_schedule.cpp
--- a/apex-solver_amd/csrc/factor_schedule.cpp
+++ b/apex-solver_amd/csrc/factor_schedule.cpp
@@ -7,15 +7,16 @@
 std::vector<SchedOp> factor_schedule(const ScheduleInput& in, int g0, int g1) {
     const std::vector<Level>& lv_ = in.lv;
     std::vector<SchedOp> ops;
-    auto launch = [&](StreamId s, int list, int64_t first, int64_t n, int arrive = -1) {
-        if (n > 0) ops.push_back({kOpLaunch, (uintptr_t)s, 0, list, first, (int)n, arrive});
+    auto launch = [&](StreamId s, int list, int64_t first, int64_t n, int arrive = -1, bool chain = false) {
+        if (n > 0) ops.push_back({kOpLaunch, (uintptr_t)s, 0, list, first, (int)n, arrive, chain ? 1 : 0});
     };
+    auto on_chain = [&](int64_t n) { return in.chain_prio > 0 && n <= in.chain_prio; };
     auto wait = [&](StreamId s, int lv, LevelEvent k) { ops.push_back({kOpWait, (uintptr_t)s, (uintptr_t)lv * kLevelEvents + k, -1, 0, 0, -1}); };
     auto record = [&](int lv, LevelEvent k, StreamId s) { ops.push_back({kOpRecord, (uintptr_t)s, (uintptr_t)lv * kLevelEvents + k, -1, 0, 0, -1}); };
-    auto potrf = [&](int lv) { launch(kMain, 0, lv_[lv].potrf, lv_[lv + 1].potrf - lv_[lv].potrf, in.gate_min > 0 ? lv : -1); };
-    auto panel = [&](int lv) { launch(kMain, 1, lv_[lv].panel, lv_[lv + 1].panel - lv_[lv].panel); };
-    auto updates = [&](int r0, int r1, StreamId s) {
-        for (int r = r0; r < r1; ++r) launch(s, 2, in.upd_rounds[r].first, in.upd_rounds[r].second);
+    auto potrf = [&](int lv) { launch(kMain, 0, lv_[lv].potrf, lv_[lv + 1].potrf - lv_[lv].potrf, in.gate_min > 0 ? lv : -1, in.chain_prio > 0); };
+    auto panel = [&](int lv) { const int64_t n = lv_[lv + 1].panel - lv_[lv].panel; launch(kMain, 1, lv_[lv].panel, n, -1, on_chain(n)); };
+    auto updates = [&](int r0, int r1, StreamId s, bool chain = false) {
+        for (int r = r0; r < r1; ++r) launch(s, 2, in.upd_rounds[r].first, in.upd_rounds[r].second, -1, chain && on_chain(in.upd_rounds[r].second));
     };
     auto gate = [&](int lv, StreamId s) { ops.push_back({kOpGate, (uintptr_t)s, 0, -1, lv + 1, lv_[lv + 2].potrf - lv_[lv + 1].potrf, -1}); };
     const bool two = in.overlap && in.n_levels > 2;
@@ -59,7 +60,7 @@
                 last_b = -1;
             }
         }
-        updates(r0, rd, kMain);
+        updates(r0, rd, kMain, true);
         updates(rd, rs, has_o ? kSo : kMain);
         o_pending = has_o;
         if (has_o) record(lv, kEvO, kSo);
diff --git a/apex-solver_amd/csrc/factor_schedule.h b/apex-solver_amd/csrc/factor_schedule.h
--- a/apex-solver_amd/csrc/factor_schedule.h
+++ b/apex-solver_amd/csrc/factor_schedule.h
@@ -29,6 +29,7 @@
     int64_t first;
     int count;
     int arrive;
+    int prio = 0;
 };
 
 struct Level { int potrf = 0, panel = 0, fwd = 0, upd = 0, u1o = 0, u2a = 0, u2b1 = 0, u2b2 = 0; std::vector<int> fwd_cut; };
@@ -44,6 +45,7 @@
     bool skip_idle_wait;
     bool flow_on;
     struct Flow { int g0, g1, first, n; } flow[2];
+    int chain_prio = 0;
 };
 
 std::vector<SchedOp> factor_schedule(const ScheduleInput& in, int g0, int g1);
diff --git a/apex-solver_amd/csrc/plan_lists.cpp b/apex-solver_amd/csrc/plan_lists.cpp
--- a/apex-solver_amd/csrc/plan_lists.cpp
+++ b/apex-solver_amd/csrc/plan_lists.cpp
@@ -686,6 +686,25 @@
         for (FactorUnit& u : out->units) u.kind &= 15;
     }
 }
+
+void mark_chain_units(const PlanStructure& s, const double* tiles, PlanLists* out) {
+    std::vector<int> row_of((size_t)s.n_slots, -1), col_of((size_t)s.n_slots, -1);
+    for (int I = 0; I < s.nt; ++I)
+        for (int J = 0; J <= I; ++J)
+            if (s.slot_of(I, J) >= 0) { row_of[(size_t)s.slot_of(I, J)] = I; col_of[(size_t)s.slot_of(I, J)] = J; }
+    auto slot_of_ptr = [&](const double* c) { return (size_t)((c - tiles) / (ptrdiff_t)(kNB * kNB)); };
+    auto narrow = [&](int J) { return s.group_of[J] >= 0 && s.group_cols[(size_t)s.group_of[J]].size() <= 2; };
+    for (FactorUnit& u : out->units) {
+        const int kind = u.kind & 15;
+        bool chain = kind == 0;
+        if (kind == 1 || kind == 2) {
+            const int I = row_of[slot_of_ptr(u.C)], J = col_of[slot_of_ptr(u.C)];
+            if (kind == 1) chain = narrow(J);
+            else { const int K = col_of[slot_of_ptr(u.A)]; chain = s.group_of[J] == s.group_of[K] + 1 && (I == J || narrow(J)); }
+        }
+        if (chain) u.kind |= kFlowCritical;
+    }
+}
 }
 
 std::string build_plan_lists(const PlanStructure& s, const std::vector<uint8_t>& present, const PlanOptions& o, double* tiles, double* linv, PlanLists* out) {
@@ -697,6 +716,7 @@
     out->two_side_plan = o.two_side == 2 || (o.two_side == 1 && (int64_t)out->upd.size() >= 256 * (int64_t)s.n_levels());
     const std::string e = flow_regions(s, o.flow_cols, o.flow_rows, tiles, linv, out);
     if (e.empty()) flag_first_writers(s, tiles, out);
+    if (e.empty() && o.chain_prio) mark_chain_units(s, tiles, out);
     return e;
 }
 
diff --git a/apex-solver_amd/csrc/plan_lists.h b/apex-solver_amd/csrc/plan_lists.h
--- a/apex-solver_amd/csrc/plan_lists.h
+++ b/apex-solver_amd/csrc/plan_lists.h
@@ -19,6 +19,7 @@
     int flow_cols = -1, flow_rows = 24;
     int64_t max_updates = 80000000LL;
     double cost_limit_ms = 0.0;
+    bool chain_prio = true;
 };
 
 using PlanCols = std::vector<std::vector<int>>;
@@ -71,11 +72,12 @@
     int gate_min = 256;
     bool skip_idle_wait = false;
     bool flow_on = true;
+    int chain_prio = 256;
 };
 inline ScheduleInput schedule_input(const PlanStructure& s, const PlanLists& l, const ScheduleSwitches& w) {
     const PlanLists::Flow* f = l.flow;
     return ScheduleInput{l.lv, l.upd_rounds, s.n_levels(), s.n_local_groups, w.overlap, w.overlap_min, w.split_u1, w.split_u1_min, l.two_side_plan,
-                         w.gate_min, w.skip_idle_wait, w.flow_on, {{f[0].g0, f[0].g1, f[0].first, f[0].n}, {f[1].g0, f[1].g1, f[1].first, f[1].n}}};
+                         w.gate_min, w.skip_idle_wait, w.flow_on, {{f[0].g0, f[0].g1, f[0].first, f[0].n}, {f[1].g0, f[1].g1, f[1].first, f[1].n}}, w.chain_prio};
 }
 
 std::vector<int> tile_order(int nt, const std::vector<uint8_t>& adj, bool nested_dissection, int leaf, int n_fixed_last = 1);
diff --git a/apex-solver_amd/csrc/tile_backend.h b/apex-solver_amd/csrc/tile_backend.h
--- a/apex-solver_amd/csrc/tile_backend.h
+++ b/apex-solver_amd/csrc/tile_backend.h
@@ -35,6 +35,7 @@
     void set_split_u1(int min_tasks) { tp_.set_split_u1(min_tasks); }
     void set_overlap_min(int n) { tp_.set_overlap_min(n); }
     void set_gate_min(int n) { tp_.set_gate_min(n); }
+    void set_chain_prio(int v) { tp_.set_chain_prio(v); }
     void set_two_side(int mode) { tp_.set_two_side(mode); }
     void set_factor_flow(int max_cols, int max_rows) { tp_.set_factor_flow(max_cols, max_rows); }
     int factor_flow_timeouts() const { return n_factor_flow_timeouts_; }
@@ -71,6 +72,11 @@
     struct ExportSegment { const double* dev; const ColumnMap* map; const JacobiScaling* scale; };
     int export_columns(std::initializer_list<ExportSegment> segs, ExportAs as, double* out);
     int export_tiles_dense(const ColumnMap& map, int64_t ld, int64_t slot_bound, double* out);
+
+   public:
+    int factor_diag(double* out, int64_t* n);
+
+   protected:
 
     virtual int rebuild_system(double lambda, double reg) = 0;
     virtual int factor_now(int* failed, bool defer_flags) = 0;
diff --git a/apex-solver_amd/csrc/tile_backend.hip b/apex-solver_amd/csrc/tile_backend.hip
--- a/apex-solver_amd/csrc/tile_backend.hip
+++ b/apex-solver_amd/csrc/tile_backend.hip
@@ -95,6 +95,18 @@
     return kOk;
 }
 
+int TileBackend::factor_diag(double* out, int64_t* n) {
+    *n = tp_.n_pad();
+    if (!out) return kOk;
+    if (!tp_.factor_valid()) return fail(kInvalidState, "no factor is held");
+    DeviceBuffer<double> d;
+    HIP_TRY(d.alloc((size_t)tp_.n_pad()));
+    tp_.diag(d);
+    HIP_TRY(hipMemcpyAsync(out, d, (size_t)tp_.n_pad() * sizeof(double), hipMemcpyDeviceToHost, stream_));
+    HIP_TRY(hipStreamSynchronize(stream_));
+    return kOk;
+}
+
 int TileBackend::enqueue_eager_eval() {
     if (!eager_host_) HIP_TRY(eager_host_.alloc(8));
     int n = 0;
diff --git a/apex-solver_amd/csrc/tile_plan.h b/apex-solver_amd/csrc/tile_plan.h
--- a/apex-solver_amd/csrc/tile_plan.h
+++ b/apex-solver_amd/csrc/tile_plan.h
@@ -2,6 +2,7 @@
 #include <hip/hip_runtime.h>
 #include <stdint.h>
 
+#include <algorithm>
 #include <array>
 #include <functional>
 #include <string>
@@ -81,6 +82,7 @@
     void enable_overlap(bool on) { sw_.overlap = on; }
     void set_overlap_min(int n) { sw_.overlap_min = n; }
     void set_two_side(int mode) { opts_.two_side = mode; }
+    void set_chain_prio(int v) { opts_.chain_prio = v != 0; sw_.chain_prio = v == 1 ? ScheduleSwitches().chain_prio : std::max(v, 0); }
     void set_gate_min(int n) { sw_.gate_min = n; }
     void set_factor_flow(int max_cols, int max_rows) { opts_.flow_cols = max_cols; if (max_rows > 0) opts_.flow_rows = max_rows; }
     int factor_flow_groups() const { return !sw_.flow_on ? 0 : (lists_.flow[0].g1 - lists_.flow[0].g0) + (lists_.flow[1].g1 - lists_.flow[1].g0); }
diff --git a/apex-solver_amd/csrc/tile_plan.hip b/apex-solver_amd/csrc/tile_plan.hip
--- a/apex-solver_amd/csrc/tile_plan.hip
+++ b/apex-solver_amd/csrc/tile_plan.hip
@@ -149,9 +149,9 @@
         const hipStream_t s = stream_of(o.stream);
         switch (o.op) {
             case kOpLaunch:
-                if (o.list == 0) launch_potrf_inv(potrf_tasks_ + o.first, o.count, flag_, s, o.arrive >= 0 ? gate_cnt_ + o.arrive : nullptr);
-                else if (o.list == 1) launch_tile_gemm_nt(trsm_tasks_ + o.first, o.count, 1.0, 0.0, s, true);
-                else if (o.list == 2) launch_tile_gemm_nt(upd_tasks_ + o.first, o.count, -1.0, 1.0, s);
+                if (o.list == 0) launch_potrf_inv(potrf_tasks_ + o.first, o.count, flag_, s, o.arrive >= 0 ? gate_cnt_ + o.arrive : nullptr, o.prio != 0);
+                else if (o.list == 1) launch_tile_gemm_nt(trsm_tasks_ + o.first, o.count, 1.0, 0.0, s, true, o.prio != 0);
+                else if (o.list == 2) launch_tile_gemm_nt(upd_tasks_ + o.first, o.count, -1.0, 1.0, s, false, o.prio != 0);
                 else launch_factor_flow(flow_units_ + o.first, o.count, flow_ver_, flag_, flag_ + 1, s, flow_trace_ ? flow_trace_ + 3 * (size_t)o.first : nullptr);
                 break;
             case kOpRecord: (void)hipEventRecord(ev_[o.event / kLevelEvents][o.event % kLevelEvents], s); break;
diff --git a/apex-solver_amd/csrc/tile_tasks.h b/apex-solver_amd/csrc/tile_tasks.h
--- a/apex-solver_amd/csrc/tile_tasks.h
+++ b/apex-solver_amd/csrc/tile_tasks.h
@@ -17,6 +17,7 @@
 };
 
 constexpr int kFlowFirstWriter = 16;
+constexpr int kFlowCritical = 32;
 constexpr int kFlowUnitsPerTile = 9;
 struct FactorUnit {
     double* C;
diff --git a/apex-solver_amd/pose_graph.py b/apex-solver_amd/pose_graph.py
--- a/apex-solver_amd/pose_graph.py
+++ b/apex-solver_amd/pose_graph.py
@@ -495,6 +495,13 @@
     def set_option(self, name: str, value: int):
         h = self._need(); h.check(h.L.apexgpu_pg_set_option(h.h, name.encode(), int(value)))
 
+    def factor_diag(self) -> np.ndarray:
+        h = self._need(); n = C.c_int64(0)
+        h.check(h.L.apexgpu_pg_debug_factor_diag(h.h, None, C.byref(n)))
+        out = np.zeros(n.value)
+        h.check(h.L.apexgpu_pg_debug_factor_diag(h.h, capi.ptr(out), C.byref(n)))
+        return out
+
     def counters(self) -> dict:
         h = self._need(); out = (C.c_int64 * 4)()
         h.check(h.L.apexgpu_pg_counters(h.h, C.byref(out)))
diff --git a/apex-solver_amd/solver.py b/apex-solver_amd/solver.py
--- a/apex-solver_amd/solver.py
+++ b/apex-solver_amd/solver.py
@@ -497,6 +497,13 @@
         h = self._need(); out = (C.c_int64 * 4)()
         h.check(h.L.apexgpu_counters(h.h, C.byref(out)))
         return dict(sweep_timeouts=int(out[0]), tri_dataflow=bool(out[1]), factor_flow_timeouts=int(out[2]), factor_flow_groups=int(out[3]))
+
+    def factor_diag(self) -> np.ndarray:
+        h = self._need(); n = C.c_int64(0)
+        h.check(h.L.apexgpu_debug_factor_diag(h.h, None, C.byref(n)))
+        out = np.zeros(n.value)
+        h.check(h.L.apexgpu_debug_factor_diag(h.h, capi.ptr(out), C.byref(n)))
+        return out
 
     def setup_times(self) -> dict:
         h = self._need(); sec = (C.c_double * 6)(); cnt = (C.c_double * 4)()
diff --git a/include/apexgpu.h b/include/apexgpu.h
--- a/include/apexgpu.h
+++ b/include/apexgpu.h
@@ -122,6 +122,7 @@
 int apexgpu_variant_info(apexgpu_solver* h, int asked_variant, int* used_variant, char* reason, int reason_len);
 int apexgpu_variant_costs(apexgpu_solver* h, double out[4]);
 int apexgpu_counters(apexgpu_solver* h, int64_t out[4]);
+int apexgpu_debug_factor_diag(apexgpu_solver* h, double* out, int64_t* n);
 int apexgpu_debug_get_pair_records(apexgpu_solver* h, uint32_t* recs4_out, int64_t cap_slots);
 int apexgpu_setup_times(apexgpu_solver* h, double seconds[6], double counts[4]);
 
@@ -293,6 +294,7 @@
 int apexgpu_pg_stage_times(apexgpu_pg_solver* h, double ms[APEXGPU_PG_NUM_STAGES], int64_t calls[APEXGPU_PG_NUM_STAGES]);
 int apexgpu_pg_info(apexgpu_pg_solver* h, double info[8]);
 int apexgpu_pg_counters(apexgpu_pg_solver* h, int64_t out[4]);
+int apexgpu_pg_debug_factor_diag(apexgpu_pg_solver* h, double* out, int64_t* n);
 
 typedef struct apexgpu_g2o apexgpu_g2o;
 #define APEXGPU_G2O_ERR_IO (-30)
```

Result: no change. 12.04 ms (median of 3 runs) (-1.2%).
